# joshspeagle/brutus

Hardware: AMD Instinct MI355X
Metric: stars/sec at 750k-model x 12-band grid; achieved HBM GB/s vs peak (higher is better)
Workload: dtype f64; 1 GPU; configs[1]: 750k-model x 12-band grid, Av-only solve (rvlim=(3.32,3.32)), no parallax; grid = synth.make_mist_like_grid (lattice-ordered like the MIST grid files); grid_generator=mist_like, nmodel=750000, nfilt=12, sub_batch=128, selected_models_last_sub_batch=44670752, streams_per_gpu=3, parallelism=stars sharded, 1 rank(s), no data-path collective

## Files before the change

### brutus_amd/csrc/fastmath.hpp

```cpp
#pragma once

namespace {

__constant__ double kExp2Tbl[64] = {
    1, 1.0108892860517005, 1.0218971486541166, 1.0330248790212284,
    1.0442737824274138, 1.0556451783605572, 1.0671404006768237, 1.0787607977571199,
    1.0905077326652577, 1.1023825833078409, 1.1143867425958924, 1.1265216186082418,
    1.1387886347566916, 1.1511892299529827, 1.1637248587775775, 1.1763969916502812,
    1.189207115002721, 1.2021567314527031, 1.215247359980469, 1.22848053610687,
    1.241857812073484, 1.2553807570246911, 1.2690509571917332, 1.2828700160787783,
    1.2968395546510096, 1.3109612115247644, 1.3252366431597413, 1.3396675240533029,
    1.3542555469368927, 1.3690024229745905, 1.383909881963832, 1.3989796725383112,
    1.4142135623730951, 1.42961333839197, 1.4451808069770467, 1.460917794180647,
    1.4768261459394993, 1.4929077282912648, 1.5091644275934228, 1.5255981507445384,
    1.5422108254079407, 1.5590044002378369, 1.5759808451078865, 1.593142151342267,
    1.6104903319492543, 1.6280274218573478, 1.6457554781539649, 1.6636765803267364,
    1.681792830507429, 1.7001063537185235, 1.7186192981224779, 1.7373338352737062,
    1.7562521603732995, 1.7753764925265212, 1.7947090750031072, 1.8142521755003989,
    1.8340080864093424, 1.8539791250833855, 1.8741676341103, 1.8945759815869656,
    1.9152065613971474, 1.9360617934922943, 1.9571441241754002, 1.9784560263879509};

__device__ __forceinline__ double fast_exp10(double x, const double *__restrict__ tbl = kExp2Tbl) {
    const double ns = fma(x, 212.60339807279118, 6755399441055744.0);
    const double n = ns - 6755399441055744.0;
    double r = fma(-n, 0.0047035936804604717, x);
    r = fma(-n, 1.7892345153159123e-12, r);
    double pl = 0.5393829291955817;
    pl = fma(pl, r, 1.1712551489122673);
    pl = fma(pl, r, 2.034678592293477);
    pl = fma(pl, r, 2.6509490552391997);
    pl = fma(pl, r, 2.302585092994046);
    pl = fma(pl, r, 1.0);
    const int ni = __double2loint(ns);
    return ldexp(tbl[ni & 63] * pl, ni >> 6);
}

__device__ __forceinline__ double poly_exp10(double x) {
    const double n = rint(x * 3.3219280948873623);
    double r = fma(-n, 3.01029995663839276e-01, x);
    r = fma(-n, 1.42502325707809354e-17, r);
    const double t = r * 2.3025850929940457;
    double pl = 1.6059043836821613e-10;
    pl = fma(pl, t, 2.08767569878681e-09);
    pl = fma(pl, t, 2.505210838544172e-08);
    pl = fma(pl, t, 2.755731922398589e-07);
    pl = fma(pl, t, 2.7557319223985893e-06);
    pl = fma(pl, t, 2.48015873015873e-05);
    pl = fma(pl, t, 1.984126984126984e-04);
    pl = fma(pl, t, 1.3888888888888889e-03);
    pl = fma(pl, t, 8.333333333333333e-03);
    pl = fma(pl, t, 4.1666666666666664e-02);
    pl = fma(pl, t, 1.6666666666666666e-01);
    pl = fma(pl, t, 0.5);
    pl = fma(pl, t, 1.0);
    pl = fma(pl, t, 1.0);
    return ldexp(pl, (int)n);
}

__device__ __forceinline__ void stage_exp_table(double *lds_tbl) {
    if (threadIdx.x < 64) lds_tbl[threadIdx.x] = kExp2Tbl[threadIdx.x];
}

__device__ __forceinline__ double fast_exp(double x, const double *__restrict__ tbl = kExp2Tbl) {
    if (!(x > -745.)) return x == x ? 0. : x;
    const double n = rint(x * 92.332482616893657);
    double r = fma(-n, 0.01083042469326756, x);
    r = fma(-n, 2.9815858269852933e-12, r);
    double pl = 8.3333333333333332e-03;
    pl = fma(pl, r, 4.1666666666666664e-02);
    pl = fma(pl, r, 1.6666666666666666e-01);
    pl = fma(pl, r, 0.5);
    pl = fma(pl, r, 1.0);
    pl = fma(pl, r, 1.0);
    const int ni = (int)n;
    return ldexp(tbl[ni & 63] * pl, ni >> 6);
}

__device__ __forceinline__ double fast_log(double x) {
    if (!(x > 0.) || !(x < INFINITY)) return log(x);
    int e;
    double m = frexp(x, &e);
    if (m < 0.70710678118654752440) {
        m *= 2.;
        --e;
    }
    const double s = (m - 1.) / (m + 1.);
    const double z = s * s;
    double pl = 1. / 21.;
    pl = fma(pl, z, 1. / 19.);
    pl = fma(pl, z, 1. / 17.);
    pl = fma(pl, z, 1. / 15.);
    pl = fma(pl, z, 1. / 13.);
    pl = fma(pl, z, 1. / 11.);
    pl = fma(pl, z, 1. / 9.);
    pl = fma(pl, z, 1. / 7.);
    pl = fma(pl, z, 1. / 5.);
    pl = fma(pl, z, 1. / 3.);
    const double lm = fma(2. * s * z, pl, 2. * s);
    const double ed = (double)e;
    return fma(ed, 6.93147180369123816490e-01, fma(ed, 1.90821492927058770002e-10, lm));
}

__device__ __forceinline__ double fast_rcp(double x) {
    double r = __builtin_amdgcn_rcp(x);
    r = fma(fma(-x, r, 1.), r, r);
    r = fma(fma(-x, r, 1.), r, r);
    return r;
}
__device__ __forceinline__ void fast_sqrt_rsqrt(double x, double &sq, double &rsq) {
    const double y = __builtin_amdgcn_rsq(x);
    double g = x * y, h = 0.5 * y;
    const double r = fma(-h, g, 0.5);
    g = fma(g, r, g);
    h = fma(h, r, h);
    g = fma(fma(-g, g, x), h, g);
    g = fma(fma(-g, g, x), h, g);
    double y2 = h + h;
    y2 = fma(y2, fma(-y2, g, 1.), y2);
    y2 = fma(y2, fma(-y2, g, 1.), y2);
    sq = x == 0. ? 0. : g;
    rsq = y2;
}
__device__ __forceinline__ void fast_sqrt_rsqrt_pos(double x, double &sq, double &rsq) {
    const double y = __builtin_amdgcn_rsq(x);
    double g = x * y, h = 0.5 * y;
    const double r = fma(-h, g, 0.5);
    g = fma(g, r, g);
    h = fma(h, r, h);
    g = fma(fma(-g, g, x), h, g);
    g = fma(fma(-g, g, x), h, g);
    double y2 = h + h;
    y2 = fma(y2, fma(-y2, g, 1.), y2);
    y2 = fma(y2, fma(-y2, g, 1.), y2);
    sq = g;
    rsq = y2;
}
__device__ __forceinline__ double fast_sqrt_pos(double x) {
    double g, h;
    fast_sqrt_rsqrt_pos(x, g, h);
    return g;
}
__device__ __forceinline__ double fast_sqrt(double x) {
    double g, h;
    fast_sqrt_rsqrt(x, g, h);
    return g;
}
__device__ __forceinline__ double fast_exp_bf(double x, const double *__restrict__ tbl) {
    const double xc = fmax(x, -745.);
    const double ns = fma(xc, 92.332482616893657, 6755399441055744.0);
    const double n = ns - 6755399441055744.0;
    double r = fma(-n, 0.01083042469326756, xc);
    r = fma(-n, 2.9815858269852933e-12, r);
    double pl = 8.3333333333333332e-03;
    pl = fma(pl, r, 4.1666666666666664e-02);
    pl = fma(pl, r, 1.6666666666666666e-01);
    pl = fma(pl, r, 0.5);
    pl = fma(pl, r, 1.0);
    pl = fma(pl, r, 1.0);
    const int ni = __double2loint(ns);
    const double v = ldexp(tbl[ni & 63] * pl, ni >> 6);
    return x > -745. ? v : (x == x ? 0. : x);
}
__device__ __forceinline__ double fast_exp_fin(double x, const double *__restrict__ tbl) {
    const double xc = fmax(x, -745.);
    const double ns = fma(xc, 92.332482616893657, 6755399441055744.0);
    const double n = ns - 6755399441055744.0;
    double r = fma(-n, 0.01083042469326756, xc);
    r = fma(-n, 2.9815858269852933e-12, r);
    double pl = 8.3333333333333332e-03;
    pl = fma(pl, r, 4.1666666666666664e-02);
    pl = fma(pl, r, 1.6666666666666666e-01);
    pl = fma(pl, r, 0.5);
    pl = fma(pl, r, 1.0);
    pl = fma(pl, r, 1.0);
    const int ni = __double2loint(ns);
    return ldexp(tbl[ni & 63] * pl, ni >> 6);
}
__device__ __forceinline__ double fast_log_r(double x) {
    int e;
    double m = frexp(x, &e);
    const bool lo = m < 0.70710678118654752440;
    m = lo ? 2. * m : m;
    e = lo ? e - 1 : e;
    const double s = (m - 1.) * fast_rcp(m + 1.);
    const double z = s * s;
    double pl = 1. / 21.;
    pl = fma(pl, z, 1. / 19.);
    pl = fma(pl, z, 1. / 17.);
    pl = fma(pl, z, 1. / 15.);
    pl = fma(pl, z, 1. / 13.);
    pl = fma(pl, z, 1. / 11.);
    pl = fma(pl, z, 1. / 9.);
    pl = fma(pl, z, 1. / 7.);
    pl = fma(pl, z, 1. / 5.);
    pl = fma(pl, z, 1. / 3.);
    const double lm = fma(2. * s * z, pl, 2. * s);
    const double ed = (double)e;
    const double v = fma(ed, 6.93147180369123816490e-01, fma(ed, 1.90821492927058770002e-10, lm));
    return x > 0. ? (x < INFINITY ? v : x) : (x == 0. ? -INFINITY : nan(""));
}
__device__ __forceinline__ double fast_log_pos(double x) {
    int e;
    double m = frexp(x, &e);
    const bool lo = m < 0.70710678118654752440;
    m = lo ? 2. * m : m;
    e = lo ? e - 1 : e;
    const double s = (m - 1.) * fast_rcp(m + 1.);
    const double z = s * s;
    double pl = 1. / 21.;
    pl = fma(pl, z, 1. / 19.);
    pl = fma(pl, z, 1. / 17.);
    pl = fma(pl, z, 1. / 15.);
    pl = fma(pl, z, 1. / 13.);
    pl = fma(pl, z, 1. / 11.);
    pl = fma(pl, z, 1. / 9.);
    pl = fma(pl, z, 1. / 7.);
    pl = fma(pl, z, 1. / 5.);
    pl = fma(pl, z, 1. / 3.);
    const double lm = fma(2. * s * z, pl, 2. * s);
    const double ed = (double)e;
    return fma(ed, 6.93147180369123816490e-01, fma(ed, 1.90821492927058770002e-10, lm));
}

}
```

### brutus_amd/csrc/fit2_kernels.hpp

```cpp
#pragma once

#include "fit_kernels.hpp"
#include "pre32_types.hpp"

namespace {

static_assert(PS_TILE == TILE && PS_NBMAX == NBMAX, "pre32_types.hpp and common.hpp disagree");

struct CallInit {
    int32_t *ids_all, *kfix, *k2, *counters;
    int ncounters;
};
__global__ void __launch_bounds__(64)
k_prep32(int nstar, const StarPrep *__restrict__ stars, float eps_scale, int dim_prior,
         Star32 *__restrict__ out, CallInit init) {
    static_assert(NBMAX <= 64, "one lane per band");
    __shared__ double s_a[NBMAX], s_b[NBMAX], s_c[NBMAX];
    __shared__ double s_gbar, s_D;
    __shared__ int s_bad;
    const int s = blockIdx.x, j = threadIdx.x;
    if (s >= nstar) return;
    if (init.ids_all && j == 0) {
        init.ids_all[s] = s;
        init.kfix[s] = 2;
// ... 171 lines not shown
                    ub2 += bw;
                    uy2 += yw;
                    aa2 = pk_fma(a, aw, aa2);
                    ab2 = pk_fma(a, bw, ab2);
                    bb2 = pk_fma(b, bw, bb2);
                    ay2 = pk_fma(a, yw, ay2);
                    by2 = pk_fma(b, yw, by2);
                    yy2 = pk_fma(y, yw, yy2);
                }
                const float ua = hsum(ua2), ub = hsum(ub2), uy = hsum(uy2), aa = hsum(aa2),
                            ab = hsum(ab2), bb = hsum(bb2), ay = hsum(ay2), by = hsum(by2),
                            yy = hsum(yy2);
                auto sweep = [&](float &dav_o, float &drv_o) -> float {
                    const float uR = ua + rv * ub;
                    const float RR = aa + rv * (2.f * ab + rv * bb);
                    const float yR = ay + rv * by;
                    float rs = uy - av * uR;
                    const float ra = (yR - av * RR) + (p.av_mean - av) * p.av_ivar;
                    const float a_den = RR + p.av_ivar;
                    float dav = (sp.S * ra - uR * rs) * __builtin_amdgcn_rcpf(sp.S * a_den - uR * uR);
                    dav = fmaxf(dav, p.avmin - av);
                    dav = fminf(dav, p.avmax - av);
                    av += dav;
                    const float r_den = bb * av * av + p.rv_ivar;
                    const float sr = ub * av;
                    rs = uy - av * uR;
                    const float bres = by - av * (ab + rv * bb);
                    const float rr = av * bres + (p.rv_mean - rv) * p.rv_ivar;
                    float drv = (sp.S * rr - sr * rs) * __builtin_amdgcn_rcpf(sp.S * r_den - sr * sr);
                    drv = fmaxf(drv, p.rvmin - rv);
                    drv = fminf(drv, p.rvmax - rv);
                    rv += drv;
                    const float RR2 = aa + rv * (2.f * ab + rv * bb);
                    const float yR2 = ay + rv * by;
                    dav_o = dav;
                    drv_o = drv;
                    const float uR2 = ua + rv * ub;
                    const float oc = (uy - av * uR2) * __builtin_amdgcn_rcpf(sp.S);
                    const float tt0 = (sp.gbar - mbar) + oc;
                    return -0.5f * ((yy - av * (2.f * yR2 - av * RR2)) + sp.S * (tt0 * tt0 - oc * oc));
                };
                float d1, d2;
                if (K >= 1) {
                    const float lw = sweep(d1, d2);
                    if (live) {
                        if (lw == lw) {
                            const float st = fmaxf(fabsf(d1), fabsf(d2));
                            mx[g][0] = fmaxf(mx[g][0], lw);
                            if (st >= p.mtol_hi) mx[g][1] = fmaxf(mx[g][1], lw);
                            if (st >= p.mtol_lo) mx[g][2] = fmaxf(mx[g][2], lw);
                        } else {
                            mx[g][8] = 1.f;
                        }
                    }
                }
                if (K >= 2) {
                    const float lw = sweep(d1, d2);
                    if (live) {
                        if (lw == lw) {
                            const float st = fmaxf(fabsf(d1), fabsf(d2));
                            mx[g][3] = fmaxf(mx[g][3], lw);
                            if (st >= p.mtol_hi) mx[g][4] = fmaxf(mx[g][4], lw);
                            if (st >= p.mtol_lo) mx[g][5] = fmaxf(mx[g][5], lw);
                        } else {
                            mx[g][8] = 1.f;
                        }
                    }
                }
                for (int k = 2; k < K; ++k) sweep(d1, d2);
            }
            float num, den;
            if constexpr (RVF) {
                num = 0.f;
                den = 0.f;
#pragma unroll
                for (int j = 0; j < NB; ++j) {
                    const float e = __builtin_amdgcn_exp2f(fmaf(C10 * av, R[j], mcC[j]));
                    const float fw = e * sp.iv[j];
                    num = fmaf(sp.dd[j], fw, num);
                    den = fmaf(e, fw, den);
                }
            } else {
                f32x2 num2 = 0.f, den2 = 0.f;
#pragma unroll
                for (int j = 0; j < NB; j += 2) {
                    const f32x2 Rj = pk_fma((f32x2)rv, ld2(dr + j), ld2(R + j));
                    const f32x2 arg = C10 * pk_fma((f32x2)av, Rj, ld2(mc + j));
                    const f32x2 e = {__builtin_amdgcn_exp2f(arg.x), __builtin_amdgcn_exp2f(arg.y)};
                    const f32x2 fw = e * ld2(sp.iv + j);
                    num2 = pk_fma(ld2(sp.dd + j), fw, num2);
                    den2 = pk_fma(e, fw, den2);
                }
                num = hsum(num2);
                den = hsum(den2);
            }
            const float q = __builtin_amdgcn_exp2f(C10 * (sp.gbar - mbar));
            float tt = num * __builtin_amdgcn_rcpf(den);
            float sc = tt * q;
            if (sc <= 1e-20f) {
                sc = 1e-20f;
                tt = sc * __builtin_amdgcn_rcpf(q);
            }
            const float chi2 = fmaf(tt, fmaf(tt, den, -2.f * num), sp.DD2);
            const float lnl = -0.5f * chi2;
            float lnlp = lnl;
            if (sp.has_par) {
                const float dp = __builtin_amdgcn_sqrtf(sc) - sp.par;
                lnlp = lnl - 0.5f * (dp * dp * sp.par_ivar);
            }
            float lnpr = lnl;
            if (p.dim_prior) lnpr = sp.c0 + sp.c1 * __logf(chi2) - 0.5f * chi2;
            if (sp.sp_on) {
                const float vt = sp.sp_var + q * q * __builtin_amdgcn_rcpf(den);
                const float ds = sc - sp.sp_mean;
                lnpr += -0.5f * (ds * ds * __builtin_amdgcn_rcpf(vt) + __logf(6.2831853071795865f * vt));
            }
            if (!(chi2 > 4.f * sp.eps) || !sp.ok) lnlp = NAN;
            lnpr = surv_clean(lnpr);
            if (!(chi2 > sp.chi2_lo) || !sp.ok) lnpr = NAN;
            if (live) {
                const int64_t o = (int64_t)s * nmodel + i;
                lnlp32[o] = lnlp;
                lnpr32[o] = lnpr;
                if (lnlp != lnlp || lnpr != lnpr) mx[g][9] = 1.f;
                if (lnlp > mx[g][6]) mx[g][6] = lnlp;
                if (lnpr > mx[g][7]) mx[g][7] = lnpr;
            }
        }
    }
    const int lane = threadIdx.x & 63;
    const int wv = __builtin_amdgcn_readfirstlane(threadIdx.x >> 6);
#pragma unroll
    for (int g = 0; g < G; ++g)
#pragma unroll
        for (int v = 0; v < NV32; ++v) {
            float x = mx[g][v];
#pragma unroll
            for (int off = 32; off > 0; off >>= 1) x = fmaxf(x, __shfl_xor(x, off, 64));
            if (lane == 0) slot[wv][g * NV32 + v] = x;
        }
    __syncthreads();
    if (threadIdx.x < G * NV32) {
        const int g = threadIdx.x / NV32, v = threadIdx.x % NV32;
        if (g < ng) {
            const int s = star_ids[g0 + g];
            const float x = fmaxf(fmaxf(slot[0][threadIdx.x], slot[1][threadIdx.x]),
                                  fmaxf(slot[2][threadIdx.x], slot[3][threadIdx.x]));
            part[((int64_t)bx * nstar + s) * NV32 + v] = x;
        }
    }
}

__global__ void k_pre_decide(int nblkx, int nstar, const int32_t *__restrict__ star_ids,
                             const float *__restrict__ part, const Star32 *__restrict__ stars,
                             float ln_init, int rvf, int32_t *kfix,
                             int accept, float *__restrict__ st32, int32_t *__restrict__ k1,
                             int32_t *__restrict__ status, double *__restrict__ nomA,
                             int32_t *ctr, int32_t *__restrict__ probe_ids,
                             int32_t *__restrict__ redo_ids, const int32_t *nrun_dev) {
    __shared__ float sm[NV32][4];
    if (nrun_dev && (int)blockIdx.x >= *nrun_dev) return;
    const int s = star_ids[blockIdx.x];
    float v[NV32];
    for (int q = 0; q < NV32; ++q) v[q] = -INFINITY;
    for (int b = threadIdx.x; b < nblkx; b += blockDim.x) {
        const float *pp = part + ((int64_t)b * nstar + s) * NV32;
        for (int q = 0; q < NV32; ++q) v[q] = fmaxf(v[q], pp[q]);
    }
    for (int q = 0; q < NV32; ++q) {
        float x = v[q];
        for (int off = 32; off > 0; off >>= 1) x = fmaxf(x, __shfl_xor(x, off, 64));
        if ((threadIdx.x & 63) == 0) sm[q][threadIdx.x >> 6] = x;
    }
    __syncthreads();
    if (threadIdx.x != 0) return;
    for (int q = 0; q < NV32; ++q)
        v[q] = fmaxf(fmaxf(sm[q][0], sm[q][1]), fmaxf(sm[q][2], sm[q][3]));
    for (int q = 0; q < NV32; ++q) st32[(int64_t)s * NV32 + q] = v[q];
    const Star32 &sp = stars[s];
    const float ew = 2.f * sp.epsw;
    int st = 2, K1 = 0;
    const int K = kfix[s];
    if (sp.ok && !(v[8] > 0.f) && v[0] > -INFINITY) {
        const bool cont1 = v[1] > v[0] + ln_init + ew;
        const bool may1 = v[2] > v[0] + ln_init - ew;
        if (!may1) {
            K1 = 1;
            st = (rvf || K == 1) ? 0 : 1;
        } else if (cont1) {
            if (rvf) {
                K1 = 2;
                st = 0;
            } else if (K >= 2) {
                const bool cont2 = v[4] > v[3] + ln_init + ew;
                const bool may2 = v[5] > v[3] + ln_init - ew;
                if (!may2) {
                    K1 = 2;
                    st = (K == 2) ? 0 : 2;
                } else if (cont2) {
                    st = 2;
                }
            }
        }
    }
    if (!accept) {
        k1[s] = K1;
        status[s] = st;
        if (ctr) {
            if (st == 1) {
                kfix[s] = K1;
                redo_ids[atomicAdd(ctr + 1, 1)] = s;
            } else if (st == 2) {
                probe_ids[atomicAdd(ctr + 0, 1)] = s;
            }
        }
    }
    nomA[s] = (double)v[6] - 2. * (double)sp.eps;
}

template <int NB, bool RVF>
struct Tile64 {
    Coef<NB> c;
    double F0[NB];
    double R[RVF ? NB : 1];
};

template <int NB, bool RVF>
__device__ __forceinline__ void tile_load(const float *__restrict__ grid, int64_t nmodel_pad,
                                          int64_t i, double rv_mean, Tile64<NB, RVF> &t) {
    load_coef<NB>(grid, nmodel_pad, i, t.c);
    load_F0<NB>(grid, nmodel_pad, i, t.F0);
    if constexpr (RVF) coef_R<NB>(t.c, rv_mean, t.R);
}

template <int NB, bool RVF>
__device__ __forceinline__ void mag_phase(const Tile64<NB, RVF> &t, const StarPrep &sp,
                                          const DevParams &p, int K, double &av, double &rv) {
    av = p.av_mean;
    rv = p.rv_mean;
    if constexpr (RVF) {
        GramR Gm;
        gram_init_rf<NB>(t.c, t.R, sp, Gm);
        double a_, c_;
        if (K > 0) gram_sweep_rf(Gm, sp.S, p, av, a_, c_);
    } else {
        Gram Gm;
        gram_init<NB>(t.c, sp, Gm);
        for (int k = 0; k < K; ++k) {
            double a_, b_, c_;
            gram_sweep(Gm, sp.S, p, av, rv, a_, b_, c_);
        }
    }
}

template <int NB, bool RVF, bool FULL>
__device__ __forceinline__ void mle_at(const Tile64<NB, RVF> &t, const StarPrep &sp,
                                       const DevParams &p, double av, double rv,
                                       const double *__restrict__ tbl, Mle &m) {
    if constexpr (RVF) mle_fast_rf<NB, true, FULL ? 2 : 0>(t.c, t.R, t.F0, sp, p, av, tbl, m);
    else mle_fast<NB, true, FULL ? 2 : 0>(t.c, t.F0, sp, p, av, rv, tbl, m);
}

__device__ __forceinline__ void audit(float *__restrict__ aud, int s, float f32v, double f64v,
                                      double thr) {
    if (aud && f64v > thr - 12. && f32v == f32v) {
        const float d = fabsf((float)(f64v - (double)f32v));
        atomicMax(reinterpret_cast<int *>(aud + s), __float_as_int(d));
    }
}

__device__ __forceinline__ int64_t mword(int s, int ntile, int t, int w) {
    return (int64_t)s * (4 * ntile) + (int64_t)t * 4 + w;
}

__global__ void __launch_bounds__(256)
k_hot_list(int nblkx, int nstar, int mode, const float *__restrict__ part32,
           const double *__restrict__ nomA, const double *__restrict__ maxsurv,
           const Star32 *__restrict__ s32, double *__restrict__ nomB, double *__restrict__ part,
           int32_t *__restrict__ hot, int32_t *__restrict__ nhot) {
    const int s = blockIdx.x;
    double nm;
    if (mode == 0) {
        nm = nomA[s];
    } else {
        nm = maxsurv[s] - (double)s32[s].eps;
        if (threadIdx.x == 0) nomB[s] = nm;
    }
    for (int b = threadIdx.x; b < nblkx; b += blockDim.x) {
        const float *pp = part32 + ((int64_t)b * nstar + s) * NV32;
        const bool is_hot = !((double)pp[6 + mode] < nm) || pp[9] > 0.f;
        if (is_hot) hot[atomicAdd(nhot, 1)] = b * BRUTUS_MAX_BATCH + s;
        else part[(int64_t)b * nstar + s] = -INFINITY;
    }
}

template <int NB, bool RVF>
__global__ void __launch_bounds__(TILE, top_waves(NB))
k_top1(const float *__restrict__ grid, int64_t nmodel, int64_t nmodel_pad, int nstar,
       const StarPrep *__restrict__ stars, DevParams p, const int32_t *__restrict__ k1, int ntile,
       int mode, const float *__restrict__ plane32, const double *__restrict__ nom,
       const int32_t *__restrict__ hot, const int32_t *__restrict__ nhot,
       double *__restrict__ part, float *__restrict__ aud) {
    __shared__ double slot[4];
    __shared__ double s_tbl[64];
    const int n = *nhot;
    if ((int)blockIdx.x >= n) return;
    stage_exp_table(s_tbl);
    __syncthreads();
    const int lane = threadIdx.x & 63;
    for (int e = blockIdx.x; e < n; e += gridDim.x) {
        const int entry = hot[e];
        const int b = entry / BRUTUS_MAX_BATCH, s = entry - b * BRUTUS_MAX_BATCH;
        const int t0 = b * F2_T, t1 = min(ntile, t0 + F2_T);
        const StarPrep &sp = stars[s];
        const double nm_s = nom[s];
        const int K = k1[s];
        float v[F2_T];
#pragma unroll
        for (int u = 0; u < F2_T; ++u) {
            const int64_t i = (int64_t)(t0 + u) * TILE + threadIdx.x;
            v[u] = plane32[(int64_t)s * nmodel + (i < nmodel ? i : nmodel - 1)];
        }
        double mx = -INFINITY;
#pragma unroll
        for (int u = 0; u < F2_T; ++u) {
            const int64_t i = (int64_t)(t0 + u) * TILE + threadIdx.x;
            bool mine = t0 + u < t1 && i < nmodel && !((double)v[u] < nm_s);
            if (mode == 1 && mine) mine = !surv_is(v[u]);
            if (__ballot(mine) == 0ull) continue;
            Tile64<NB, RVF> tl;
            tile_load<NB, RVF>(grid, nmodel_pad, i, p.rv_mean, tl);
            double av, rv;
            mag_phase<NB, RVF>(tl, sp, p, K, av, rv);
            Mle m;
            mle_at<NB, RVF, false>(tl, sp, p, av, rv, s_tbl, m);
            double val;
            if (mode == 0) val = cull_stat(sp, m);
            else val = first_cut_lnprob(sp, final_lnl<false>(sp, p, m.chi2, false), m.scale, m.i00);
            if (mine) audit(aud, s, v[u], val, nm_s);
            if (mine && val == val) mx = val > mx ? val : mx;
        }
        block_max_store(mx, slot, part + (int64_t)b * nstar + s);
    }
}

__global__ void k_top_decide(int nblkx, int nstar, const int32_t *__restrict__ star_ids, int mode,
                             const double *__restrict__ part, const Star32 *__restrict__ s32,
                             double ln_thr, const double *__restrict__ maxsurv,
                             double *__restrict__ thr, double *__restrict__ cand) {
    __shared__ double sm[4];
    const int s = star_ids[blockIdx.x];
    double v = -INFINITY;
    for (int b = threadIdx.x; b < nblkx; b += blockDim.x) {
        const double x = part[(int64_t)b * nstar + s];
        v = x > v ? x : v;
    }
    v = wave_max(v);
    if ((threadIdx.x & 63) == 0) sm[threadIdx.x >> 6] = v;
    __syncthreads();
    if (threadIdx.x != 0) return;
    v = sm[0];
    for (int w = 1; w < 4; ++w) v = sm[w] > v ? sm[w] : v;
    if (mode == 0) {
        thr[s] = v + ln_thr;
        cand[s] = v + ln_thr - (double)s32[s].eps;
    } else {
        const double m = maxsurv[s] > v ? maxsurv[s] : v;
        thr[s] = m + ln_thr;
    }
}

__global__ void __launch_bounds__(TILE)
k_cmp_count32(int64_t nmodel, int ntile, const float *__restrict__ plane,
              const double *__restrict__ thr, int64_t *__restrict__ counts,
              unsigned long long *__restrict__ mask) {
    __shared__ int wsum[4];
    const int s = blockIdx.y, c = blockIdx.x;
    const int t0 = (int)((int64_t)ntile * c / NCHUNK), t1 = (int)((int64_t)ntile * (c + 1) / NCHUNK);
    const double th = thr[s];
    int n = 0;
#ifndef CNT_U
#define CNT_U 16
#endif
    constexpr int U = CNT_U;
    for (int tb = t0; tb < t1; tb += U) {
        float v[U];
#pragma unroll
        for (int u = 0; u < U; ++u) {
            const int64_t i = (int64_t)(tb + u) * TILE + threadIdx.x;
            const bool in = tb + u < t1 && i < nmodel;
            const float x = plane[(int64_t)s * nmodel + (in ? i : nmodel - 1)];
            v[u] = in ? x : -INFINITY;
        }
#pragma unroll
        for (int u = 0; u < U; ++u) {
            if (tb + u >= t1) break;
            const bool hit = !((double)v[u] < th);
            n += hit ? 1 : 0;
            const unsigned long long b = __ballot(hit);
            if ((threadIdx.x & 63) == 0)
                mask[(int64_t)s * (4 * ntile) + (int64_t)(tb + u) * 4 + (threadIdx.x >> 6)] = b;
        }
    }
#pragma unroll
    for (int off = 32; off > 0; off >>= 1) n += __shfl_xor(n, off, 64);
    if ((threadIdx.x & 63) == 0) wsum[threadIdx.x >> 6] = n;
    __syncthreads();
    if (threadIdx.x == 0) counts[(int64_t)s * NCHUNK + c] = wsum[0] + wsum[1] + wsum[2] + wsum[3];
}

__global__ void __launch_bounds__(TILE)
k_sel_classify(int64_t nmodel, int ntile, const Star32 *__restrict__ s32,
               const float *__restrict__ lnpr32,
               const double *__restrict__ lnprob_st, const int64_t *__restrict__ cand_off,
               const double *__restrict__ thr_sel,
               int64_t *__restrict__ counts, unsigned long long *__restrict__ mask,
               int64_t *__restrict__ dcounts, unsigned long long *__restrict__ dmask,
               int32_t *__restrict__ bandq, int32_t *__restrict__ bandn) {
    __shared__ int qn;
    __shared__ int wsum[4], dsum[4];
    if (threadIdx.x == 0) qn = 0;
    __syncthreads();
    const int s = blockIdx.y, c = blockIdx.x;
    const int t0 = (int)((int64_t)ntile * c / NCHUNK), t1 = (int)((int64_t)ntile * (c + 1) / NCHUNK);
    const double th = thr_sel[s];
    const double e = (double)s32[s].eps;
    const int64_t cbase = cand_off[s];
    int32_t *queue = bandq + (int64_t)s * nmodel + (int64_t)t0 * TILE;
    int n = 0, nd = 0;
#ifndef CLS_U
#define CLS_U 12
#endif
    constexpr int U = CLS_U;
    for (int tb = t0; tb < t1; tb += U) {
        float v32[U];
#pragma unroll
        for (int u = 0; u < U; ++u) {
            const int64_t i = (int64_t)(tb + u) * TILE + threadIdx.x;
            const bool in = tb + u < t1 && i < nmodel;
            const float x = lnpr32[(int64_t)s * nmodel + (in ? i : nmodel - 1)];
            v32[u] = in ? x : -INFINITY;
        }
        double vst[U];
#pragma unroll
        for (int u = 0; u < U; ++u)
            vst[u] = surv_is(v32[u]) ? lnprob_st[cbase + surv_slot(v32[u])] : 0.;
#pragma unroll
        for (int u = 0; u < U; ++u) {
            const int t = tb + u;
            if (t >= t1) break;
            const int64_t i = (int64_t)t * TILE + threadIdx.x;
            bool yes = false, der = false, bd = false;
            if (i < nmodel) {
                if (surv_is(v32[u])) {
                    yes = vst[u] > th;
                } else {
                    const double v = (double)v32[u];
                    yes = der = v >= th + e;
                    bd = !yes && !(v < th - e);
                }
            }
            n += yes ? 1 : 0;
            nd += der ? 1 : 0;
            const unsigned long long b = __ballot(yes), bdr = __ballot(der);
            if ((threadIdx.x & 63) == 0) {
                const int64_t a = (int64_t)s * (4 * ntile) + (int64_t)t * 4 + (threadIdx.x >> 6);
                mask[a] = b;
                dmask[a] = bdr;
            }
            if (bd) queue[atomicAdd(&qn, 1)] = (int32_t)i;
        }
    }
#pragma unroll
    for (int off = 32; off > 0; off >>= 1) {
        n += __shfl_xor(n, off, 64);
        nd += __shfl_xor(nd, off, 64);
    }
    if ((threadIdx.x & 63) == 0) {
        wsum[threadIdx.x >> 6] = n;
        dsum[threadIdx.x >> 6] = nd;
    }
    __syncthreads();
    if (threadIdx.x == 0) {
        counts[(int64_t)s * NCHUNK + c] = wsum[0] + wsum[1] + wsum[2] + wsum[3];
        dcounts[(int64_t)s * NCHUNK + c] = dsum[0] + dsum[1] + dsum[2] + dsum[3];
        bandn[s * NCHUNK + c] = qn;
    }
}

constexpr int LIST_U = 4;
static_assert(F2_T % LIST_U == 0, "a unit of the list passes must not straddle two blocks");

__device__ __forceinline__ unsigned long long
live_blocks(const float *__restrict__ part32, int nstar, int s, int b0, int blast, double cand,
            bool first_cut, double thr_lo) {
    const int b = b0 + (int)(threadIdx.x & 63);
    bool live = true;
    if (b <= blast) {
        const float *pp = part32 + ((int64_t)b * nstar + s) * NV32;
        const float m6 = pp[6], m7 = pp[7], f9 = pp[9];
        const bool dead = ((double)m6 < cand) & (f9 <= 0.f) & (!first_cut | ((double)m7 < thr_lo));
        live = !dead;
    }
    return __ballot(live);
}

template <bool V4>
__device__ __forceinline__ int64_t unit_model(int t, int k, int lane) {
    return (int64_t)t * TILE + (V4 ? 4 * lane + k : 64 * k + lane);
}
template <bool V4>
__device__ __forceinline__ void unit_load(const float *__restrict__ row, int64_t nmodel, int q,
                                          int ta, int tz, int lane, float (&v)[LIST_U][4]) {
#pragma unroll
    for (int u = 0; u < LIST_U; ++u) {
        const int t = q * LIST_U + u;
        const bool tin = t >= ta && t < tz;
        if constexpr (V4) {
            const int64_t i = unit_model<true>(t, 0, lane);
            const bool in = tin && i < nmodel;
            const float4 x = *reinterpret_cast<const float4 *>(row + (in ? i : nmodel - 4));
            v[u][0] = in ? x.x : -INFINITY;
            v[u][1] = in ? x.y : -INFINITY;
            v[u][2] = in ? x.z : -INFINITY;
            v[u][3] = in ? x.w : -INFINITY;
        } else {
#pragma unroll
            for (int k = 0; k < 4; ++k) {
                const int64_t i = unit_model<false>(t, k, lane);
                const bool in = tin && i < nmodel;
                const float x = row[in ? i : nmodel - 1];
                v[u][k] = in ? x : -INFINITY;
            }
        }
    }
}

template <bool V4>
__device__ __forceinline__ void tile_words(unsigned long long *__restrict__ mrow, int t, bool tin, int lane,
                                           const bool (&hit)[4]) {
    if constexpr (V4) {
        int y = ((hit[0] ? 1 : 0) | (hit[1] ? 2 : 0) | (hit[2] ? 4 : 0) | (hit[3] ? 8 : 0)) << (4 * (lane & 7));
        y |= dpp_i32<0xB1, 0xf>(y);
        y |= dpp_i32<0x4E, 0xf>(y);
        y |= dpp_i32<0x141, 0xf>(y);
        if (tin && (lane & 7) == 0) reinterpret_cast<int *>(mrow)[(int64_t)t * 8 + (lane >> 3)] = y;
    } else {
#pragma unroll
        for (int k = 0; k < 4; ++k) {
            const unsigned long long b = __ballot(hit[k]);
            if (tin && lane == 0) mrow[(int64_t)t * 4 + k] = b;
        }
    }
}
__device__ __forceinline__ void zero_words(unsigned long long *__restrict__ mrow, int ta, int tz, int lane) {
    if (lane < (tz - ta) * 8) reinterpret_cast<int *>(mrow)[(int64_t)ta * 8 + lane] = 0;
}

template <class F>
__device__ __forceinline__ void walk_units(int t0, int t1, const float *__restrict__ part32, int nstar,
                                           int s, double cand, bool first_cut, double thr_lo, F f) {
    if (t0 >= t1) return;
    constexpr int QB = F2_T / LIST_U;
    const int w = __builtin_amdgcn_readfirstlane((int)(threadIdx.x >> 6));
    const int blast = (t1 - 1) / F2_T;
    for (int bs = t0 / F2_T; bs <= blast; bs += 64) {
        const unsigned long long live = live_blocks(part32, nstar, s, bs, blast, cand, first_cut, thr_lo);
        const int qa = max(t0 / LIST_U, bs * QB);
        const int qz = min((t1 + LIST_U - 1) / LIST_U, (bs + 64) * QB);
        for (int q = qa + w; q < qz; q += TILE / 64)
            f(q, max(q * LIST_U, t0), min(q * LIST_U + LIST_U, t1), ((live >> (q / QB - bs)) & 1ull) != 0ull);
    }
}

template <bool V4>
__global__ void __launch_bounds__(TILE)
k_cmp_count32_live(int64_t nmodel, int ntile, int nstar, const float *__restrict__ plane,
                   const float *__restrict__ part32, const double *__restrict__ thr,
                   int64_t *__restrict__ counts, unsigned long long *__restrict__ mask) {
    __shared__ int wsum[4];
    const int s = blockIdx.y, c = blockIdx.x;
    const int t0 = (int)((int64_t)ntile * c / NCHUNK), t1 = (int)((int64_t)ntile * (c + 1) / NCHUNK);
    const double th = thr[s];
    const int lane = threadIdx.x & 63;
    const float *row = plane + (int64_t)s * nmodel;
    unsigned long long *mrow = mask + (int64_t)s * (4 * ntile);
    int n = 0;
    walk_units(t0, t1, part32, nstar, s, th, false, 0., [&](int q, int ta, int tz, bool live) {
        if (!live) {
            zero_words(mrow, ta, tz, lane);
            return;
        }
        float v[LIST_U][4];
        unit_load<V4>(row, nmodel, q, ta, tz, lane, v);
#pragma unroll
        for (int u = 0; u < LIST_U; ++u) {
            const int t = q * LIST_U + u;
            const bool tin = t >= ta && t < tz;
            bool hit[4];
#pragma unroll
            for (int k = 0; k < 4; ++k) {
                hit[k] = tin & (unit_model<V4>(t, k, lane) < nmodel) & !((double)v[u][k] < th);
                n += hit[k] ? 1 : 0;
            }
            tile_words<V4>(mrow, t, tin, lane, hit);
        }
    });
#pragma unroll
    for (int off = 32; off > 0; off >>= 1) n += __shfl_xor(n, off, 64);
    if (lane == 0) wsum[threadIdx.x >> 6] = n;
    __syncthreads();
    if (threadIdx.x == 0) counts[(int64_t)s * NCHUNK + c] = wsum[0] + wsum[1] + wsum[2] + wsum[3];
}

__global__ void __launch_bounds__(TILE)
k_sel_classify_live(int64_t nmodel, int ntile, int nstar, const Star32 *__restrict__ s32,
                    const float *__restrict__ lnpr32, const float *__restrict__ part32,
                    const double *__restrict__ candS,
                    const double *__restrict__ lnprob_st, const int64_t *__restrict__ cand_off,
                    const double *__restrict__ thr_sel,
                    int64_t *__restrict__ counts, unsigned long long *__restrict__ mask,
                    int64_t *__restrict__ dcounts, unsigned long long *__restrict__ dmask,
                    int32_t *__restrict__ bandq, int32_t *__restrict__ bandn) {
    __shared__ int qn;
    __shared__ int wsum[4], dsum[4];
    if (threadIdx.x == 0) qn = 0;
    __syncthreads();
    const int s = blockIdx.y, c = blockIdx.x;
    const int t0 = (int)((int64_t)ntile * c / NCHUNK), t1 = (int)((int64_t)ntile * (c + 1) / NCHUNK);
    const double th = thr_sel[s];
    const double e = (double)s32[s].eps;
    const int64_t cbase = cand_off[s];
    const int lane = threadIdx.x & 63;
    const float *row = lnpr32 + (int64_t)s * nmodel;
    unsigned long long *mrow = mask + (int64_t)s * (4 * ntile), *drow = dmask + (int64_t)s * (4 * ntile);
    int32_t *queue = bandq + (int64_t)s * nmodel + (int64_t)t0 * TILE;
    int n = 0, nd = 0;
    walk_units(t0, t1, part32, nstar, s, candS[s], true, th - e, [&](int q, int ta, int tz, bool live) {
        if (!live) {
            zero_words(mrow, ta, tz, lane);
            zero_words(drow, ta, tz, lane);
            return;
        }
        float v32[LIST_U][4];
        unit_load<true>(row, nmodel, q, ta, tz, lane, v32);
        double vst[LIST_U][4];
#pragma unroll
        for (int u = 0; u < LIST_U; ++u)
#pragma unroll
            for (int k = 0; k < 4; ++k)
                vst[u][k] = surv_is(v32[u][k]) ? lnprob_st[cbase + surv_slot(v32[u][k])] : 0.;
#pragma unroll
        for (int u = 0; u < LIST_U; ++u) {
            const int t = q * LIST_U + u;
            const bool tin = t >= ta && t < tz;
            bool yes[4], der[4];
#pragma unroll
            for (int k = 0; k < 4; ++k) {
                const int64_t i = unit_model<true>(t, k, lane);
                bool bd = false;
                yes[k] = der[k] = false;
                if (tin && i < nmodel) {
                    if (surv_is(v32[u][k])) {
                        yes[k] = vst[u][k] > th;
                    } else {
                        const double v = (double)v32[u][k];
                        yes[k] = der[k] = v >= th + e;
                        bd = !yes[k] && !(v < th - e);
                    }
                }
                n += yes[k] ? 1 : 0;
                nd += der[k] ? 1 : 0;
                if (bd) queue[atomicAdd(&qn, 1)] = (int32_t)i;
            }
            tile_words<true>(mrow, t, tin, lane, yes);
            tile_words<true>(drow, t, tin, lane, der);
        }
    });
#pragma unroll
    for (int off = 32; off > 0; off >>= 1) {
        n += __shfl_xor(n, off, 64);
        nd += __shfl_xor(nd, off, 64);
    }
    if (lane == 0) {
        wsum[threadIdx.x >> 6] = n;
        dsum[threadIdx.x >> 6] = nd;
    }
    __syncthreads();
    if (threadIdx.x == 0) {
        counts[(int64_t)s * NCHUNK + c] = wsum[0] + wsum[1] + wsum[2] + wsum[3];
        dcounts[(int64_t)s * NCHUNK + c] = dsum[0] + dsum[1] + dsum[2] + dsum[3];
        bandn[s * NCHUNK + c] = qn;
    }
}

constexpr int SB_C = 8, SB_Z = 8;
template <int NB, bool RVF>
__global__ void __launch_bounds__(TILE, band_waves(NB))
k_sel_band(const float *__restrict__ grid, int64_t nmodel, int64_t nmodel_pad, int ntile,
           const StarPrep *__restrict__ stars, DevParams p, const int32_t *__restrict__ k1,
           const float *__restrict__ lnpr32, const double *__restrict__ thr_sel,
           const int32_t *__restrict__ bandq, const int32_t *__restrict__ bandn,
           int64_t *__restrict__ counts, unsigned long long *__restrict__ mask,
           int64_t *__restrict__ dcounts, unsigned long long *__restrict__ dmask,
           float *__restrict__ aud) {
    const int s = blockIdx.y, c0 = blockIdx.x * SB_C;
    int pre[SB_C + 1];
    pre[0] = 0;
#pragma unroll
    for (int k = 0; k < SB_C; ++k) pre[k + 1] = pre[k] + bandn[s * NCHUNK + c0 + k];
    const int n = pre[SB_C];
    if ((int)(blockIdx.z * TILE) >= n) return;
    __shared__ double s_tbl[64];
    stage_exp_table(s_tbl);
    __syncthreads();
    const StarPrep &sp = stars[s];
    const double th = thr_sel[s];
    const int K = k1[s];
    for (int q = blockIdx.z * TILE + threadIdx.x; q < n; q += TILE * gridDim.z) {
        int k = 0;
#pragma unroll
        for (int j = 1; j < SB_C; ++j) k += q >= pre[j] ? 1 : 0;
        int qk = q;
#pragma unroll
        for (int j = 1; j < SB_C; ++j) qk = k == j ? q - pre[j] : qk;
        const int c = c0 + k;
        const int t0 = (int)((int64_t)ntile * c / NCHUNK);
        const int64_t i = bandq[(int64_t)s * nmodel + (int64_t)t0 * TILE + qk];
        Tile64<NB, RVF> tl;
        gather_coef<NB>(grid, nmodel_pad, i, tl.c);
        compute_F0_tbl<NB>(tl.c, s_tbl, tl.F0);
        if constexpr (RVF) coef_R<NB>(tl.c, p.rv_mean, tl.R);
        double av, rv;
        mag_phase<NB, RVF>(tl, sp, p, K, av, rv);
        Mle m;
        mle_at<NB, RVF, false>(tl, sp, p, av, rv, s_tbl, m);
        const double lnprob =
            first_cut_lnprob(sp, final_lnl<false>(sp, p, m.chi2, false), m.scale, m.i00);
        audit(aud, s, lnpr32[(int64_t)s * nmodel + i], lnprob, th);
        if (lnprob > th) {
            atomicOr(mask + (int64_t)s * (4 * ntile) + (i >> 6), 1ull << (i & 63));
            atomicOr(dmask + (int64_t)s * (4 * ntile) + (i >> 6), 1ull << (i & 63));
            atomicAdd(reinterpret_cast<unsigned long long *>(counts + (int64_t)s * NCHUNK + c), 1ull);
            atomicAdd(reinterpret_cast<unsigned long long *>(dcounts + (int64_t)s * NCHUNK + c), 1ull);
        }
    }
}


__global__ void k_k1_deep_decide(int ntile, int kmax, const double *__restrict__ part,
                                 double ln_init, int32_t *__restrict__ out_k1) {
    __shared__ double sm[2][4];
    __shared__ int done;
    if (threadIdx.x == 0) done = 0;
    __syncthreads();
    for (int k = 0; k < kmax; ++k) {
        double L = -INFINITY, T = -INFINITY;
        for (int t = threadIdx.x; t < ntile; t += blockDim.x) {
            const double *pp = part + (int64_t)t * (2 * kmax) + 2 * k;
            L = pp[0] > L ? pp[0] : L;
            T = pp[1] > T ? pp[1] : T;
        }
        L = wave_max(L);
        T = wave_max(T);
        if ((threadIdx.x & 63) == 0) {
            sm[0][threadIdx.x >> 6] = L;
            sm[1][threadIdx.x >> 6] = T;
        }
        __syncthreads();
        if (threadIdx.x == 0) {
            for (int w = 1; w < 4; ++w) {
                L = sm[0][w] > L ? sm[0][w] : L;
                T = sm[1][w] > T ? sm[1][w] : T;
            }
            L = L > -BIG ? L : -BIG;
            if (!(T > L + ln_init)) {
                *out_k1 = k + 1;
                done = 1;
            }
        }
        __syncthreads();
        if (done) return;
    }
    if (threadIdx.x == 0) *out_k1 = 0;
}

}
```

### brutus_amd/csrc/fit_kernels.hpp

```cpp
#pragma once

#include "common.hpp"
#include "fastmath.hpp"
#include "grid_kernels.hpp"

namespace {


struct Gram {
    double ua, ub, uy, aa, ab, bb, ay, by, yy;
};

template <int NB>
__device__ __forceinline__ void gram_init(const Coef<NB> &c, const StarPrep &sp, Gram &G) {
    double ua = 0., ub = 0., uy = 0., aa = 0., ab = 0., bb = 0., ay = 0., by = 0., yy = 0.;
#pragma unroll
    for (int j = 0; j < NB; ++j) {
        const double w = sp.iW[j];
        const double a = (double)c.r0[j], b = (double)c.dr[j];
        const double y = sp.g[j] - (double)c.m[j];
        const double aw = a * w, bw = b * w, yw = y * w;
        ua += aw;
        ub += bw;
        uy += yw;
        aa += a * aw;
        ab += a * bw;
        bb += b * bw;
        ay += a * yw;
        by += b * yw;
        yy += y * yw;
    }
    G.ua = ua; G.ub = ub; G.uy = uy; G.aa = aa; G.ab = ab; G.bb = bb;
    G.ay = ay; G.by = by; G.yy = yy;
}

__device__ __forceinline__ void gram_sweep(const Gram &G, double S, const DevParams &p, double &av,
                                           double &rv, double &dav_o, double &drv_o,
                                           double &logwt) {
    const double uR = G.ua + rv * G.ub;
    const double RR = G.aa + rv * (2. * G.ab + rv * G.bb);
    const double yR = G.ay + rv * G.by;
    double rs = G.uy - av * uR;
    const double ra = (yR - av * RR) + (p.av_mean - av) * p.av_ivar;
    const double a_den = RR + p.av_ivar;
    double dav = (S * ra - uR * rs) / (S * a_den - uR * uR);
    if (dav < p.avmin - av) dav = p.avmin - av;
    if (dav > p.avmax - av) dav = p.avmax - av;
    av = av + dav;
    const double r_den = G.bb * av * av + p.rv_ivar;
    const double sr = G.ub * av;
    rs = G.uy - av * uR;
    const double bres = G.by - av * (G.ab + rv * G.bb);
    const double rr = av * bres + (p.rv_mean - rv) * p.rv_ivar;
    double drv = (S * rr - sr * rs) / (S * r_den - sr * sr);
    if (drv < p.rvmin - rv) drv = p.rvmin - rv;
    if (drv > p.rvmax - rv) drv = p.rvmax - rv;
    rv = rv + drv;
    const double RR2 = G.aa + rv * (2. * G.ab + rv * G.bb);
    const double yR2 = G.ay + rv * G.by;
    const double chi2 = G.yy - av * (2. * yR2 - av * RR2);
    dav_o = dav;
    drv_o = drv;
    logwt = -0.5 * chi2;
}

template <int NB, bool TBL, int LV = 2>
__device__ __forceinline__ void mle_fast(const Coef<NB> &c, const double (&F0)[NB],
                                         const StarPrep &sp, const DevParams &p, double av,
                                         double rv, const double *__restrict__ tbl, Mle &o) {
    const double fac = -0.92103403719761827361;
    const double mav = -0.4 * av;
    double F[NB];
    double s_num = 0., s_den = 0.;
#pragma unroll
    for (int j = 0; j < NB; ++j) {
        const double R = (double)c.r0[j] + rv * (double)c.dr[j];
        const double f = F0[j] * (TBL ? fast_exp10(mav * R, tbl) : poly_exp10(mav * R));
        F[j] = f;
        const double fw = f * sp.iV[j];
        s_num += sp.d[j] * fw;
        s_den += f * fw;
    }
    double s = s_num / s_den;
    if (s <= 1e-20) s = 1e-20;
    double SA = 0., SR = 0., AR = 0., AA = 0., RR = 0., AN = 0., RN = 0., chi2 = 0.;
    const double s2 = s + s;
#pragma unroll
    for (int j = 0; j < NB; ++j) {
        const double iv = sp.iV[j];
        const double D0 = (double)c.dr[j];
        const double R0 = (double)c.r0[j] + rv * D0;
        const double u = R0 * F[j], v = D0 * F[j];
        const double res = fma(-s, F[j], sp.d[j]);
        const double rw = res * iv, uw = u * iv, vw = v * iv;
        chi2 = fma(res, rw, chi2);
        AN = fma(u, rw, AN);
        AA = fma(u, uw, AA);
        if (LV >= 1) {
            RN = fma(v, rw, RN);
            RR = fma(v, vw, RR);
        }
        if (LV >= 2) {
            const double t = fma(s2, F[j], -sp.d[j]);
            const double q = fma(-s, F0[j], t);
            SA = fma(uw, t, SA);
            SR = fma(vw, t, SR);
            AR = fma(vw, q, AR);
        }
    }
    const double cs = fac * s, cs2 = cs * cs;
    double a_den = cs2 * AA, r_den = cs2 * RR;
    const double a_num = cs * AN, r_num = cs * RN;
    const double sa_mix = fac * SA, sr_mix = fac * SR, ar_mix = cs * AR;
    o.a_ss = a_den;
    o.r_ss = r_den;
    o.a_num = a_num;
    o.r_num = r_num;
    a_den += p.av_ivar;
    r_den += p.rv_ivar;
    a_den += p.a_reg;
    r_den += p.r_reg;
    o.scale = s;
    o.chi2 = chi2;
    o.i00 = s_den;
    o.i01 = sa_mix;
    o.i02 = sr_mix;
    o.i11 = a_den;
    o.i12 = ar_mix;
    o.i22 = r_den;
}


struct GramR {
    double uR, RR, yR, uy, yy;
};

template <int NB>
__device__ __forceinline__ void coef_R(const Coef<NB> &c, double rv, double (&R)[NB]) {
#pragma unroll
    for (int j = 0; j < NB; ++j) R[j] = (double)c.r0[j] + rv * (double)c.dr[j];
}

template <int NB>
__device__ __forceinline__ void gram_init_rf(const Coef<NB> &c, const double (&R)[NB],
                                             const StarPrep &sp, GramR &G) {
    double uR = 0., RR = 0., yR = 0., uy = 0., yy = 0.;
#pragma unroll
    for (int j = 0; j < NB; ++j) {
        const double w = sp.iW[j];
        const double y = sp.g[j] - (double)c.m[j];
        const double Rw = R[j] * w, yw = y * w;
        uR += Rw;
        RR += R[j] * Rw;
        yR += R[j] * yw;
        uy += yw;
        yy += y * yw;
    }
    G.uR = uR; G.RR = RR; G.yR = yR; G.uy = uy; G.yy = yy;
}

__device__ __forceinline__ void gram_sweep_rf(const GramR &G, double S, const DevParams &p,
                                              double &av, double &dav_o, double &logwt) {
    const double rs = G.uy - av * G.uR;
    const double ra = (G.yR - av * G.RR) + (p.av_mean - av) * p.av_ivar;
    const double a_den = G.RR + p.av_ivar;
    double dav = (S * ra - G.uR * rs) / (S * a_den - G.uR * G.uR);
    if (dav < p.avmin - av) dav = p.avmin - av;
    if (dav > p.avmax - av) dav = p.avmax - av;
    av = av + dav;
    const double chi2 = G.yy - av * (2. * G.yR - av * G.RR);
    dav_o = dav;
    logwt = -0.5 * chi2;
}

template <int NB, bool TBL, int LV>
__device__ __forceinline__ void mle_fast_rf(const Coef<NB> &c, const double (&R)[NB],
                                            const double (&F0)[NB], const StarPrep &sp,
                                            const DevParams &p, double av,
                                            const double *__restrict__ tbl, Mle &o) {
    const double fac = -0.92103403719761827361;
    const double mav = -0.4 * av;
    double F[NB];
    double s_num = 0., s_den = 0.;
#pragma unroll
    for (int j = 0; j < NB; ++j) {
        const double f = F0[j] * (TBL ? fast_exp10(mav * R[j], tbl) : poly_exp10(mav * R[j]));
        F[j] = f;
        const double fw = f * sp.iV[j];
        s_num += sp.d[j] * fw;
        s_den += f * fw;
    }
    double s = s_num / s_den;
    if (s <= 1e-20) s = 1e-20;
    double SA = 0., SR = 0., AR = 0., AA = 0., RR = 0., AN = 0., RN = 0., chi2 = 0.;
    const double s2 = s + s;
#pragma unroll
    for (int j = 0; j < NB; ++j) {
        const double iv = sp.iV[j];
        const double u = R[j] * F[j];
        const double res = fma(-s, F[j], sp.d[j]);
        const double rw = res * iv, uw = u * iv;
        chi2 = fma(res, rw, chi2);
        AN = fma(u, rw, AN);
        AA = fma(u, uw, AA);
        if (LV >= 2) {
            const double t = fma(s2, F[j], -sp.d[j]);
            const double v = (double)c.dr[j] * F[j];
            const double q = fma(-s, F0[j], t);
            const double vw = v * iv;
            SA = fma(uw, t, SA);
            RN = fma(v, rw, RN);
            RR = fma(v, vw, RR);
            SR = fma(vw, t, SR);
            AR = fma(vw, q, AR);
        }
    }
    const double cs = fac * s, cs2 = cs * cs;
    double a_den = cs2 * AA, r_den = cs2 * RR;
    const double a_num = cs * AN, r_num = cs * RN;
    const double sa_mix = fac * SA, sr_mix = fac * SR, ar_mix = cs * AR;
    o.a_ss = a_den;
    o.r_ss = r_den;
    o.a_num = a_num;
    o.r_num = r_num;
    a_den += p.av_ivar;
    r_den += p.rv_ivar;
    a_den += p.a_reg;
    r_den += p.r_reg;
    o.scale = s;
    o.chi2 = chi2;
    o.i00 = s_den;
    o.i01 = sa_mix;
    o.i02 = sr_mix;
    o.i11 = a_den;
    o.i12 = ar_mix;
    o.i22 = r_den;
}

#ifndef BRUTUS_WIDE_FROM
#define BRUTUS_WIDE_FROM 25
#endif
constexpr bool wide_bands(int nb) { return nb >= BRUTUS_WIDE_FROM; }
#ifndef BRUTUS_LIST_OCC1_FROM
#define BRUTUS_LIST_OCC1_FROM 17
#endif
constexpr int list_waves(int nb) { return nb >= BRUTUS_LIST_OCC1_FROM ? 1 : 2; }
#ifndef BRUTUS_FFLUX_OCC1_FROM
#define BRUTUS_FFLUX_OCC1_FROM BRUTUS_LIST_OCC1_FROM
#endif
constexpr int fflux_waves(int nb, bool first) {
    return nb >= (first ? BRUTUS_FFLUX_OCC1_FROM : BRUTUS_LIST_OCC1_FROM) ? 1 : 2;
}
constexpr int top_waves(int nb) { return nb > 24 ? 1 : 2; }
constexpr int band_waves(int nb) { return nb > 16 ? 1 : 2; }
typedef __attribute__((address_space(3))) volatile double *LdsColumn;
#ifndef BRUTUS_WIDE_GROUP
#define BRUTUS_WIDE_GROUP 32
#endif
__device__ __forceinline__ double wide_f64(float x, double after) {
    double r;
    asm("v_cvt_f64_f32_e32 %0, %1" : "=v"(r) : "v"(x), "v"(after));
    return r;
}
#define WIDE_ANCHOR(var, sum) if (j % BRUTUS_WIDE_GROUP == 0 && j) var = (sum)

template <int NB, int LV>
__device__ __forceinline__ void mle_wide(const Coef<NB> &c, const StarPrep &sp,
                                         const DevParams &p, double av, double rv,
                                         const double *__restrict__ tbl, LdsColumn Fc,
                                         Mle &o) {
    const double fac = -0.92103403719761827361;
    const double mav = -0.4 * av;
    double s_num = 0., s_den = 0.;
    double after = mav;
#pragma unroll
    for (int j = 0; j < NB; ++j) {
        WIDE_ANCHOR(after, s_den);
        const double R = fma(rv, wide_f64(c.dr[j], after), wide_f64(c.r0[j], after));
        const double f = fast_exp10(fma(mav, R, -0.4 * wide_f64(c.m[j], after)), tbl);
        Fc[j * TILE] = f;
        const double fw = f * sp.iV[j];
        s_num += sp.d[j] * fw;
        s_den += f * fw;
    }
    double s = s_num / s_den;
    if (s <= 1e-20) s = 1e-20;
    double SA = 0., SR = 0., AR = 0., AA = 0., RR = 0., AN = 0., RN = 0., chi2 = 0.;
    const double s2 = s + s;
    after = s;
#pragma unroll
    for (int j = 0; j < NB; ++j) {
        WIDE_ANCHOR(after, chi2);
        const double iv = sp.iV[j];
        const double f = Fc[j * TILE];
        const double D0 = wide_f64(c.dr[j], after);
        const double u = fma(rv, D0, wide_f64(c.r0[j], after)) * f;
        const double res = fma(-s, f, sp.d[j]);
        const double rw = res * iv, uw = u * iv;
        chi2 = fma(res, rw, chi2);
        AN = fma(u, rw, AN);
        AA = fma(u, uw, AA);
        if (LV >= 1) {
            const double v = D0 * f;
            const double vw = v * iv;
            RN = fma(v, rw, RN);
            RR = fma(v, vw, RR);
            if (LV >= 2) {
                const double t = fma(s2, f, -sp.d[j]);
                const double q = fma(-s, fast_exp10(-0.4 * wide_f64(c.m[j], after), tbl), t);
                SA = fma(uw, t, SA);
                SR = fma(vw, t, SR);
                AR = fma(vw, q, AR);
            }
        }
    }
    const double cs = fac * s, cs2 = cs * cs;
    double a_den = cs2 * AA, r_den = cs2 * RR;
    o.a_ss = a_den;
    o.r_ss = r_den;
    o.a_num = cs * AN;
    o.r_num = cs * RN;
    a_den += p.av_ivar;
    r_den += p.rv_ivar;
    a_den += p.a_reg;
    r_den += p.r_reg;
    o.scale = s;
    o.chi2 = chi2;
    o.i00 = s_den;
    o.i01 = fac * SA;
    o.i02 = fac * SR;
    o.i11 = a_den;
    o.i12 = cs * AR;
    o.i22 = r_den;
}

template <int NB>
__device__ __forceinline__ void gram_init_rf_wide(const Coef<NB> &c, double rv,
                                                  const StarPrep &sp, GramR &G) {
    double uR = 0., RR = 0., yR = 0., uy = 0., yy = 0.;
    double after = rv;
#pragma unroll
    for (int j = 0; j < NB; ++j) {
        WIDE_ANCHOR(after, yy);
        const double w = sp.iW[j];
        const double R = fma(rv, wide_f64(c.dr[j], after), wide_f64(c.r0[j], after));
        const double y = sp.g[j] - wide_f64(c.m[j], after);
        const double Rw = R * w, yw = y * w;
        uR += Rw;
        RR += R * Rw;
        yR += R * yw;
        uy += yw;
        yy += y * yw;
    }
    G.uR = uR; G.RR = RR; G.yR = yR; G.uy = uy; G.yy = yy;
}

template <int NB, bool RVF, bool FULL, int NR, int NF>
__device__ __forceinline__ void mle_list(const Coef<NB> &c, const double (&R)[NR],
                                         const double (&F0)[NF], LdsColumn Fc,
                                         const StarPrep &sp, const DevParams &p, double av,
                                         double rv, const double *__restrict__ tbl, Mle &o) {
    constexpr int LV = FULL ? 2 : RVF ? 0 : 1;
    if constexpr (wide_bands(NB)) mle_wide<NB, LV>(c, sp, p, av, rv, tbl, Fc, o);
    else if constexpr (RVF) mle_fast_rf<NB, true, LV>(c, R, F0, sp, p, av, tbl, o);
    else mle_fast<NB, true, LV>(c, F0, sp, p, av, rv, tbl, o);
}

template <int NB>
__device__ __forceinline__ void load_F0(const float *__restrict__ grid, int64_t nmodel_pad,
                                        int64_t i, double (&F0)[NB]) {
    const double *t = reinterpret_cast<const double *>(grid + (int64_t)6 * NB * nmodel_pad);
#pragma unroll
    for (int j = 0; j < NB; ++j) F0[j] = t[(int64_t)j * nmodel_pad + i];
}
template <int NB>
__device__ __forceinline__ void compute_F0_fast(const Coef<NB> &c, double (&F0)[NB]) {
#pragma unroll
    for (int j = 0; j < NB; ++j) F0[j] = poly_exp10(-0.4 * (double)c.m[j]);
}
template <int NB>
__device__ __forceinline__ void compute_F0_tbl(const Coef<NB> &c, const double *__restrict__ tbl,
                                               double (&F0)[NB]) {
#pragma unroll
    for (int j = 0; j < NB; ++j) F0[j] = fast_exp10(-0.4 * (double)c.m[j], tbl);
}

template <bool FASTLOG = false>
__device__ __forceinline__ double final_lnl(const StarPrep &sp, const DevParams &p, double chi2,
                                            bool survivor) {
    if (p.dim_prior)
        return chi2 > 0. ? sp.c0 + sp.c1 * (FASTLOG ? fast_log_r(chi2) : log(chi2)) - chi2 / 2.
                         : -INFINITY;
    return survivor ? -0.5 * chi2 + sp.lnl_const : -0.5 * chi2;
}
__device__ __forceinline__ double first_cut_lnprob(const StarPrep &sp, double lnl, double scale,
                                                   double i00) {
    double lnprob = lnl;
    if (sp.sp_on) {
        const double serr2 = 1. / fabs(i00);
        const double vt = sp.sp_var + serr2;
        const double ds = scale - sp.sp_mean;
        lnprob = lnl + -0.5 * (ds * ds / vt + log(2. * M_PI * vt));
    }
    if (!isfinite(lnprob)) lnprob = -BIG;
    return lnprob;
}

__device__ __forceinline__ double cull_stat(const StarPrep &sp, const Mle &m) {
    double lnlp = -0.5 * m.chi2;
    if (sp.has_par) {
        const double dp = sqrt(m.scale) - sp.par;
        lnlp -= 0.5 * (dp * dp * sp.par_ivar);
    }
    return lnlp;
}

template <int NB, int KS, bool RVF>
__global__ void __launch_bounds__(TILE)
k_k1probe(const float *__restrict__ grid, int64_t nmodel, int64_t nmodel_pad, int nstar, int nrun,
          const int32_t *__restrict__ star_ids, const StarPrep *__restrict__ stars, DevParams p,
          int tiles_per_block, int ntile, double *__restrict__ part,
          const int32_t *__restrict__ nrun_dev) {
    constexpr int NV = 2 * KS;
    __shared__ double slot[4];
    if (nrun_dev) nrun = *nrun_dev;
    for (int y = blockIdx.y; y < nrun; y += gridDim.y) {
    const int s = star_ids[y];
    const StarPrep &sp = stars[s];
    double mx[NV];
#pragma unroll
    for (int v = 0; v < NV; ++v) mx[v] = -INFINITY;
    const int t0 = blockIdx.x * tiles_per_block;
    const int t1 = min(ntile, t0 + tiles_per_block);
    for (int t = t0; t < t1; ++t) {
        const int64_t i = (int64_t)t * TILE + threadIdx.x;
        const bool live = i < nmodel;
        Coef<NB> c;
        load_coef<NB>(grid, nmodel_pad, i, c);
        double av = p.av_mean, rv = p.rv_mean;
        if constexpr (RVF) {
            double R[NB];
            coef_R<NB>(c, p.rv_mean, R);
            GramR G;
            gram_init_rf<NB>(c, R, sp, G);
            double dav, lw;
            gram_sweep_rf(G, sp.S, p, av, dav, lw);
            if (live && lw == lw) {
                mx[0] = lw > mx[0] ? lw : mx[0];
                if (fabs(dav) >= p.mtol) mx[1] = lw > mx[1] ? lw : mx[1];
#pragma unroll
                for (int k = 1; k < KS; ++k) mx[2 * k] = lw > mx[2 * k] ? lw : mx[2 * k];
            }
        } else {
            Gram G;
            gram_init<NB>(c, sp, G);
#pragma unroll
            for (int k = 0; k < KS; ++k) {
                double dav, drv, lw;
                gram_sweep(G, sp.S, p, av, rv, dav, drv, lw);
                if (live && lw == lw) {
                    const bool big = (fabs(dav) >= p.mtol) || (fabs(drv) >= p.mtol);
                    mx[2 * k] = lw > mx[2 * k] ? lw : mx[2 * k];
                    if (big) mx[2 * k + 1] = lw > mx[2 * k + 1] ? lw : mx[2 * k + 1];
                }
            }
        }
    }
#pragma unroll
    for (int v = 0; v < NV; ++v)
        block_max_store(mx[v], slot, part + ((int64_t)blockIdx.x * nstar + s) * NV + v);
    }
}

__global__ void k_k1_decide(int nblkx, int nstar, const int32_t *__restrict__ star_ids, int KS,
                            const double *__restrict__ part, double ln_init,
                            int32_t *__restrict__ k1, const int32_t *nrun_dev, int32_t *kfix,
                            int32_t *ctr, int32_t *__restrict__ redo_ids, int rvf, int max_iter) {
    __shared__ double sm[KCAP * 2][4];
    if (nrun_dev && (int)blockIdx.x >= *nrun_dev) return;
    const int s = star_ids[blockIdx.x];
    const int NV = 2 * KS;
    double v[KCAP * 2];
    for (int q = 0; q < NV; ++q) v[q] = -INFINITY;
    for (int b = threadIdx.x; b < nblkx; b += blockDim.x) {
        const double *pp = part + ((int64_t)b * nstar + s) * NV;
        for (int q = 0; q < NV; ++q) v[q] = pp[q] > v[q] ? pp[q] : v[q];
    }
    for (int q = 0; q < NV; ++q) {
        const double m = wave_max(v[q]);
        if ((threadIdx.x & 63) == 0) sm[q][threadIdx.x >> 6] = m;
    }
    __syncthreads();
    if (threadIdx.x != 0) return;
    int K1 = 0;
    for (int k = 0; k < KS; ++k) {
        double L = sm[2 * k][0], T = sm[2 * k + 1][0];
        for (int w = 1; w < 4; ++w) {
            L = sm[2 * k][w] > L ? sm[2 * k][w] : L;
            T = sm[2 * k + 1][w] > T ? sm[2 * k + 1][w] : T;
        }
        L = L > -BIG ? L : -BIG;
        if (!(T > L + ln_init)) {
            K1 = k + 1;
            break;
        }
    }
    k1[s] = K1;
    if (ctr) {
        if (K1 == 0 || K1 > max_iter) {
            atomicOr(ctr + 3, 1);
        } else {
            kfix[s] = K1;
            if (!rvf && K1 != 2) redo_ids[atomicAdd(ctr + 1, 1)] = s;
        }
    }
}

struct OffsetsJob {
    const int64_t *counts;
    int64_t *offsets, *star_off;
    int32_t *wbase;
    int64_t *total_out;
};
constexpr int OFF_T = 1024;
__global__ void __launch_bounds__(OFF_T)
k_offsets(int nstar, OffsetsJob job0, OffsetsJob job1) {
    constexpr int NT = OFF_T;
    constexpr int EPT = (BRUTUS_MAX_BATCH * NCHUNK + NT - 1) / NT;
    __shared__ int64_t s_slot64[NT / 64 + 1];
    __shared__ int32_t s_slot32[NT / 64 + 1];
    const OffsetsJob job = (blockIdx.x >> 1) == 0 ? job0 : job1;
    const bool items = (blockIdx.x & 1) != 0;
    const int64_t *__restrict__ counts = job.counts;
    const int total = nstar * NCHUNK;
    const int ept = (total + NT - 1) / NT;
    const int e0 = threadIdx.x * ept;
    if (!items) {
        int64_t r[EPT];
        int64_t sum = 0;
#pragma unroll
        for (int k = 0; k < EPT; ++k) {
            const int e = e0 + k;
            const int64_t v = counts[e < total ? e : total - 1];
            r[k] = k < ept && e < total ? v : 0;
            sum += r[k];
        }
        int64_t all;
        int64_t pre = block_exclusive_sum<int64_t, NT>(sum, s_slot64, all);
#pragma unroll
        for (int k = 0; k < EPT; ++k) {
            if (k < ept && e0 + k < total) {
                job.offsets[e0 + k] = pre;
                if ((e0 + k) % NCHUNK == 0) job.star_off[(e0 + k) / NCHUNK] = pre;
            }
            pre += r[k];
        }
        if (threadIdx.x == 0) {
            job.star_off[nstar] = all;
            if (job.total_out) *job.total_out = all;
        }
        return;
    }
    if (!job.wbase) return;
    {
        int32_t r[EPT];
        int32_t sum = 0;
        int c = e0 / nstar, q = e0 - c * nstar;
#pragma unroll
        for (int k = 0; k < EPT; ++k) {
            const int e = e0 + k;
            const bool in = k < ept && e < total;
            const int64_t v = counts[in ? (int64_t)q * NCHUNK + c : 0];
            r[k] = in ? (int32_t)((v + TILE - 1) / TILE) : 0;
            sum += r[k];
            if (++q == nstar) {
                q = 0;
                ++c;
            }
        }
        int32_t all;
        int32_t pre = block_exclusive_sum<int32_t, NT>(sum, s_slot32, all);
#pragma unroll
        for (int k = 0; k < EPT; ++k) {
            if (k < ept && e0 + k < total) job.wbase[e0 + k] = pre;
            pre += r[k];
        }
        if (threadIdx.x == 0) job.wbase[total] = all;
    }
}

__global__ void __launch_bounds__(TILE)
k_cmp_scatter(int64_t nmodel, int ntile, const unsigned long long *__restrict__ mask,
              const int64_t *__restrict__ offsets, int64_t capacity,
              int32_t *__restrict__ out_idx) {
    __shared__ int s_slot[TILE / 64 + 1];
    __shared__ unsigned long long s_word[TILE];
    __shared__ int s_pre[TILE];
    const int s = blockIdx.y, c = blockIdx.x;
    const int t0 = (int)((int64_t)ntile * c / NCHUNK), t1 = (int)((int64_t)ntile * (c + 1) / NCHUNK);
    int64_t base = offsets[(int64_t)s * NCHUNK + c];
    const int lane = threadIdx.x & 63, w = threadIdx.x >> 6;
    const unsigned long long below = (1ull << lane) - 1ull;
    const unsigned long long *__restrict__ row = mask + (int64_t)s * (4 * ntile);
    for (int tb = t0; tb < t1; tb += TILE / 4) {
        const int nt = min(TILE / 4, t1 - tb);
        const unsigned long long word =
            (int)threadIdx.x < 4 * nt ? row[(int64_t)tb * 4 + threadIdx.x] : 0ull;
        int tot;
        const int pre = block_exclusive_sum<int, TILE>(__popcll(word), s_slot, tot);
        s_word[threadIdx.x] = word;
        s_pre[threadIdx.x] = pre;
        __syncthreads();
#pragma unroll 4
        for (int k = 0; k < nt; ++k) {
            const unsigned long long b = s_word[4 * k + w];
            if ((b >> lane) & 1ull) {
                const int64_t r = base + s_pre[4 * k + w] + __popcll(b & below);
                if (r < capacity) out_idx[r] = (int32_t)((int64_t)(tb + k) * TILE + threadIdx.x);
            }
        }
        base += tot;
        __syncthreads();
    }
}

constexpr int SURV_TAG_END = 27 << 23;
__device__ __forceinline__ float surv_tag(int64_t slot) { return __int_as_float((int)slot + 1); }
__device__ __forceinline__ bool surv_is(float x) {
    const int b = __float_as_int(x);
    return b > 0 && b < SURV_TAG_END;
}
__device__ __forceinline__ float surv_clean(float x) { return fabsf(x) < 0x1p-100f ? 0.f : x; }
__device__ __forceinline__ int surv_slot(float x) { return __float_as_int(x) - 1; }

struct ItemGeom {
    int64_t q0;
    int32_t s, n;
};
__global__ void k_items(int nstar, const int32_t *__restrict__ wbase,
                        const int64_t *__restrict__ offsets, const int64_t *__restrict__ star_off,
                        ItemGeom *__restrict__ items) {
    const int e = blockIdx.x * blockDim.x + threadIdx.x;
    if (e >= NCHUNK * nstar) return;
    const int c = e / nstar, s = e - c * nstar;
    const int64_t start = offsets[(int64_t)s * NCHUNK + c];
    const int64_t end = c + 1 < NCHUNK ? offsets[(int64_t)s * NCHUNK + c + 1] : star_off[s + 1];
    const int first = wbase[e], np = wbase[e + 1] - first;
    for (int k = 0; k < np; ++k) {
        ItemGeom g;
        g.q0 = start + (int64_t)k * TILE;
        g.s = s;
        g.n = (int)(end - g.q0 < TILE ? end - g.q0 : TILE);
        items[first + k] = g;
    }
}

constexpr int LIST_RUN = 16;
struct ItemWalk {
    const int32_t *wbase;
    int nstar, c, item, me, nw, run, left, end, rot;
    __device__ __forceinline__ void seek() {
        for (; c < NCHUNK; c += 8) {
            const int base = wbase[c * nstar];
            end = wbase[(c + 1) * nstar];
            int r = me - rot;
            if (r < 0) r += nw;
            if (run > 1) rot = (rot + (end - base + run - 1) / run) % nw;
            item = base + r * run;
            left = run;
            if (item < end) return;
        }
        item = -1;
    }
    __device__ __forceinline__ void init(const int32_t *wb, int ns, int xcd, int me_, int nw_, int run_) {
        wbase = wb;
        nstar = ns;
        me = me_;
        nw = nw_;
        run = run_;
        if (run_ < 0) {
            const int even = wb[NCHUNK * ns] / (8 * nw_);
            run = -run_ < even ? -run_ : even > 1 ? even : 1;
        }
        rot = 0;
        c = xcd;
        seek();
    }
    __device__ __forceinline__ bool done() const { return item < 0; }
    __device__ __forceinline__ void next() {
        ++item;
        if (--left == 0) {
            item += (nw - 1) * run;
            left = run;
        }
        if (item >= end) {
            c += 8;
            seek();
        }
    }
};

constexpr int CONT_P = 16;
struct SegWalk {
    int item, end;
    __device__ __forceinline__ void init(const int32_t *wbase, int nstar, const int32_t *act, int nact,
                                         int unit) {
        const int c = unit % NCHUNK, a = (unit / NCHUNK) % nact;
        const int piece = unit / (NCHUNK * nact);
        const int e = c * nstar + act[a];
        end = wbase[e + 1];
        item = wbase[e] + piece;
        if (item >= end) item = -1;
    }
    __device__ __forceinline__ bool done() const { return item < 0; }
    __device__ __forceinline__ void next() {
        item += CONT_P;
        if (item >= end) item = -1;
    }
};

template <int NB>
__device__ __forceinline__ void gather_coef(const float *__restrict__ grid, int64_t nmodel_pad,
                                            int64_t i, Coef<NB> &c) {
    const float4 *row =
        reinterpret_cast<const float4 *>(grid + (int64_t)3 * NB * nmodel_pad + i * (3 * NB));
    float t[3 * NB];
#pragma unroll
    for (int q = 0; q < 3 * NB / 4; ++q) {
        const float4 v = row[q];
        t[4 * q] = v.x;
        t[4 * q + 1] = v.y;
        t[4 * q + 2] = v.z;
        t[4 * q + 3] = v.w;
    }
#pragma unroll
    for (int j = 0; j < NB; ++j) {
        c.m[j] = t[3 * j];
        c.r0[j] = t[3 * j + 1];
        c.dr[j] = t[3 * j + 2];
    }
}

typedef float f32x4 __attribute__((ext_vector_type(4)));
template <int NB>
struct RowRegs {
    f32x4 q[3 * NB / 4];
};
template <int NB>
__device__ __forceinline__ void gather_row(const float *__restrict__ grid, int64_t nmodel_pad,
                                           int64_t i, RowRegs<NB> &r) {
    const f32x4 *row =
        reinterpret_cast<const f32x4 *>(grid + (int64_t)3 * NB * nmodel_pad + i * (3 * NB));
#pragma unroll
    for (int q = 0; q < 3 * NB / 4; ++q) r.q[q] = row[q];
}
template <int NB>
__device__ __forceinline__ void row_to_coef(const RowRegs<NB> &r, Coef<NB> &c) {
    float t[3 * NB];
#pragma unroll
    for (int q = 0; q < 3 * NB / 4; ++q) {
        t[4 * q] = r.q[q].x;
        t[4 * q + 1] = r.q[q].y;
        t[4 * q + 2] = r.q[q].z;
        t[4 * q + 3] = r.q[q].w;
    }
#pragma unroll
    for (int j = 0; j < NB; ++j) {
        c.m[j] = t[3 * j];
        c.r0[j] = t[3 * j + 1];
        c.dr[j] = t[3 * j + 2];
    }
}
template <int NB>
__device__ __forceinline__ void landed(RowRegs<NB> &r) {
#pragma unroll
    for (int q = 0; q < 3 * NB / 4; ++q) {
        f32x4 t = r.q[q];
        asm volatile("" : "+v"(t) : : "memory");
        r.q[q] = t;
    }
}
__device__ __forceinline__ void landed(int32_t &x) {
    int32_t t = x;
    asm volatile("" : "+v"(t) : : "memory");
    x = t;
}

struct RecPlanes {
    double *vals;
    int64_t cap;
    __device__ __forceinline__ double *plane(int v) const { return vals + (int64_t)v * cap; }
};

template <int NB, bool RVF, bool FIRST>
__global__ void __launch_bounds__(TILE, fflux_waves(NB, FIRST))
k_fflux(const float *__restrict__ grid, int64_t nmodel, int64_t nmodel_pad, int nstar,
        const StarPrep *__restrict__ stars, DevParams p, const int32_t *__restrict__ k1,
        const int32_t *__restrict__ k2state, const int32_t *__restrict__ cand_idx,
        const int64_t *__restrict__ cand_off, const int32_t *__restrict__ wbase,
        const ItemGeom *__restrict__ items, RecPlanes rec, double *__restrict__ step_st,
        double *__restrict__ lnprob_st, double *__restrict__ part, float *__restrict__ surv32,
        const double *__restrict__ thr_cull, const int32_t *__restrict__ act, int nact,
        const int32_t *__restrict__ nact_dev, int run) {
    if (!FIRST && nact_dev) nact = *nact_dev;
    if (!FIRST && nact <= 0) return;
    __shared__ double s_tbl[64];
    stage_exp_table(s_tbl);
    __syncthreads();
    constexpr bool WIDE = wide_bands(NB);
    __shared__ double s_F[WIDE ? NB * TILE : 1];
    const LdsColumn Fc = (LdsColumn)s_F + (WIDE ? threadIdx.x : 0);
    constexpr int niter = FIRST ? 2 : 1;
    int s_nxt = 0;
    auto lane_model = [&](int item) -> int32_t {
        const ItemGeom ig = items[item < 0 ? 0 : item];
        s_nxt = ig.s;
        const int64_t q = ig.q0 + threadIdx.x;
        const int64_t last = ig.q0 + ig.n - 1;
        return cand_idx[q < last ? q : last];
    };
    double *__restrict__ r_lnl = rec.plane(0), *__restrict__ r_chi2 = rec.plane(1),
                        *__restrict__ r_scale = rec.plane(2), *__restrict__ r_av = rec.plane(3),
                        *__restrict__ r_rv = rec.plane(4);
    auto walk = [&](auto &wk) {
    int32_t i_nxt = lane_model(wk.item);
    constexpr bool PER_STAR = FIRST && NB <= 12;
    double aL = -INFINITY, aT = -INFINITY, aM = -INFINITY;
    while (!wk.done()) {
        const int item = wk.item;
        wk.next();
        const ItemGeom ig = items[item];
        const int s = ig.s;
        const int32_t i_me = i_nxt;
        i_nxt = lane_model(wk.item);
        if (k2state[s] < 0) {
            landed(i_nxt);
            continue;
        }
        const StarPrep &sp = stars[s];
        const int64_t q = ig.q0 + threadIdx.x;
        const bool live = (int)threadIdx.x < ig.n && q < rec.cap;
        double L = -INFINITY, T = -INFINITY, M = -INFINITY;
        bool go = live;
        const int64_t i = i_me;
        const int64_t o = (int64_t)s * nmodel + i;
        if (!FIRST && live) go = surv_is(surv32[o]);
        Mle m;
        double o_lnl = 0., o_lnprob = 0., o_av = 0., o_rv = 0., o_step = 0.;
        bool store = false;
        if (go) {
            Coef<NB> c;
            gather_coef<NB>(grid, nmodel_pad, i, c);
            double F0[WIDE ? 1 : NB];
#ifdef BRUTUS_F0_FROM_TABLE
            if constexpr (!WIDE) load_F0<NB>(grid, nmodel_pad, i, F0);
#else
            if constexpr (!WIDE) compute_F0_tbl<NB>(c, s_tbl, F0);
#endif
            double av, rv, step, lnl_old;
            double R[RVF && !WIDE ? NB : 1];
            if constexpr (RVF && !WIDE) coef_R<NB>(c, p.rv_mean, R);
            if constexpr (FIRST) {
                av = p.av_mean;
                rv = p.rv_mean;
                const int K = k1[s];
                if constexpr (RVF) {
                    GramR G;
                    if constexpr (WIDE) gram_init_rf_wide<NB>(c, p.rv_mean, sp, G);
                    else gram_init_rf<NB>(c, R, sp, G);
                    for (int k = 0; k < K; ++k) {
                        double a_, c_;
                        gram_sweep_rf(G, sp.S, p, av, a_, c_);
                    }
                } else {
                    Gram G;
                    gram_init<NB>(c, sp, G);
                    for (int k = 0; k < K; ++k) {
                        double a_, b_, c_;
                        gram_sweep(G, sp.S, p, av, rv, a_, b_, c_);
                    }
                }
                step = 1.0;
                lnl_old = -BIG;
            } else {
                av = r_av[q];
                rv = RVF ? p.rv_mean : r_rv[q];
                step = step_st[q];
                lnl_old = -0.5 * r_chi2[q];
            }
            mle_list<NB, RVF, false>(c, R, F0, Fc, sp, p, av, rv, s_tbl, m);
            if constexpr (FIRST) {
                go = cull_stat(sp, m) > thr_cull[s];
                if (go) surv32[o] = surv_tag(q - cand_off[s]);
            }
            double lnl_new = lnl_old, dl = 0.;
            for (int it = 0; go && it < niter; ++it) {
                double dav = (m.a_num + (p.av_mean - av) * p.av_ivar) / (m.a_ss + p.av_ivar) * step;
                if (dav < p.avmin - av) dav = p.avmin - av;
                if (dav > p.avmax - av) dav = p.avmax - av;
                av += dav;
                if constexpr (RVF) {
                    if (it + 1 < niter) mle_list<NB, RVF, false>(c, R, F0, Fc, sp, p, av, rv, s_tbl, m);
                    else mle_list<NB, RVF, true>(c, R, F0, Fc, sp, p, av, rv, s_tbl, m);
                } else {
                    double drv = (m.r_num + (p.rv_mean - rv) * p.rv_ivar) / (m.r_ss + p.rv_ivar) * step;
                    if (drv < p.rvmin - rv) drv = p.rvmin - rv;
                    if (drv > p.rvmax - rv) drv = p.rvmax - rv;
                    rv += drv;
                    constexpr bool SHORT_FIRST = NB != 16;
                    if (SHORT_FIRST && it + 1 < niter) mle_list<NB, RVF, false>(c, R, F0, Fc, sp, p, av, rv, s_tbl, m);
                    else mle_list<NB, RVF, true>(c, R, F0, Fc, sp, p, av, rv, s_tbl, m);
                }
                lnl_new = -0.5 * m.chi2;
                dl = fabs(lnl_new - lnl_old);
                if (lnl_new < lnl_old) step /= 1.2;
                lnl_old = lnl_new;
            }
            if (go) {
                o_lnl = final_lnl<RVF>(sp, p, m.chi2, true);
                o_lnprob = first_cut_lnprob(sp, o_lnl, m.scale, m.i00);
                o_av = av;
                o_rv = rv;
                o_step = step;
                M = o_lnprob;
                if (lnl_new == lnl_new) {
                    L = lnl_new;
                    if (dl > p.ltol) T = lnl_new;
                }
            }
            store = go;
        }
        landed(i_nxt);
        if (store) {
#define FF_ST(p, x) __builtin_nontemporal_store((x), (p) + q)
            FF_ST(r_lnl, o_lnl);
            FF_ST(r_chi2, m.chi2);
            FF_ST(r_scale, m.scale);
            FF_ST(r_av, o_av);
            if constexpr (!RVF) FF_ST(r_rv, o_rv);
            FF_ST(rec.plane(5), m.i00);
            FF_ST(rec.plane(6), m.i01);
            FF_ST(rec.plane(7), m.i02);
            FF_ST(rec.plane(8), m.i11);
            FF_ST(rec.plane(9), m.i12);
            FF_ST(rec.plane(10), m.i22);
            FF_ST(step_st, o_step);
            FF_ST(lnprob_st, o_lnprob);
#undef FF_ST
        }
        if constexpr (PER_STAR) {
            aL = L > aL ? L : aL;
            aT = T > aT ? T : aT;
            aM = M > aM ? M : aM;
            L = T = M = -INFINITY;
            if (wk.done() || s_nxt != s) {
                L = wave_max_dpp(aL);
                T = wave_max_dpp(aT);
                M = wave_max_dpp(aM);
                aL = aT = aM = -INFINITY;
            }
        } else {
            L = wave_max_dpp(L);
            T = wave_max_dpp(T);
            M = wave_max_dpp(M);
        }
        if ((threadIdx.x & 63) == 0) {
            double *out = part + ((int64_t)item * (TILE / 64) + (threadIdx.x >> 6)) * 3;
            out[0] = L;
            out[1] = T;
            out[2] = M;
        }
    }
    };
    if constexpr (FIRST) {
        ItemWalk wk;
        wk.init(wbase, nstar, blockIdx.x & 7, blockIdx.x >> 3, (gridDim.x + 7 - (blockIdx.x & 7)) >> 3, run);
        walk(wk);
    } else {
        const int nunit = NCHUNK * nact * CONT_P;
        for (int unit = blockIdx.x; unit < nunit; unit += gridDim.x) {
            SegWalk wk;
            wk.init(wbase, nstar, act, nact, unit);
            walk(wk);
        }
    }
}

__global__ void k_fflux_decide(int nstar, const int32_t *__restrict__ wbase,
                               const double *__restrict__ part, double ln_sub,
                               int32_t *__restrict__ k2state, double *__restrict__ maxsurv,
                               int32_t *__restrict__ n_unconv, int32_t *__restrict__ act,
                               int32_t *__restrict__ zero_next) {
    __shared__ double sm[3][4];
    const int s = blockIdx.x;
    if (zero_next && s == 0 && threadIdx.x == 0) *zero_next = 0;
    if (k2state[s] < 0) return;
    double v[3] = {-INFINITY, -INFINITY, -INFINITY};
    const int per = TILE / 64;
    {
        const int lpc = blockDim.x / NCHUNK;
        const int c = threadIdx.x / lpc, j = threadIdx.x - c * lpc;
        const int e = c * nstar + s;
        const int lo = wbase[e] * per, hi = wbase[e + 1] * per;
        constexpr int U = 4;
        for (int it = lo + j; it < hi; it += U * lpc) {
            double x[U][3];
#pragma unroll
            for (int u = 0; u < U; ++u) {
                const int a = it + u * lpc < hi ? it + u * lpc : it;
#pragma unroll
                for (int q = 0; q < 3; ++q) x[u][q] = part[(int64_t)a * 3 + q];
            }
#pragma unroll
            for (int u = 0; u < U; ++u)
#pragma unroll
                for (int q = 0; q < 3; ++q) v[q] = x[u][q] > v[q] ? x[u][q] : v[q];
        }
    }
    for (int q = 0; q < 3; ++q) {
        const double m = wave_max(v[q]);
        if ((threadIdx.x & 63) == 0) sm[q][threadIdx.x >> 6] = m;
    }
    __syncthreads();
    if (threadIdx.x != 0) return;
    for (int q = 0; q < 3; ++q) {
        double m = sm[q][0];
        for (int w = 1; w < 4; ++w) m = sm[q][w] > m ? sm[q][w] : m;
        v[q] = m;
    }
    maxsurv[s] = v[2];
    if (v[1] > v[0] + ln_sub) {
        k2state[s] += 1;
        const int q = atomicAdd(n_unconv, 1);
        if (act) act[q] = s;
    } else {
        k2state[s] = -k2state[s] - 1;
    }
}

__global__ void __launch_bounds__(TILE)
k_rec_index(int64_t nmodel, int ntile, int nstar, const unsigned long long *__restrict__ mask,
            const unsigned long long *__restrict__ dmask,
            const unsigned long long *__restrict__ cmask, const int64_t *__restrict__ offsets,
            const int64_t *__restrict__ doffsets, const int64_t *__restrict__ coffsets,
            const int64_t *__restrict__ cand_off, int64_t capacity,
            int32_t *__restrict__ rec_idx, int32_t *__restrict__ rec_slot,
            int32_t *__restrict__ der_idx) {
    __shared__ unsigned long long s_slot[TILE / 64 + 1];
    __shared__ unsigned long long s_word[3][TILE];
    __shared__ unsigned long long s_pre[TILE];
    const int s = blockIdx.y, c = blockIdx.x;
    const int t0 = (int)((int64_t)ntile * c / NCHUNK), t1 = (int)((int64_t)ntile * (c + 1) / NCHUNK);
    int64_t base = offsets[(int64_t)s * NCHUNK + c];
    int64_t dbase = doffsets[(int64_t)s * NCHUNK + c] + cand_off[nstar];
    int64_t cbase = coffsets[(int64_t)s * NCHUNK + c];
    const int lane = threadIdx.x & 63, w = threadIdx.x >> 6;
    const unsigned long long below = (1ull << lane) - 1ull;
    const int64_t row = (int64_t)s * (4 * ntile);
    constexpr unsigned long long F20 = (1ull << 20) - 1ull;
    for (int tb = t0; tb < t1; tb += TILE / 4) {
        const int nt = min(TILE / 4, t1 - tb);
        const bool in = (int)threadIdx.x < 4 * nt;
        const int64_t a = row + (int64_t)tb * 4 + (in ? threadIdx.x : 0);
        unsigned long long wm = mask[a], wd = dmask[a], wc = cmask[a];
        if (!in) wm = wd = wc = 0ull;
        unsigned long long tot;
        const unsigned long long pre = block_exclusive_sum<unsigned long long, TILE>(
            (unsigned long long)__popcll(wm) | ((unsigned long long)__popcll(wd) << 20) |
                ((unsigned long long)__popcll(wc) << 40),
            s_slot, tot);
        s_word[0][threadIdx.x] = wm;
        s_word[1][threadIdx.x] = wd;
        s_word[2][threadIdx.x] = wc;
        s_pre[threadIdx.x] = pre;
        __syncthreads();
#pragma unroll 4
        for (int k = 0; k < nt; ++k) {
            const unsigned long long b = s_word[0][4 * k + w];
            if ((b >> lane) & 1ull) {
                const unsigned long long bd = s_word[1][4 * k + w], bc = s_word[2][4 * k + w];
                const unsigned long long pk = s_pre[4 * k + w];
                const int32_t i = (int32_t)((int64_t)(tb + k) * TILE + threadIdx.x);
                const int64_t r = base + (int64_t)(pk & F20) + __popcll(b & below);
                int64_t slot;
                if ((bd >> lane) & 1ull) {
                    slot = dbase + (int64_t)((pk >> 20) & F20) + __popcll(bd & below);
                    der_idx[slot - cand_off[nstar]] = i;
                } else {
                    slot = cbase + (int64_t)(pk >> 40) + __popcll(bc & below);
                }
                if (r < capacity) {
                    rec_idx[r] = i;
                    rec_slot[r] = (int32_t)slot;
                }
            }
        }
        base += (int64_t)(tot & F20);
        dbase += (int64_t)((tot >> 20) & F20);
        cbase += (int64_t)(tot >> 40);
        __syncthreads();
    }
}

template <int NB, bool RVF>
__global__ void __launch_bounds__(TILE, list_waves(NB))
k_derive(const float *__restrict__ grid, int64_t nmodel_pad, int nstar,
         const StarPrep *__restrict__ stars, DevParams p, const int32_t *__restrict__ k1,
         const int32_t *__restrict__ der_idx, const int32_t *__restrict__ wbase,
         const ItemGeom *__restrict__ items, const int64_t *__restrict__ cand_off,
         RecPlanes rec, int run) {
    __shared__ double s_tbl[64];
    stage_exp_table(s_tbl);
    __syncthreads();
    constexpr bool WIDE = wide_bands(NB);
    __shared__ double s_F[WIDE ? NB * TILE : 1];
    const LdsColumn Fc = (LdsColumn)s_F + (WIDE ? threadIdx.x : 0);
    auto lane_model = [&](int item) -> int32_t {
        if (item < 0) return 0;
        const ItemGeom ig = items[item];
        const int64_t q = ig.q0 + threadIdx.x;
        const int64_t last = ig.q0 + ig.n - 1;
        return der_idx[q < last ? q : last];
    };
    const int64_t slot0 = cand_off[nstar];
    ItemWalk wk;
    wk.init(wbase, nstar, blockIdx.x & 7, blockIdx.x >> 3, (gridDim.x + 7 - (blockIdx.x & 7)) >> 3, run);
    if (wk.done()) return;
    int item = wk.item;
    wk.next();
    int item1 = wk.item;
    constexpr bool PIPE = NB <= 12;
    int32_t i0 = lane_model(item), i1 = lane_model(item1);
    RowRegs<NB> nx;
    if (PIPE) gather_row<NB>(grid, nmodel_pad, i0, nx);
    landed(i1);
    if (PIPE) landed<NB>(nx);
    while (item >= 0) {
        Coef<NB> c;
        if (PIPE) {
            row_to_coef<NB>(nx, c);
            gather_row<NB>(grid, nmodel_pad, i1, nx);
        } else {
            gather_row<NB>(grid, nmodel_pad, i0, nx);
            row_to_coef<NB>(nx, c);
        }
        if (item1 >= 0) wk.next();
        const int item2 = item1 >= 0 ? wk.item : -1;
        int32_t i2 = lane_model(item2);
        const ItemGeom ig = items[item];
        const int s = ig.s;
        const int64_t slot = slot0 + ig.q0 + threadIdx.x;
        const bool live = (int)threadIdx.x < ig.n && slot < rec.cap;
        const bool wave_live = (int)(threadIdx.x & ~63u) < ig.n;
        double o_lnl = 0., o_av = 0., o_rv = 0.;
        Mle m;
        if (wave_live) {
            const StarPrep &sp = stars[s];
            double F0[WIDE ? 1 : NB];
#ifdef BRUTUS_F0_FROM_TABLE
            if constexpr (!WIDE) load_F0<NB>(grid, nmodel_pad, i0, F0);
#else
            if constexpr (!WIDE) compute_F0_tbl<NB>(c, s_tbl, F0);
#endif
            double av = p.av_mean, rv = p.rv_mean;
            const int K = k1[s];
            if constexpr (RVF) {
                double R[WIDE ? 1 : NB];
                GramR G;
                if constexpr (WIDE) {
                    gram_init_rf_wide<NB>(c, rv, sp, G);
                } else {
                    coef_R<NB>(c, rv, R);
                    gram_init_rf<NB>(c, R, sp, G);
                }
                double a_, c_;
                if (K > 0) gram_sweep_rf(G, sp.S, p, av, a_, c_);
                mle_list<NB, true, true>(c, R, F0, Fc, sp, p, av, rv, s_tbl, m);
            } else {
                Gram G;
                gram_init<NB>(c, sp, G);
                for (int kk = 0; kk < K; ++kk) {
                    double a_, b_, c_;
                    gram_sweep(G, sp.S, p, av, rv, a_, b_, c_);
                }
                const double R1[1] = {0.};
                mle_list<NB, false, true>(c, R1, F0, Fc, sp, p, av, rv, s_tbl, m);
            }
            o_lnl = final_lnl<RVF>(sp, p, m.chi2, false);
            o_av = av;
            o_rv = rv;
        }
        if (PIPE) landed<NB>(nx);
        landed(i2);
        if (wave_live && live) {
            double *out = rec.vals + slot;
#define REC_ST(k, x) __builtin_nontemporal_store((x), out + (int64_t)(k) * rec.cap)
            REC_ST(0, o_lnl);
            REC_ST(1, m.chi2);
            REC_ST(2, m.scale);
            REC_ST(3, o_av);
            if constexpr (!RVF) REC_ST(4, o_rv);
            REC_ST(5, m.i00);
            REC_ST(6, m.i01);
            REC_ST(7, m.i02);
            REC_ST(8, m.i11);
            REC_ST(9, m.i12);
            REC_ST(10, m.i22);
#undef REC_ST
        }
        item = item1;
        item1 = item2;
        i0 = i1;
        i1 = i2;
    }
}

}
```

### brutus_amd/csrc/post_kernels.hpp

```cpp
#pragma once

#include "common.hpp"
#include "fastmath.hpp"
#include "mt_kernels.hpp"

namespace {

struct Philox4 {
    uint32_t w[4];
};

#define ZIG_TABLE_QUAL __device__ const
#include "zig_table.inc"
#undef ZIG_TABLE_QUAL

__device__ __forceinline__ Philox4 philox4x32_7(uint32_t c0, uint32_t c1, uint32_t c2, uint32_t c3,
                                                uint32_t k0, uint32_t k1) {
#pragma unroll
    for (int r = 0; r < 7; ++r) {
        if (r > 0) {
            k0 += 0x9E3779B9u;
            k1 += 0xBB67AE85u;
        }
        const uint64_t p0 = (uint64_t)0xD2511F53u * c0, p1 = (uint64_t)0xCD9E8D57u * c2;
        const uint32_t hi0 = (uint32_t)(p0 >> 32), lo0 = (uint32_t)p0;
        const uint32_t hi1 = (uint32_t)(p1 >> 32), lo1 = (uint32_t)p1;
        const uint32_t n0 = hi1 ^ c1 ^ k0, n2 = hi0 ^ c3 ^ k1;
        c0 = n0;
        c1 = lo1;
        c2 = n2;
        c3 = lo0;
    }
    Philox4 o;
    o.w[0] = c0; o.w[1] = c1; o.w[2] = c2; o.w[3] = c3;
    return o;
}

__device__ __forceinline__ double u53(uint32_t a, uint32_t b) {
    return ((double)(a >> 5) * 67108864.0 + (double)(b >> 6)) / 9007199254740992.0;
}

__device__ __forceinline__ double rng_uniform(uint64_t seed, uint64_t q) {
    const Philox4 o = philox4x32_7((uint32_t)q, (uint32_t)(q >> 32), 0u, 1u ,
                                   (uint32_t)seed, (uint32_t)(seed >> 32));
    return u53(o.w[0], o.w[1]);
}

constexpr uint32_t STREAM_NORMAL = 0u, STREAM_UNIFORM = 1u, STREAM_RETRY = 2u, STREAM_TAIL = 3u;

__device__ __forceinline__ bool zig_try(uint32_t a, uint32_t b, const double *__restrict__ X,
                                        double &x, int &i, bool &neg) {
    i = (int)(b & (uint32_t)(ZIG_N - 1));
    neg = (b >> 10) & 1u;
    const double u = ldexp((double)a * 2097152.0 + (double)(b >> 11), -53);
    x = u * X[i];
    return x < X[i + 1];
}
__device__ __forceinline__ double zig_signed(double x, uint32_t b) {
    return __hiloint2double(__double2hiint(x) | (int)((b << 21) & 0x80000000u), __double2loint(x));
}
__device__ __forceinline__ Philox4 philox_at(uint64_t seed, uint64_t idx, uint32_t c2, uint32_t stream) {
    return philox4x32_7((uint32_t)idx, (uint32_t)(idx >> 32), c2, stream, (uint32_t)seed,
                        (uint32_t)(seed >> 32));
}
__device__ __forceinline__ double zig_slow(uint64_t seed, uint64_t j, double x, int i, bool neg) {
#pragma clang fp contract(off)
    for (uint32_t r = 0;; ++r) {
        const Philox4 v = philox_at(seed, j, r, STREAM_RETRY);
        if (r > 0 && zig_try(v.w[0], v.w[1], kZigX, x, i, neg)) break;
        if (i == 0) {
            const double R = kZigX[1];
            for (uint32_t k = 0;; ++k) {
                const Philox4 t = philox_at(seed, j, (r << 16) | k, STREAM_TAIL);
                const double xt = -log(1.0 - u53(t.w[0], t.w[1])) / R;
                const double yt = -log(1.0 - u53(t.w[2], t.w[3]));
                if (yt + yt > xt * xt) {
                    x = R + xt;
                    break;
                }
            }
            break;
        }
        const double u2 = u53(v.w[2], v.w[3]);
        const double yl = kZigY[i] + u2 * (kZigY[i + 1] - kZigY[i]);
        if (yl < exp(-0.5 * x * x)) break;
    }
    return neg ? -x : x;
}
__device__ __forceinline__ void rng_normal_call(uint64_t seed, uint64_t q, const double *__restrict__ X,
                                                double &z0, double &z1) {
    const Philox4 o = philox_at(seed, q, 0u, STREAM_NORMAL);
    double x0, x1;
    int i0, i1;
    bool n0, n1;
    const bool f0 = zig_try(o.w[0], o.w[1], X, x0, i0, n0), f1 = zig_try(o.w[2], o.w[3], X, x1, i1, n1);
    z0 = n0 ? -x0 : x0;
    z1 = n1 ? -x1 : x1;
    if (!f0) z0 = zig_slow(seed, 2 * q, x0, i0, n0);
    if (!f1) z1 = zig_slow(seed, 2 * q + 1, x1, i1, n1);
}
__device__ __forceinline__ double rng_normal(uint64_t seed, uint64_t j) {
    double z0, z1;
    rng_normal_call(seed, j >> 1, kZigX, z0, z1);
    return (j & 1) ? z1 : z0;
}
__device__ __forceinline__ void stage_zig_table(double *lds_x) {
    for (int k = threadIdx.x; k <= ZIG_N; k += blockDim.x) lds_x[k] = kZigX[k];
}
__device__ __forceinline__ void stage_zig_pairs(double2 *lds_p) {
    for (int k = threadIdx.x; k < ZIG_N; k += blockDim.x)
        lds_p[k] = make_double2(ldexp(kZigX[k], -53), kZigX[k + 1]);
}
__device__ __forceinline__ bool zig_try_p(uint32_t a, uint32_t b, const double2 *__restrict__ P, double &x) {
    const double2 e = P[b & (uint32_t)(ZIG_N - 1)];
    x = ((double)a * 2097152.0 + (double)(b >> 11)) * e.x;
    return x < e.y;
}

struct PostParams {
    int32_t nmc, ndraws, return_distreds, has_feh, has_loga, per_object;
    double wt_thresh, avlim[2], rvlim[2];
    int64_t nsel_max, object0;
    uint64_t seed, normal_base, uniform_base;
    double R_solar, Z_solar, R_thin, Z_thin, Rs_thin, R_thick, Z_thick, f_thick, Rs_thick;
    double Rs_halo, q_halo_ctr, q_halo_inf, r_q_halo, eta_halo, f_halo;
    double feh_mean[3], feh_sigma[3];
    double age_mean[3], age_sigma[3], age_lnnorm[3], min_age, max_age;
    double frame_mat[9], frame_off[3];
    double ln_f_thick, ln_f_halo, inv_reff_solar2;
    double inv_R_thin, inv_Z_thin, inv_R_thick, inv_Z_thick, inv_r_q;
    double Rs_thin2, Rs_thick2, Rs_halo2, rq2, abs_Z_solar;
    double lnK, c0_thin, c0_thick, c0_halo;
    double feh_nh_isig2[3], feh_c0[3], age_isig[3], age_c0[3];
    double halo_b[7], halo_tbl;
};
constexpr int POST_DERIVED = 37;

__device__ __forceinline__ uint64_t star_seed(const PostParams &pp, int s) {
    return pp.per_object ? pp.seed + (uint64_t)(pp.object0 + s) : pp.seed;
}
__device__ __forceinline__ uint64_t star_ubase(const PostParams &pp, int s) {
    return pp.per_object ? 0ull
                         : pp.uniform_base + (uint64_t)s * (uint64_t)(pp.ndraws * (pp.return_distreds ? 2 : 1));
}

struct StarGeom {
    double ux, uy, uz;
    double par, par_ivar, par_lnorm;
    int has_par;
    int dust_on, nd;
    const double *los;
    double d_off, d_scale, d_smooth, d_scat2;
    int dt_on, dt_nd;
    const double *dtab;
    double mc[32];
};

enum McC {
    MC_A2, MC_A1, MC_A0, MC_UZ, MC_O2, MC_RS_THIN2, MC_RS_THICK2, MC_C0T, MC_IRT, MC_IZT, MC_C0K,
    MC_IRK, MC_IZK, MC_QINF, MC_DQE, MC_RQ2, MC_IRQ, MC_RS_HALO2, MC_B1, MC_B2, MC_B3, MC_B4, MC_B5,
    MC_B6, MC_B7, MC_AV0, MC_AV1, MC_RV0, MC_RV1, MC_PAR, MC_PIVAR, MC_NC
};
static_assert(MC_NC <= 32, "StarGeom::mc");
typedef const double __attribute__((address_space(4))) *CPtr;
__device__ __forceinline__ CPtr mc_refresh(CPtr p) {
    uint64_t a = (uint64_t)p;
    asm volatile("" : "+s"(a));
    return (CPtr)a;
}

struct DustCtx {
    const double *d_los;
    const int32_t *d_ok;
    int nd;
    double offset, scale, smooth, scatter;
};

__device__ __forceinline__ double dust_lnp(const StarGeom &g, double dist, double av) {
    const double *xp = g.los, *fm = g.los + g.nd, *fe = g.los + 2 * g.nd;
    double m, e;
    if (!(dist > xp[0])) {
        m = dist == dist ? fm[0] : dist;
        e = fe[0];
    } else if (dist >= xp[g.nd - 1]) {
        m = fm[g.nd - 1];
        e = fe[g.nd - 1];
    } else {
        int lo = 0, hi = g.nd - 1;
        while (hi - lo > 1) {
            const int mid = (lo + hi) >> 1;
            if (xp[mid] <= dist) lo = mid; else hi = mid;
        }
        const double dx = xp[lo + 1] - xp[lo], t = dist - xp[lo];
        m = (fm[lo + 1] - fm[lo]) / dx * t + fm[lo];
        e = (fe[lo + 1] - fe[lo]) / dx * t + fe[lo];
    }
    const double mean = g.d_scale * m + g.d_off;
    const double er = g.d_smooth * g.d_scale * e;
    const double e2 = er * er + g.d_scat2;
    const double dv = av - mean;
    return -0.5 * (dv * dv / e2 + log(2. * M_PI * e2));
}

struct DistCtx {
    const double *d_tab;
    int nd, replace;
};
constexpr int DT_OFF = 0, DT_MUL = 1, DT_REP = 2, DT_RT = 3;

__device__ __forceinline__ double dtab_lnp(const double *__restrict__ tab, int nd, double dist) {
    const double *xp = tab, *fp = tab + nd;
    if (!(dist > xp[0])) return dist == dist ? fp[0] : dist;
    if (dist >= xp[nd - 1]) return fp[nd - 1];
    int lo = 0, hi = nd - 1;
    while (hi - lo > 1) {
        const int mid = (lo + hi) >> 1;
        if (xp[mid] <= dist) lo = mid; else hi = mid;
    }
    return (fp[lo + 1] - fp[lo]) / (xp[lo + 1] - xp[lo]) * (dist - xp[lo]) + fp[lo];
}

__device__ __forceinline__ double lse3(double a, double b, double c) {
    double m = a > b ? a : b;
    m = c > m ? c : m;
    if (!(m > -INFINITY)) return m;
    return log(exp(a - m) + exp(b - m) + exp(c - m)) + m;
}

__device__ __forceinline__ void label_terms(const PostParams &pp, double feh, double loga,
                                            double (&Fc)[3], double (&Ac)[3],
                                            const double *__restrict__ tbl = kExp2Tbl) {
    const double age = pp.has_loga ? fast_exp10(loga - 9., tbl) : 0.;
    const bool age_out = age < pp.min_age || age > pp.max_age;
#pragma unroll
    for (int c = 0; c < 3; ++c) {
        Fc[c] = 1.;
        Ac[c] = 1.;
        if (pp.has_feh) {
            const double d = pp.feh_mean[c] - feh;
            Fc[c] = fast_exp_fin(fma(d * d, pp.feh_nh_isig2[c], pp.feh_c0[c]), tbl);
        }
        if (pp.has_loga) {
            const double xi = (age - pp.age_mean[c]) * pp.age_isig[c];
            Ac[c] = age_out ? 0. : fast_exp_fin(fma(-0.5 * xi, xi, pp.age_c0[c]), tbl);
        }
    }
}

constexpr int HALO_E0 = 8, HALO_TBL = 384;
__device__ __forceinline__ void stage_halo_table(const PostParams &pp, double *ht) {
    if (pp.halo_tbl == 0.) return;
    const double h = 0.5 * pp.eta_halo;
    for (int k = threadIdx.x; k < 128; k += blockDim.x) {
        const double ic = 1. / (1. + ((double)k + 0.5) * (1. / 128.));
        ht[256 + k] = ic;
        ht[128 + k] = pow(ic, h);
        ht[k] = exp(pp.c0_halo) * pow(pp.inv_reff_solar2, -h) * pow(2., -h * (double)(k - HALO_E0));
    }
}
template <class B>
__device__ __forceinline__ double halo_pow(const B &hb, double Y, const double *__restrict__ ht) {
    const unsigned hi = (unsigned)__double2hiint(Y);
    const unsigned ie = ((hi >> 20) - (unsigned)(1023 - HALO_E0)) & 127u;
    const unsigned k = (hi >> 13) & 127u;
    const double m = __hiloint2double((int)((hi & 0x000fffffu) | 0x3ff00000u), __double2loint(Y));
    const double r = fma(m, ht[256 + k], -1.);
    double pl = hb[6];
    pl = fma(pl, r, hb[5]);
    pl = fma(pl, r, hb[4]);
    pl = fma(pl, r, hb[3]);
    pl = fma(pl, r, hb[2]);
    pl = fma(pl, r, hb[1]);
    pl = fma(pl, r, hb[0]);
    pl = fma(pl, r, 1.);
    return (ht[ie] * ht[128 + k]) * pl;
}

__device__ __forceinline__ double gal_prior_lin(const PostParams &pp, const StarGeom &g, double d,
                                                const double (&EF)[3], const double (&EA)[3],
                                                const double *__restrict__ tbl,
                                                const double *__restrict__ ht = nullptr) {
    const double x = fma(d, g.ux, pp.frame_off[0]), y = fma(d, g.uy, pp.frame_off[1]),
                 Z = fma(d, g.uz, pp.frame_off[2]);
    const double R2 = x * x + y * y;
    const double dZ = fabs(Z) - pp.abs_Z_solar;
    const double Rt = fast_sqrt(R2 + pp.Rs_thin2);
    const double Rk = pp.Rs_thick2 == pp.Rs_thin2 ? Rt : fast_sqrt(R2 + pp.Rs_thick2);
    const double T0 = fast_exp_fin(pp.c0_thin - (Rt * pp.inv_R_thin + dZ * pp.inv_Z_thin), tbl);
    const double T1 = fast_exp_fin(pp.c0_thick - (Rk * pp.inv_R_thick + dZ * pp.inv_Z_thick), tbl);
    const double q = pp.q_halo_inf -
                     (pp.q_halo_inf - pp.q_halo_ctr) *
                         fast_exp_fin(1. - fast_sqrt(R2 + Z * Z + pp.rq2) * pp.inv_r_q, tbl);
    const double zq = Z * fast_rcp(q);
    const double Y = R2 + zq * zq + pp.Rs_halo2;
    const double T2 = ht ? halo_pow(pp.halo_b, Y, ht)
                         : fast_exp_fin(pp.c0_halo - 0.5 * pp.eta_halo * fast_log_pos(Y * pp.inv_reff_solar2), tbl);
    double num = d * d + 1e-300;
    if (pp.has_feh) num *= T0 * EF[0] + T1 * EF[1] + T2 * EF[2];
    if (pp.has_loga) num *= T0 * EA[0] + T1 * EA[1] + T2 * EA[2];
    const double S = T0 + T1 + T2;
    const int npow = (pp.has_feh ? 1 : 0) + (pp.has_loga ? 1 : 0);
    if (npow == 2) num *= fast_rcp(S);
    else if (npow == 0) num *= S;
    return num;
}
__device__ __forceinline__ double gal_lnprior_dev(const PostParams &pp, const StarGeom &g, double d,
                                                  const double (&EF)[3], const double (&EA)[3],
                                                  const double *__restrict__ tbl) {
    return pp.lnK + fast_log_r(gal_prior_lin(pp, g, d, EF, EA, tbl));
}

constexpr int PCH = 64;

__device__ __forceinline__ int64_t mask_base(const int64_t *__restrict__ off, int s) {
    return ((off[s] + 63) >> 6) + 8 * (int64_t)s;
}

__device__ __forceinline__ void rec_range(const int64_t *__restrict__ off, int s, int c, int64_t &a,
                                          int64_t &b) {
    const int64_t lo = off[s], n = off[s + 1] - lo;
    const int64_t ntile = (n + TILE - 1) / TILE;
    a = lo + (ntile * c / PCH) * TILE;
    b = lo + (ntile * (c + 1) / PCH) * TILE;
    if (b > lo + n) b = lo + n;
    if (a > lo + n) a = lo + n;
}

__device__ __forceinline__ void rec_range_n(int64_t lo, int64_t n, int c, int64_t &a, int64_t &b) {
    const int64_t ntile = (n + TILE - 1) / TILE;
    a = lo + (ntile * c / PCH) * TILE;
    b = lo + (ntile * (c + 1) / PCH) * TILE;
    if (b > lo + n) b = lo + n;
    if (a > lo + n) a = lo + n;
}

__global__ void __launch_bounds__(TILE)
k_post_lnp1(PostParams pp, int64_t cap, const int32_t *__restrict__ sel_idx, const int32_t *__restrict__ rec_slot,
            const double *__restrict__ sel_vals, const int64_t *__restrict__ sel_off,
            const StarGeom *__restrict__ geom, const double *__restrict__ lnprior,
            const double *__restrict__ feh, const double *__restrict__ loga,
            double *__restrict__ lnp1, double *__restrict__ part) {
    __shared__ double slot[4];
    __shared__ double s_tbl[64];
    stage_exp_table(s_tbl);
    __syncthreads();
    const int s = blockIdx.y, c = blockIdx.x;
    int64_t a, b;
    rec_range(sel_off, s, c, a, b);
    const StarGeom g = geom[s];
    double m = -INFINITY;
    for (int64_t r0 = a; r0 < b; r0 += TILE) {
        const int64_t r = r0 + threadIdx.x;
        if (r < b) {
            const int64_t i = sel_idx[r], vs = rec_slot[r];
            double Fc[3], Ac[3];
            label_terms(pp, pp.has_feh ? feh[i] : 0., pp.has_loga ? loga[i] : 0., Fc, Ac, s_tbl);
            const double scale = sel_vals[2 * cap + vs];
            const double dist = 1. / sqrt(scale);
            double v = sel_vals[vs] + lnprior[i];
            if (g.dt_on != DT_REP) v += gal_lnprior_dev(pp, g, dist, Fc, Ac, s_tbl);
            if (g.dt_on) v += dtab_lnp(g.dtab, g.dt_nd, dist);
            if (g.dust_on) v += dust_lnp(g, dist, sel_vals[3 * cap + vs]);
            lnp1[r] = v;
            if (v > m) m = v;
        }
    }
    block_max_store(m, slot, part + (int64_t)s * PCH + c);
}

__global__ void __launch_bounds__(TILE)
k_post_count2(double ln_wt, const int64_t *__restrict__ sel_off, const double *__restrict__ lnp1,
              const double *__restrict__ part, int64_t *__restrict__ counts,
              unsigned long long *__restrict__ mask) {
    __shared__ int wsum[4];
    const int s = blockIdx.y, c = blockIdx.x;
    double mx = -INFINITY;
    for (int q = 0; q < PCH; ++q) {
        const double v = part[(int64_t)s * PCH + q];
        mx = v > mx ? v : mx;
    }
    const double thr = mx + ln_wt;
    int64_t a, b;
    rec_range(sel_off, s, c, a, b);
    int n = 0;
    for (int64_t r0 = a; r0 < b; r0 += TILE) {
        const int64_t r = r0 + threadIdx.x;
        const bool hit = r < b && lnp1[r] > thr;
        n += hit ? 1 : 0;
        const unsigned long long bl = __ballot(hit);
        if ((threadIdx.x & 63) == 0)
            mask[mask_base(sel_off, s) + ((r0 - sel_off[s]) >> 6) + (threadIdx.x >> 6)] = bl;
    }
#pragma unroll
    for (int off = 32; off > 0; off >>= 1) n += __shfl_xor(n, off, 64);
    if ((threadIdx.x & 63) == 0) wsum[threadIdx.x >> 6] = n;
    __syncthreads();
    if (threadIdx.x == 0) counts[(int64_t)s * PCH + c] = wsum[0] + wsum[1] + wsum[2] + wsum[3];
}

__global__ void k_post_offsets(PostParams pp, int nstar, const int64_t *__restrict__ counts,
                               int64_t *__restrict__ offsets, int64_t *__restrict__ off2,
                               uint64_t *__restrict__ nbase, int32_t *__restrict__ flags,
                               int64_t *__restrict__ nsel) {
    __shared__ int64_t tot[BRUTUS_MAX_BATCH + 1];
    const int s = threadIdx.x;
    int64_t n = 0;
    if (s < nstar)
        for (int c = 0; c < PCH; ++c) n += counts[(int64_t)s * PCH + c];
    if (s < nstar) tot[s] = n;
    __syncthreads();
    if (s == 0) {
        int64_t run = 0;
        uint64_t nb = pp.normal_base;
        for (int q = 0; q < nstar; ++q) {
            const int64_t m = tot[q];
            tot[q] = run;
            off2[q] = run;
            nbase[q] = pp.per_object ? 0ull : nb;
            const int64_t used = m > pp.nsel_max ? pp.nsel_max : m;
            flags[q] = m > pp.nsel_max ? 1 : 0;
            nsel[q] = used;
            nb += (uint64_t)(3 * (int64_t)pp.nmc * used);
            run += m;
        }
        off2[nstar] = run;
        nbase[nstar] = nb;
    }
    __syncthreads();
    if (s < nstar) {
        int64_t run = tot[s];
        for (int c = 0; c < PCH; ++c) {
            offsets[(int64_t)s * PCH + c] = run;
            run += counts[(int64_t)s * PCH + c];
        }
    }
}

struct RecPost {
    int32_t *src;
    double *lnp;
    double *chol;
};

__device__ __forceinline__ bool inv3_sym(const double (&A)[6], double (&C)[6]) {
    const double a00 = A[0], a01 = A[1], a02 = A[2], a11 = A[3], a12 = A[4], a22 = A[5];
    const double c00 = a11 * a22 - a12 * a12, c01 = a12 * a02 - a01 * a22, c02 = a01 * a12 - a11 * a02;
    const double c11 = a22 * a00 - a02 * a02, c12 = a02 * a01 - a12 * a00;
    const double c22 = a00 * a11 - a01 * a01;
    const double d0 = c00 * a00 + c01 * a01 + c02 * a02;
    const double d1 = c01 * a01 + c11 * a11 + c12 * a12;
    const double d2 = c02 * a02 + c12 * a12 + c22 * a22;
    const double det = (d0 + d1 + d2) / 3.;
    C[0] = c00 / det; C[1] = c01 / det; C[2] = c02 / det;
    C[3] = c11 / det; C[4] = c12 / det; C[5] = c22 / det;
    return true;
}

__device__ __forceinline__ bool is_pd3(const double (&C)[6]) {
    const double m2 = C[0] * C[3] - C[1] * C[1];
    const double m3 = C[0] * (C[3] * C[5] - C[4] * C[4]) - C[1] * (C[1] * C[5] - C[4] * C[2]) +
                      C[2] * (C[1] * C[4] - C[3] * C[2]);
    return C[0] > 0. && m2 > 0. && m3 > 0.;
}

__device__ __forceinline__ void rec_cov(const double *__restrict__ sel_vals, int64_t cap, int64_t vs,
                                        double (&C)[6]) {
    double A[6];
#pragma unroll
    for (int k = 0; k < 6; ++k) A[k] = sel_vals[(int64_t)(5 + k) * cap + vs];
    inv3_sym(A, C);
    const double scale = sel_vals[2 * cap + vs];
    const double width = 0.02;
    double count = 1.;
    for (int it = 0; it < 200 && !is_pd3(C); ++it) {
        const double sf = scale * width;
        const bool i1 = C[0] <= 0., i2 = C[3] <= 0., i3 = C[5] <= 0.;
        if (i1 || (!i2 && !i3)) A[0] += count / (sf * sf);
        if (i2 || (!i1 && !i3)) A[3] += count / (width * width);
        if (i3 || (!i1 && !i2)) A[5] += count / (width * width);
        inv3_sym(A, C);
        count *= 2.;
    }
}

__global__ void __launch_bounds__(TILE)
k_post_scatter2(int64_t cap, const int32_t *__restrict__ sel_idx, const int32_t *__restrict__ rec_slot, const double *__restrict__ sel_vals,
                const int64_t *__restrict__ sel_off, const double *__restrict__ lnprior,
                const unsigned long long *__restrict__ mask, const int64_t *__restrict__ offsets,
                RecPost rp) {
    __shared__ int wsum[4];
    const int s = blockIdx.y, c = blockIdx.x;
    int64_t a, b;
    rec_range(sel_off, s, c, a, b);
    int64_t base = offsets[(int64_t)s * PCH + c];
    const int lane = threadIdx.x & 63, w = threadIdx.x >> 6;
    for (int64_t r0 = a; r0 < b; r0 += TILE) {
        const int64_t r = r0 + threadIdx.x;
        const unsigned long long bl = mask[mask_base(sel_off, s) + ((r0 - sel_off[s]) >> 6) + w];
        const bool sel = (bl >> lane) & 1ull;
        const int rank = __popcll(bl & ((1ull << lane) - 1ull));
        if (lane == 0) wsum[w] = __popcll(bl);
        __syncthreads();
        int woff = 0;
        for (int q = 0; q < w; ++q) woff += wsum[q];
        const int tot = wsum[0] + wsum[1] + wsum[2] + wsum[3];
        if (sel) {
            const int64_t o = base + woff + rank;
            rp.src[o] = (int32_t)(r - sel_off[s]);
            const int64_t vs = rec_slot[r];
            rp.lnp[o] = sel_vals[vs] + lnprior[sel_idx[r]];
            double C[6];
            rec_cov(sel_vals, cap, vs, C);
            const double l00 = sqrt(C[0] + 1e-30);
            const double l10 = C[1] / l00, l20 = C[2] / l00;
            const double l11 = sqrt(C[3] + 1e-30 - l10 * l10);
            const double l21 = (C[4] - l20 * l10) / l11;
            const double l22 = sqrt(C[5] + 1e-30 - l20 * l20 - l21 * l21);
            rp.chol[0 * cap + o] = l00;
            rp.chol[1 * cap + o] = l10;
            rp.chol[2 * cap + o] = l11;
            rp.chol[3 * cap + o] = l20;
            rp.chol[4 * cap + o] = l21;
            rp.chol[5 * cap + o] = l22;
        }
        base += tot;
        __syncthreads();
    }
}

struct NormalReader {
    uint64_t seed, p;
    double z0, z1;
    bool have;
    const double *zs;
    const ZMap *zm;
// ... 1022 lines not shown
```

Before: 39150 stars/s.

## Use 2048-entry exp2 table with cubic polynomial for fast_exp10

Replaces the 64-entry table plus degree-5 polynomial in fast_exp10 with a 2048-entry table and a cubic, cutting FMAs per exp10 in the F0 computation. Kernels now either stage the larger table in LDS (16KB) or read it straight from constant memory, and the F0 computation in the list kernel is moved after the Gram sweep with an asm dependency so it does not raise register pressure. top_waves is raised to 3 for twelve bands or fewer. The larger LDS footprint and scattered constant-memory lookups may cut occupancy or add memory latency, and precision depends on the new table.

Result: no change. 39330 stars/s (median of 6 runs) (+0.5%).

```diff
diff --git a/brutus_amd/csrc/exp2_table.inc b/brutus_amd/csrc/exp2_table.inc
--- /dev/null
+++ b/brutus_amd/csrc/exp2_table.inc
@@ -0,0 +1,515 @@
+constexpr int EXP10_TBL_LOGN = 11;
+__constant__ double kExp2TblFine[2048] = {
+    0x1.0000000000000p+0, 0x1.00162f3904052p+0, 0x1.002c605e2e8cfp+0, 0x1.0042936faa3d8p+0,
+    0x1.0058c86da1c0ap+0, 0x1.006eff583fc3dp+0, 0x1.0085382faef83p+0, 0x1.009b72f41a12bp+0,
+    0x1.00b1afa5abcbfp+0, 0x1.00c7ee448ee02p+0, 0x1.00de2ed0ee0f5p+0, 0x1.00f4714af41d3p+0,
+    0x1.010ab5b2cbd11p+0, 0x1.0120fc089ff63p+0, 0x1.0137444c9b5b5p+0, 0x1.014d8e7ee8d2fp+0,
+    0x1.0163da9fb3335p+0, 0x1.017a28af25567p+0, 0x1.019078ad6a19fp+0, 0x1.01a6ca9aac5f3p+0,
+    0x1.01bd1e77170b4p+0, 0x1.01d37442d5070p+0, 0x1.01e9cbfe113efp+0, 0x1.020025a8f6a35p+0,
+    0x1.02168143b0281p+0, 0x1.022cdece68c4fp+0, 0x1.02433e494b755p+0, 0x1.02599fb483385p+0,
+    0x1.027003103b10ep+0, 0x1.0286685c9e059p+0, 0x1.029ccf99d720ap+0, 0x1.02b338c811703p+0,
+    0x1.02c9a3e778061p+0, 0x1.02e010f835f7bp+0, 0x1.02f67ffa765e6p+0, 0x1.030cf0ee64571p+0,
+    0x1.032363d42b027p+0, 0x1.0339d8abf5851p+0, 0x1.03504f75ef071p+0, 0x1.0366c83242b47p+0,
+    0x1.037d42e11bbccp+0, 0x1.0393bf82a5538p+0, 0x1.03aa3e170aafep+0, 0x1.03c0be9e770cbp+0,
+    0x1.03d7411915a8ap+0, 0x1.03edc58711c63p+0, 0x1.04044be896ab6p+0, 0x1.041ad43dcfa24p+0,
+    0x1.04315e86e7f85p+0, 0x1.0447eac40aff0p+0, 0x1.045e78f5640b9p+0, 0x1.0475091b1e76dp+0,
+    0x1.048b9b35659d8p+0, 0x1.04a22f4464e00p+0, 0x1.04b8c54847a28p+0, 0x1.04cf5d41394cfp+0,
+    0x1.04e5f72f654b1p+0, 0x1.04fc9312f70c5p+0, 0x1.051330ec1a03fp+0, 0x1.0529d0baf9a8fp+0,
+    0x1.0540727fc1762p+0, 0x1.0557163a9ce9fp+0, 0x1.056dbbebb786bp+0, 0x1.058463933cd29p+0,
+    0x1.059b0d3158574p+0, 0x1.05b1b8c635a28p+0, 0x1.05c866520045bp+0, 0x1.05df15d4e3d5ep+0,
+    0x1.05f5c74f0bec2p+0, 0x1.060c7ac0a4252p+0, 0x1.06233029d8216p+0, 0x1.0639e78ad3853p+0,
+    0x1.0650a0e3c1f89p+0, 0x1.06675c34cf276p+0, 0x1.067e197e26c14p+0, 0x1.0694d8bff479ap+0,
+    0x1.06ab99fa6407cp+0, 0x1.06c25d2da1268p+0, 0x1.06d92259d794dp+0, 0x1.06efe97f33152p+0,
+    0x1.0706b29ddf6dep+0, 0x1.071d7db608693p+0, 0x1.07344ac7d9d51p+0, 0x1.074b19d37f833p+0,
+    0x1.0761ead925493p+0, 0x1.0778bdd8f7005p+0, 0x1.078f92d32085dp+0, 0x1.07a669c7cdba9p+0,
+    0x1.07bd42b72a836p+0, 0x1.07d41da162c8cp+0, 0x1.07eafa86a2771p+0, 0x1.0801d967157e8p+0,
+    0x1.0818ba42e7d30p+0, 0x1.082f9d1a456c5p+0, 0x1.084681ed5a462p+0, 0x1.085d68bc525fcp+0,
+    0x1.0874518759bc8p+0, 0x1.088b3c4e9c635p+0, 0x1.08a22912465f2p+0, 0x1.08b917d283be8p+0,
+    0x1.08d0088f8093fp+0, 0x1.08e6fb4968f5dp+0, 0x1.08fdf00068fe2p+0, 0x1.0914e6b4accafp+0,
+    0x1.092bdf66607e0p+0, 0x1.0942da15b03cdp+0, 0x1.0959d6c2c830dp+0, 0x1.0970d56dd4875p+0,
+    0x1.0987d61701716p+0, 0x1.099ed8be7b23dp+0, 0x1.09b5dd646dd77p+0, 0x1.09cce40905c8cp+0,
+    0x1.09e3ecac6f383p+0, 0x1.09faf74ed66a0p+0, 0x1.0a1203f067a63p+0, 0x1.0a2912914f38cp+0,
+    0x1.0a402331b9715p+0, 0x1.0a5735d1d2a39p+0, 0x1.0a6e4a71c726ep+0, 0x1.0a856111c3568p+0,
+    0x1.0a9c79b1f3919p+0, 0x1.0ab39452843b1p+0, 0x1.0acab0f3a1b9cp+0, 0x1.0ae1cf9578784p+0,
+    0x1.0af8f03834e52p+0, 0x1.0b1012dc0372cp+0, 0x1.0b27378110974p+0, 0x1.0b3e5e2788ccbp+0,
+    0x1.0b5586cf9890fp+0, 0x1.0b6cb1796c65ep+0, 0x1.0b83de2530d11p+0, 0x1.0b9b0cd3125bfp+0,
+    0x1.0bb23d833d93fp+0, 0x1.0bc97035df0a2p+0, 0x1.0be0a4eb2353bp+0, 0x1.0bf7dba337098p+0,
+    0x1.0c0f145e46c85p+0, 0x1.0c264f1c7f30ep+0, 0x1.0c3d8bde0ce7ap+0, 0x1.0c54caa31c94fp+0,
+    0x1.0c6c0b6bdae53p+0, 0x1.0c834e3874886p+0, 0x1.0c9a93091632ap+0, 0x1.0cb1d9ddec9bbp+0,
+    0x1.0cc922b7247f7p+0, 0x1.0ce06d94ea9d7p+0, 0x1.0cf7ba776bb94p+0, 0x1.0d0f095ed49a3p+0,
+    0x1.0d265a4b520bap+0, 0x1.0d3dad3d10dc9p+0, 0x1.0d5502343de02p+0, 0x1.0d6c593105ed4p+0,
+    0x1.0d83b23395decp+0, 0x1.0d9b0d3c1a933p+0, 0x1.0db26a4ac0ed5p+0, 0x1.0dc9c95fb5d37p+0,
+    0x1.0de12a7b26300p+0, 0x1.0df88d9d3ef15p+0, 0x1.0e0ff2c62d096p+0, 0x1.0e2759f61d6e6p+0,
+    0x1.0e3ec32d3d1a2p+0, 0x1.0e562e6bb90a8p+0, 0x1.0e6d9bb1be415p+0, 0x1.0e850aff79c41p+0,
+    0x1.0e9c7c55189c6p+0, 0x1.0eb3efb2c7d7bp+0, 0x1.0ecb6518b4874p+0, 0x1.0ee2dc870bc07p+0,
+    0x1.0efa55fdfa9c5p+0, 0x1.0f11d17dae37fp+0, 0x1.0f294f0653b45p+0, 0x1.0f40ce9818366p+0,
+    0x1.0f58503328e6dp+0, 0x1.0f6fd3d7b2f26p+0, 0x1.0f875985e389bp+0, 0x1.0f9ee13de7e15p+0,
+    0x1.0fb66affed31bp+0, 0x1.0fcdf6cc20b73p+0, 0x1.0fe584a2afb21p+0, 0x1.0ffd1483c7669p+0,
+    0x1.1014a66f951cep+0, 0x1.102c3a6646210p+0, 0x1.1043d06807c2fp+0, 0x1.105b68750756ap+0,
+    0x1.1073028d7233ep+0, 0x1.108a9eb175b68p+0, 0x1.10a23ce13f3e2p+0, 0x1.10b9dd1cfc2e8p+0,
+    0x1.10d17f64d9ef1p+0, 0x1.10e923b905eb7p+0, 0x1.1100ca19ad92fp+0, 0x1.11187286fe591p+0,
+    0x1.11301d0125b51p+0, 0x1.1147c98851223p+0, 0x1.115f781cae1fap+0, 0x1.117728be6a309p+0,
+    0x1.118edb6db2dc1p+0, 0x1.11a6902ab5ad2p+0, 0x1.11be46f5a032cp+0, 0x1.11d5ffce9fffep+0,
+    0x1.11edbab5e2ab6p+0, 0x1.120577ab95d00p+0, 0x1.121d36afe70c9p+0, 0x1.1234f7c30403ep+0,
+    0x1.124cbae51a5c8p+0, 0x1.1264801657c12p+0, 0x1.127c4756e9e05p+0, 0x1.129410a6fe6cbp+0,
+    0x1.12abdc06c31ccp+0, 0x1.12c3a97665aafp+0, 0x1.12db78f613d5bp+0, 0x1.12f34a85fb5f7p+0,
+    0x1.130b1e264a0e9p+0, 0x1.1322f3d72dad5p+0, 0x1.133acb98d40a2p+0, 0x1.1352a56b6af72p+0,
+    0x1.136a814f204abp+0, 0x1.13825f4421defp+0, 0x1.139a3f4a9d922p+0, 0x1.13b22162c1466p+0,
+    0x1.13ca058cbae1ep+0, 0x1.13e1ebc8b84ebp+0, 0x1.13f9d416e77afp+0, 0x1.1411be777658bp+0,
+    0x1.1429aaea92de0p+0, 0x1.144199706b04ep+0, 0x1.14598a092ccb7p+0, 0x1.14717cb50633ap+0,
+    0x1.1489717425438p+0, 0x1.14a16846b804fp+0, 0x1.14b9612cec861p+0, 0x1.14d15c26f0d8bp+0,
+    0x1.14e95934f312ep+0, 0x1.15015857214e8p+0, 0x1.1519598da9a9ap+0, 0x1.15315cd8ba461p+0,
+    0x1.154962388149ep+0, 0x1.156169ad2cdefp+0, 0x1.15797336eb333p+0, 0x1.15917ed5ea789p+0,
+    0x1.15a98c8a58e51p+0, 0x1.15c19c5464b2ap+0, 0x1.15d9ae343c1f2p+0, 0x1.15f1c22a0d6cap+0,
+    0x1.1609d83606e12p+0, 0x1.1621f05856c68p+0, 0x1.163a0a912b6acp+0, 0x1.165226e0b3200p+0,
+    0x1.166a45471c3c2p+0, 0x1.168265c495194p+0, 0x1.169a88594c157p+0, 0x1.16b2ad056f92cp+0,
+    0x1.16cad3c92df73p+0, 0x1.16e2fca4b5ad0p+0, 0x1.16fb279835224p+0, 0x1.171354a3dac91p+0,
+    0x1.172b83c7d517bp+0, 0x1.1743b50452885p+0, 0x1.175be85981992p+0, 0x1.17741dc790cc7p+0,
+    0x1.178c554eaea89p+0, 0x1.17a48eef09b7dp+0, 0x1.17bccaa8d0888p+0, 0x1.17d5087c31ad2p+0,
+    0x1.17ed48695bbc0p+0, 0x1.18058a707d4fbp+0, 0x1.181dce91c506ap+0, 0x1.183614cd61836p+0,
+    0x1.184e5d23816c9p+0, 0x1.1866a794536ccp+0, 0x1.187ef4200632bp+0, 0x1.189742c6c8711p+0,
+    0x1.18af9388c8deap+0, 0x1.18c7e66636363p+0, 0x1.18e03b5f3f36bp+0, 0x1.18f8927412a2fp+0,
+    0x1.1910eba4df41fp+0, 0x1.192946f1d3decp+0, 0x1.1941a45b1f487p+0, 0x1.195a03e0f0522p+0,
+    0x1.1972658375d2fp+0, 0x1.198ac942dea64p+0, 0x1.19a32f1f59ab4p+0, 0x1.19bb971915c57p+0,
+    0x1.19d4013041dc2p+0, 0x1.19ec6d650cdadp+0, 0x1.1a04dbb7a5b13p+0, 0x1.1a1d4c283b52dp+0,
+    0x1.1a35beb6fcb75p+0, 0x1.1a4e336418da9p+0, 0x1.1a66aa2fbebc7p+0, 0x1.1a7f231a1d60cp+0,
+    0x1.1a979e2363cf8p+0, 0x1.1ab01b4bc114dp+0, 0x1.1ac89a936440dp+0, 0x1.1ae11bfa7c67bp+0,
+    0x1.1af99f8138a1cp+0, 0x1.1b122527c80b7p+0, 0x1.1b2aacee59c53p+0, 0x1.1b4336d51cf38p+0,
+    0x1.1b5bc2dc40bf0p+0, 0x1.1b745103f4548p+0, 0x1.1b8ce14c66e4cp+0, 0x1.1ba573b5c7a4bp+0,
+    0x1.1bbe084045cd4p+0, 0x1.1bd69eec109b8p+0, 0x1.1bef37b95750bp+0, 0x1.1c07d2a849321p+0,
+    0x1.1c206fb91588fp+0, 0x1.1c390eebeba2ep+0, 0x1.1c51b040fad15p+0, 0x1.1c6a53b8726a0p+0,
+    0x1.1c82f95281c6bp+0, 0x1.1c9ba10f58454p+0, 0x1.1cb44aef2547ap+0, 0x1.1cccf6f21833fp+0,
+    0x1.1ce5a51860746p+0, 0x1.1cfe55622d773p+0, 0x1.1d1707cfaeaedp+0, 0x1.1d2fbc611391cp+0,
+    0x1.1d4873168b9aap+0, 0x1.1d612bf046484p+0, 0x1.1d79e6ee731d7p+0, 0x1.1d92a41141a12p+0,
+    0x1.1dab6358e15e8p+0, 0x1.1dc424c581e4bp+0, 0x1.1ddce85752c71p+0, 0x1.1df5ae0e839d2p+0,
+    0x1.1e0e75eb44027p+0, 0x1.1e273fedc396bp+0, 0x1.1e400c1631fdbp+0, 0x1.1e58da64bedf8p+0,
+    0x1.1e71aad999e82p+0, 0x1.1e8a7d74f2c7ep+0, 0x1.1ea35236f9330p+0, 0x1.1ebc291fdce22p+0,
+    0x1.1ed5022fcd91dp+0, 0x1.1eeddd66fb02dp+0, 0x1.1f06bac594fa0p+0, 0x1.1f1f9a4bcb409p+0,
+    0x1.1f387bf9cda38p+0, 0x1.1f515fcfcbf45p+0, 0x1.1f6a45cdf6085p+0, 0x1.1f832df47bb94p+0,
+    0x1.1f9c18438ce4dp+0, 0x1.1fb504bb596cep+0, 0x1.1fcdf35c1137ap+0, 0x1.1fe6e425e42f3p+0,
+    0x1.1fffd7190241ep+0, 0x1.2018cc359b625p+0, 0x1.2031c37bdf872p+0, 0x1.204abcebfeab3p+0,
+    0x1.2063b88628cd6p+0, 0x1.207cb64a8df0fp+0, 0x1.2095b6395e1d2p+0, 0x1.20aeb852c95d7p+0,
+    0x1.20c7bc96ffc18p+0, 0x1.20e0c306315d1p+0, 0x1.20f9cba08e483p+0, 0x1.2112d666469efp+0,
+    0x1.212be3578a819p+0, 0x1.2144f2748a14ap+0, 0x1.215e03bd7580cp+0, 0x1.217717327cf2cp+0,
+    0x1.21902cd3d09b9p+0, 0x1.21a944a1a0b07p+0, 0x1.21c25e9c1d6aap+0, 0x1.21db7ac37707bp+0,
+    0x1.21f49917ddc96p+0, 0x1.220db99981f59p+0, 0x1.2226dc4893d64p+0, 0x1.2240012543b9cp+0,
+    0x1.2259282fc1f27p+0, 0x1.227251683ed71p+0, 0x1.228b7cceeac25p+0, 0x1.22a4aa63f6134p+0,
+    0x1.22bdda27912d1p+0, 0x1.22d70c19ec773p+0, 0x1.22f0403b385d2p+0, 0x1.2309768ba54ecp+0,
+    0x1.2322af0b63bffp+0, 0x1.233be9baa428fp+0, 0x1.2355269997062p+0, 0x1.236e65a86cd81p+0,
+    0x1.2387a6e756238p+0, 0x1.23a0ea5683718p+0, 0x1.23ba2ff6254f4p+0, 0x1.23d377c66c4e1p+0,
+    0x1.23ecc1c78903ap+0, 0x1.24060df9ac09bp+0, 0x1.241f5c5d05fe6p+0, 0x1.2438acf1c783ep+0,
+    0x1.2451ffb82140ap+0, 0x1.246b54b043df6p+0, 0x1.2484abda600efp+0, 0x1.249e0536a6828p+0,
+    0x1.24b760c547f15p+0, 0x1.24d0be8675170p+0, 0x1.24ea1e7a5eb35p+0, 0x1.250380a1358a3p+0,
+    0x1.251ce4fb2a63fp+0, 0x1.25364b886e0d0p+0, 0x1.254fb44931561p+0, 0x1.25691f3da5140p+0,
+    0x1.25828c65fa1ffp+0, 0x1.259bfbc261576p+0, 0x1.25b56d530b9bcp+0, 0x1.25cee11829d31p+0,
+    0x1.25e85711ece75p+0, 0x1.2601cf4085c6ep+0, 0x1.261b49a425645p+0, 0x1.2634c63cfcb65p+0,
+    0x1.264e450b3cb82p+0, 0x1.2667c60f1668ep+0, 0x1.26814948bacc3p+0, 0x1.269aceb85ae9dp+0,
+    0x1.26b4565e27cddp+0, 0x1.26cde03a52888p+0, 0x1.26e76c4d0c2e5p+0, 0x1.2700fa9685d82p+0,
+    0x1.271a8b16f0a30p+0, 0x1.27341dce7db03p+0, 0x1.274db2bd5e254p+0, 0x1.276749e3c32c0p+0,
+    0x1.2780e341ddf29p+0, 0x1.279a7ed7dfab5p+0, 0x1.27b41ca5f98cbp+0, 0x1.27cdbcac5cd1cp+0,
+    0x1.27e75eeb3ab98p+0, 0x1.28010362c4877p+0, 0x1.281aaa132b832p+0, 0x1.283452fca0f8ap+0,
+    0x1.284dfe1f56381p+0, 0x1.2867ab7b7c95fp+0, 0x1.28815b11456b1p+0, 0x1.289b0ce0e2147p+0,
+    0x1.28b4c0ea83f36p+0, 0x1.28ce772e5c6d7p+0, 0x1.28e82fac9cecap+0, 0x1.2901ea6576df0p+0,
+    0x1.291ba7591bb70p+0, 0x1.29356687bceb6p+0, 0x1.294f27f18bf72p+0, 0x1.2968eb96ba59ap+0,
+    0x1.2982b17779965p+0, 0x1.299c7993fb354p+0, 0x1.29b643ec70c27p+0, 0x1.29d010810bce8p+0,
+    0x1.29e9df51fdee1p+0, 0x1.2a03b05f78ba5p+0, 0x1.2a1d83a9add08p+0, 0x1.2a375930ced25p+0,
+    0x1.2a5130f50d65cp+0, 0x1.2a6b0af69b350p+0, 0x1.2a84e735a9eecp+0, 0x1.2a9ec5b26b45bp+0,
+    0x1.2ab8a66d10f13p+0, 0x1.2ad28965ccac9p+0, 0x1.2aec6e9cd037bp+0, 0x1.2b0656124d56bp+0,
+    0x1.2b203fc675d1fp+0, 0x1.2b3a2bb97b763p+0, 0x1.2b5419eb90148p+0, 0x1.2b6e0a5ce5823p+0,
+    0x1.2b87fd0dad990p+0, 0x1.2ba1f1fe1a36ep+0, 0x1.2bbbe92e5d3e3p+0, 0x1.2bd5e29ea8959p+0,
+    0x1.2befde4f2e280p+0, 0x1.2c09dc401fe4cp+0, 0x1.2c23dc71afbf7p+0, 0x1.2c3ddee40fb02p+0,
+    0x1.2c57e39771b2fp+0, 0x1.2c71ea8c07c89p+0, 0x1.2c8bf3c203f5fp+0, 0x1.2ca5ff3998446p+0,
+    0x1.2cc00cf2f6c18p+0, 0x1.2cda1cee517f3p+0, 0x1.2cf42f2bda93dp+0, 0x1.2d0e43abc41a0p+0,
+    0x1.2d285a6e4030bp+0, 0x1.2d42737380fb4p+0, 0x1.2d5c8ebbb8a15p+0, 0x1.2d76ac47194efp+0,
+    0x1.2d90cc15d5346p+0, 0x1.2daaee281e867p+0, 0x1.2dc5127e277e3p+0, 0x1.2ddf39182258fp+0,
+    0x1.2df961f641589p+0, 0x1.2e138d18b6c33p+0, 0x1.2e2dba7fb4e33p+0, 0x1.2e47ea2b6e077p+0,
+    0x1.2e621c1c14833p+0, 0x1.2e7c5051daadfp+0, 0x1.2e9686ccf2e3bp+0, 0x1.2eb0bf8d8f849p+0,
+    0x1.2ecafa93e2f56p+0, 0x1.2ee537e01f9f1p+0, 0x1.2eff777277ef0p+0, 0x1.2f19b94b1e570p+0,
+    0x1.2f33fd6a454d2p+0, 0x1.2f4e43d01f4bep+0, 0x1.2f688c7cded23p+0, 0x1.2f82d770b6634p+0,
+    0x1.2f9d24abd886bp+0, 0x1.2fb7742e77c89p+0, 0x1.2fd1c5f8c6b93p+0, 0x1.2fec1a0af7ed6p+0,
+    0x1.300670653dfe4p+0, 0x1.3020c907cb896p+0, 0x1.303b23f2d330bp+0, 0x1.30558126879a7p+0,
+    0x1.306fe0a31b715p+0, 0x1.308a4268c1648p+0, 0x1.30a4a677ac276p+0, 0x1.30bf0cd00e71ep+0,
+    0x1.30d975721b004p+0, 0x1.30f3e05e04933p+0, 0x1.310e4d93fdefbp+0, 0x1.3128bd1439df5p+0,
+    0x1.31432edeeb2fdp+0, 0x1.315da2f444b39p+0, 0x1.3178195479413p+0, 0x1.319291ffbbb3cp+0,
+    0x1.31ad0cf63eeacp+0, 0x1.31c78a3835ca1p+0, 0x1.31e209c5d33a0p+0, 0x1.31fc8b9f4a275p+0,
+    0x1.32170fc4cd831p+0, 0x1.323196369042ep+0, 0x1.324c1ef4c560ap+0, 0x1.3266a9ff9fdacp+0,
+    0x1.3281375752b40p+0, 0x1.329bc6fc10f3ap+0, 0x1.32b658ee0da54p+0, 0x1.32d0ed2d7bd8ep+0,
+    0x1.32eb83ba8ea32p+0, 0x1.33061c95791ccp+0, 0x1.3320b7be6e633p+0, 0x1.333b5535a1984p+0,
+    0x1.3355f4fb45e20p+0, 0x1.3370970f8e6b3p+0, 0x1.338b3b72ae62dp+0, 0x1.33a5e224d8fc7p+0,
+    0x1.33c08b26416ffp+0, 0x1.33db36771af9cp+0, 0x1.33f5e41798daap+0, 0x1.34109407ee57fp+0,
+    0x1.342b46484ebb4p+0, 0x1.3445fad8ed52cp+0, 0x1.3460b1b9fd712p+0, 0x1.347b6aebb26d5p+0,
+    0x1.3496266e3fa2dp+0, 0x1.34b0e441d8719p+0, 0x1.34cba466b03e1p+0, 0x1.34e666dcfa710p+0,
+    0x1.35012ba4ea77dp+0, 0x1.351bf2beb3c42p+0, 0x1.3536bc2a89cc4p+0, 0x1.355187e8a00aep+0,
+    0x1.356c55f929ff1p+0, 0x1.3587265c5b2c7p+0, 0x1.35a1f912671b1p+0, 0x1.35bcce1b81578p+0,
+    0x1.35d7a577dd72bp+0, 0x1.35f27f27af022p+0, 0x1.360d5b2b299fcp+0, 0x1.3628398280ea0p+0,
+    0x1.36431a2de883bp+0, 0x1.365dfd2d94143p+0, 0x1.3678e281b7475p+0, 0x1.3693ca2a85cd7p+0,
+    0x1.36aeb428335b4p+0, 0x1.36c9a07af3aa2p+0, 0x1.36e48f22fa77cp+0, 0x1.36ff80207b865p+0,
+    0x1.371a7373aa9cbp+0, 0x1.3735691cbb85fp+0, 0x1.3750611be211cp+0, 0x1.376b5b7152147p+0,
+    0x1.3786581d3f669p+0, 0x1.37a1571fdde55p+0, 0x1.37bc587961726p+0, 0x1.37d75c29fdf3fp+0,
+    0x1.37f26231e754ap+0, 0x1.380d6a9151839p+0, 0x1.3828754870746p+0, 0x1.38438257781f6p+0,
+    0x1.385e91be9c811p+0, 0x1.3879a37e119abp+0, 0x1.3894b7960b71fp+0, 0x1.38afce06be10ep+0,
+    0x1.38cae6d05d866p+0, 0x1.38e601f31de57p+0, 0x1.39011f6f3345fp+0, 0x1.391c3f44d1c41p+0,
+    0x1.393761742d808p+0, 0x1.395285fd7aa09p+0, 0x1.396dace0ed4e1p+0, 0x1.3988d61eb9b74p+0,
+    0x1.39a401b7140efp+0, 0x1.39bf2faa308c8p+0, 0x1.39da5ff8436bcp+0, 0x1.39f592a180ed3p+0,
+    0x1.3a10c7a61d55bp+0, 0x1.3a2bff064ceecp+0, 0x1.3a4738c244064p+0, 0x1.3a6274da36eedp+0,
+    0x1.3a7db34e59ff7p+0, 0x1.3a98f41ee193cp+0, 0x1.3ab4374c020bdp+0, 0x1.3acf7cd5efcc6p+0,
+    0x1.3aeac4bcdf3eap+0, 0x1.3b060f0104d04p+0, 0x1.3b215ba294f39p+0, 0x1.3b3caaa1c41f7p+0,
+    0x1.3b57fbfec6cf4p+0, 0x1.3b734fb9d182fp+0, 0x1.3b8ea5d318befp+0, 0x1.3ba9fe4ad10c4p+0,
+    0x1.3bc559212ef89p+0, 0x1.3be0b6566715fp+0, 0x1.3bfc15eaadfb1p+0, 0x1.3c1777de38434p+0,
+    0x1.3c32dc313a8e5p+0, 0x1.3c4e42e3e9808p+0, 0x1.3c69abf679c2ep+0, 0x1.3c8517692002ep+0,
+    0x1.3ca0853c10f28p+0, 0x1.3cbbf56f81488p+0, 0x1.3cd76803a5c00p+0, 0x1.3cf2dcf8b318dp+0,
+    0x1.3d0e544ede173p+0, 0x1.3d29ce065b842p+0, 0x1.3d454a1f602d0p+0, 0x1.3d60c89a20e40p+0,
+    0x1.3d7c4976d27fap+0, 0x1.3d97ccb5a9db3p+0, 0x1.3db35256dbd67p+0, 0x1.3dceda5a9d55cp+0,
+    0x1.3dea64c123422p+0, 0x1.3e05f18aa2891p+0, 0x1.3e2180b7501ccp+0, 0x1.3e3d124760f3dp+0,
+    0x1.3e58a63b0a09bp+0, 0x1.3e743c92805e2p+0, 0x1.3e8fd54df8f5cp+0, 0x1.3eab706da8d99p+0,
+    0x1.3ec70df1c5175p+0, 0x1.3ee2adda82c14p+0, 0x1.3efe502816ee3p+0, 0x1.3f19f4dab6b9cp+0,
+    0x1.3f359bf29743fp+0, 0x1.3f51456fedb16p+0, 0x1.3f6cf152ef2b8p+0, 0x1.3f889f9bd0e02p+0,
+    0x1.3fa4504ac801cp+0, 0x1.3fc0036009c78p+0, 0x1.3fdbb8dbcb6d2p+0, 0x1.3ff770be4232fp+0,
+    0x1.40132b07a35dfp+0, 0x1.402ee7b82437bp+0, 0x1.404aa6cffa0e5p+0, 0x1.4066684f5a34bp+0,
+    0x1.40822c367a024p+0, 0x1.409df2858ed31p+0, 0x1.40b9bb3cce07cp+0, 0x1.40d5865c6d05ap+0,
+    0x1.40f153e4a136ap+0, 0x1.410d23d5a0095p+0, 0x1.4128f62f9ef0ep+0, 0x1.4144caf2d3653p+0,
+    0x1.4160a21f72e2ap+0, 0x1.417c7bb5b2ea5p+0, 0x1.419857b5c901fp+0, 0x1.41b4361feab3fp+0,
+    0x1.41d016f44d8f5p+0, 0x1.41ebfa332727ap+0, 0x1.4207dfdcad153p+0, 0x1.4223c7f114f50p+0,
+    0x1.423fb2709468ap+0, 0x1.425b9f5b61163p+0, 0x1.42778eb1b0a8bp+0, 0x1.42938073b8cf9p+0,
+    0x1.42af74a1af3f1p+0, 0x1.42cb6b3bc9b00p+0, 0x1.42e764423ddfdp+0, 0x1.43035fb54190bp+0,
+    0x1.431f5d950a897p+0, 0x1.433b5de1ce958p+0, 0x1.4357609bc3850p+0, 0x1.437365c31f2ccp+0,
+    0x1.438f6d5817663p+0, 0x1.43ab775ae20f7p+0, 0x1.43c783cbb50b4p+0, 0x1.43e392aac6413p+0,
+    0x1.43ffa3f84b9d4p+0, 0x1.441bb7b47b105p+0, 0x1.4437cddf8a8fep+0, 0x1.4453e679b0160p+0,
+    0x1.4470018321a1ap+0, 0x1.448c1efc15362p+0, 0x1.44a83ee4c0dbdp+0, 0x1.44c4613d5a9f9p+0,
+    0x1.44e086061892dp+0, 0x1.44fcad3f30cbep+0, 0x1.4518d6e8d965bp+0, 0x1.45350303487fep+0,
+    0x1.4551318eb43ecp+0, 0x1.456d628b52cb4p+0, 0x1.458995f95a532p+0, 0x1.45a5cbd90108bp+0,
+    0x1.45c2042a7d232p+0, 0x1.45de3eee04de2p+0, 0x1.45fa7c23ce7a4p+0, 0x1.4616bbcc103cbp+0,
+    0x1.4632fde7006f4p+0, 0x1.464f4274d5609p+0, 0x1.466b8975c563ep+0, 0x1.4687d2ea06d15p+0,
+    0x1.46a41ed1d0057p+0, 0x1.46c06d2d5761dp+0, 0x1.46dcbdfcd34c8p+0, 0x1.46f911407a306p+0,
+    0x1.471566f8827d0p+0, 0x1.4731bf2522a6ap+0, 0x1.474e19c691265p+0, 0x1.476a76dd0479cp+0,
+    0x1.4786d668b3237p+0, 0x1.47a33869d3aa7p+0, 0x1.47bf9ce09c9abp+0, 0x1.47dc03cd4484ep+0,
+    0x1.47f86d3001fe5p+0, 0x1.4814d9090ba11p+0, 0x1.48314758980bfp+0, 0x1.484db81edde28p+0,
+    0x1.486a2b5c13cd0p+0, 0x1.4886a11070788p+0, 0x1.48a3193c2a96cp+0, 0x1.48bf93df78de3p+0,
+    0x1.48dc10fa920a1p+0, 0x1.48f8908dacda7p+0, 0x1.491512990013fp+0, 0x1.4931971cc2802p+0,
+    0x1.494e1e192aed2p+0, 0x1.496aa78e702dfp+0, 0x1.4987337cc91a5p+0, 0x1.49a3c1e46c8ebp+0,
+    0x1.49c052c5916c4p+0, 0x1.49dce6206e991p+0, 0x1.49f97bf53affdp+0, 0x1.4a1614442d900p+0,
+    0x1.4a32af0d7d3dep+0, 0x1.4a4f4c5161028p+0, 0x1.4a6bec100fdbap+0, 0x1.4a888e49c0cbdp+0,
+    0x1.4aa532feaada6p+0, 0x1.4ac1da2f05135p+0, 0x1.4ade83db0687ap+0, 0x1.4afb3002e64cep+0,
+    0x1.4b17dea6db7d7p+0, 0x1.4b348fc71d388p+0, 0x1.4b514363e2a20p+0, 0x1.4b6df97d62e2cp+0,
+    0x1.4b8ab213d5283p+0, 0x1.4ba76d2770a49p+0, 0x1.4bc42ab86c8f1p+0, 0x1.4be0eac700237p+0,
+    0x1.4bfdad5362a27p+0, 0x1.4c1a725dcb517p+0, 0x1.4c3739e6717aap+0, 0x1.4c5403ed8c6d2p+0,
+    0x1.4c70d073537cap+0, 0x1.4c8d9f77fe01dp+0, 0x1.4caa70fbc35a1p+0, 0x1.4cc744fedae78p+0,
+    0x1.4ce41b817c114p+0, 0x1.4d00f483de431p+0, 0x1.4d1dd00638ed8p+0, 0x1.4d3aae08c3860p+0,
+    0x1.4d578e8bb586bp+0, 0x1.4d74718f466ecp+0, 0x1.4d915713adc1ep+0, 0x1.4dae3f192308cp+0,
+    0x1.4dcb299fddd0dp+0, 0x1.4de816a815ac6p+0, 0x1.4e05063202327p+0, 0x1.4e21f83ddafefp+0,
+    0x1.4e3eeccbd7b2ap+0, 0x1.4e5be3dc2ff30p+0, 0x1.4e78dd6f1b6a6p+0, 0x1.4e95d984d1c81p+0,
+    0x1.4eb2d81d8abffp+0, 0x1.4ecfd9397e0aep+0, 0x1.4eecdcd8e3669p+0, 0x1.4f09e2fbf2958p+0,
+    0x1.4f26eba2e35f0p+0, 0x1.4f43f6cded8f4p+0, 0x1.4f61047d48f73p+0, 0x1.4f7e14b12d6cbp+0,
+    0x1.4f9b2769d2ca7p+0, 0x1.4fb83ca770efep+0, 0x1.4fd5546a3fc17p+0, 0x1.4ff26eb277284p+0,
+    0x1.500f8b804f127p+0, 0x1.502caad3ff72dp+0, 0x1.5049ccadc0412p+0, 0x1.5066f10dc97a0p+0,
+    0x1.508417f4531eep+0, 0x1.50a1416195360p+0, 0x1.50be6d55c7ca9p+0, 0x1.50db9bd122ec9p+0,
+    0x1.50f8ccd3deb0dp+0, 0x1.5116005e33311p+0, 0x1.51333670588bfp+0, 0x1.51506f0a86e4ep+0,
+    0x1.516daa2cf6642p+0, 0x1.518ae7d7df36ep+0, 0x1.51a8280b798f4p+0, 0x1.51c56ac7fda42p+0,
+    0x1.51e2b00da3b14p+0, 0x1.51fff7dca3f75p+0, 0x1.521d423536bbep+0, 0x1.523a8f1794495p+0,
+    0x1.5257de83f4eefp+0, 0x1.5275307a9100ep+0, 0x1.529284fba0d84p+0, 0x1.52afdc075cd2fp+0,
+    0x1.52cd359dfd53dp+0, 0x1.52ea91bfbac28p+0, 0x1.5307f06ccd8bap+0, 0x1.532551a56e20cp+0,
+    0x1.5342b569d4f82p+0, 0x1.53601bba3a8d1p+0, 0x1.537d8496d75fcp+0, 0x1.539aefffe3f54p+0,
+    0x1.53b85df598d78p+0, 0x1.53d5ce782e955p+0, 0x1.53f34187ddc28p+0, 0x1.5410b724def7bp+0,
+    0x1.542e2f4f6ad27p+0, 0x1.544baa07b9f54p+0, 0x1.5469274e05078p+0, 0x1.5486a72284b58p+0,
+    0x1.54a4298571b06p+0, 0x1.54c1ae7704ae4p+0, 0x1.54df35f7766a3p+0, 0x1.54fcc006ffa42p+0,
+    0x1.551a4ca5d920fp+0, 0x1.5537dbd43baa5p+0, 0x1.55556d92600f1p+0, 0x1.557301e07f22cp+0,
+    0x1.559098bed1bdfp+0, 0x1.55ae322d90be2p+0, 0x1.55cbce2cf505bp+0, 0x1.55e96cbd377bep+0,
+    0x1.56070dde910d2p+0, 0x1.5624b1913aaa8p+0, 0x1.564257d56d4a2p+0, 0x1.566000ab61e73p+0,
+    0x1.567dac1351819p+0, 0x1.569b5a0d751e4p+0, 0x1.56b90a9a05c72p+0, 0x1.56d6bdb93c8b0p+0,
+    0x1.56f4736b527dap+0, 0x1.57122bb080b7dp+0, 0x1.572fe68900573p+0, 0x1.574da3f50a7e5p+0,
+    0x1.576b63f4d854cp+0, 0x1.57892688a3072p+0, 0x1.57a6ebb0a3c6dp+0, 0x1.57c4b36d13ca5p+0,
+    0x1.57e27dbe2c4cfp+0, 0x1.58004aa4268f1p+0, 0x1.581e1a1f3bd60p+0, 0x1.583bec2fa56c1p+0,
+    0x1.5859c0d59ca07p+0, 0x1.587798115ac76p+0, 0x1.589571e31939fp+0, 0x1.58b34e4b11567p+0,
+    0x1.58d12d497c7fdp+0, 0x1.58ef0ede941e4p+0, 0x1.590cf30a919edp+0, 0x1.592ad9cdae738p+0,
+    0x1.5948c32824135p+0, 0x1.5966af1a2bfa5p+0, 0x1.59849da3ffa96p+0, 0x1.59a28ec5d8a69p+0,
+    0x1.59c0827ff07ccp+0, 0x1.59de78d280bbep+0, 0x1.59fc71bdc2f8ep+0, 0x1.5a1a6d41f0cdbp+0,
+    0x1.5a386b5f43d92p+0, 0x1.5a566c15f5bf3p+0, 0x1.5a746f664028bp+0, 0x1.5a9275505cc38p+0,
+    0x1.5ab07dd485429p+0, 0x1.5ace88f2f35dcp+0, 0x1.5aec96abe0d1fp+0, 0x1.5b0aa6ff87610p+0,
+    0x1.5b28b9ee20d1ep+0, 0x1.5b46cf77e6f06p+0, 0x1.5b64e79d138d8p+0, 0x1.5b83025de07f2p+0,
+    0x1.5ba11fba87a03p+0, 0x1.5bbf3fb342d0ap+0, 0x1.5bdd62484bf56p+0, 0x1.5bfb8779dcf88p+0,
+    0x1.5c19af482fc8fp+0, 0x1.5c37d9b37e5abp+0, 0x1.5c5606bc02a6dp+0, 0x1.5c743661f6ab6p+0,
+    0x1.5c9268a5946b7p+0, 0x1.5cb09d8715ef3p+0, 0x1.5cced506b543ap+0, 0x1.5ced0f24ac7b2p+0,
+    0x1.5d0b4be135accp+0, 0x1.5d298b3c8af4cp+0, 0x1.5d47cd36e6747p+0, 0x1.5d6611d082522p+0,
+    0x1.5d84590998b93p+0, 0x1.5da2a2e263d9fp+0, 0x1.5dc0ef5b1de9ep+0, 0x1.5ddf3e7401238p+0,
+    0x1.5dfd902d47c65p+0, 0x1.5e1be4872c16dp+0, 0x1.5e3a3b81e85ecp+0, 0x1.5e58951db6eccp+0,
+    0x1.5e76f15ad2148p+0, 0x1.5e955039742eep+0, 0x1.5eb3b1b9d799ap+0, 0x1.5ed215dc36b7bp+0,
+    0x1.5ef07ca0cbf0fp+0, 0x1.5f0ee607d1b29p+0, 0x1.5f2d5211826e8p+0, 0x1.5f4bc0be189bep+0,
+    0x1.5f6a320dceb71p+0, 0x1.5f88a600df413p+0, 0x1.5fa71c9784c0bp+0, 0x1.5fc595d1f9c0fp+0,
+    0x1.5fe411b078d26p+0, 0x1.600290333c8acp+0, 0x1.6021115a7f849p+0, 0x1.603f95267c5f9p+0,
+    0x1.605e1b976dc09p+0, 0x1.607ca4ad8e517p+0, 0x1.609b306918c13p+0, 0x1.60b9beca47c3ep+0,
+    0x1.60d84fd15612ap+0, 0x1.60f6e37e7e6bbp+0, 0x1.611579d1fb925p+0, 0x1.613412cc084f1p+0,
+    0x1.6152ae6cdf6f4p+0, 0x1.61714cb4bbc5bp+0, 0x1.618feda3d829fp+0, 0x1.61ae913a6f78dp+0,
+    0x1.61cd3778bc944p+0, 0x1.61ebe05efa634p+0, 0x1.620a8bed63d1fp+0, 0x1.62293a2433d18p+0,
+    0x1.6247eb03a5585p+0, 0x1.62669e8bf361bp+0, 0x1.628554bd58ee5p+0, 0x1.62a40d981103cp+0,
+    0x1.62c2c91c56acdp+0, 0x1.62e1874a64f97p+0, 0x1.6300482276fe8p+0, 0x1.631f0ba4c7d64p+0,
+    0x1.633dd1d1929fdp+0, 0x1.635c9aa9127fbp+0, 0x1.637b662b829f5p+0, 0x1.639a34591e2d5p+0,
+    0x1.63b90532205d8p+0, 0x1.63d7d8b6c468ap+0, 0x1.63f6aee7458cdp+0, 0x1.641587c3df0d3p+0,
+    0x1.6434634ccc320p+0, 0x1.645341824848bp+0, 0x1.647222648ea3dp+0, 0x1.649105f3da9b2p+0,
+    0x1.64afec30678b7p+0, 0x1.64ced51a70d6bp+0, 0x1.64edc0b231e41p+0, 0x1.650caef7e61fdp+0,
+    0x1.652b9febc8fb7p+0, 0x1.654a938e15ed7p+0, 0x1.656989df08719p+0, 0x1.658882dedc08cp+0,
+    0x1.65a77e8dcc390p+0, 0x1.65c67cec148d8p+0, 0x1.65e57df9f096bp+0, 0x1.660481b79bea1p+0,
+    0x1.6623882552225p+0, 0x1.664291434edf4p+0, 0x1.66619d11cdc5fp+0, 0x1.6680ab910a809p+0,
+    0x1.669fbcc140be7p+0, 0x1.66bed0a2ac343p+0, 0x1.66dde735889b8p+0, 0x1.66fd007a11b33p+0,
+    0x1.671c1c70833f6p+0, 0x1.673b3b1919094p+0, 0x1.675a5c740edf5p+0, 0x1.67798081a0951p+0,
+    0x1.6798a7420a036p+0, 0x1.67b7d0b587083p+0, 0x1.67d6fcdc5386ap+0, 0x1.67f62bb6ab672p+0,
+    0x1.68155d44ca973p+0, 0x1.68349186ed099p+0, 0x1.6853c87d4eb62p+0, 0x1.687302282b9a1p+0,
+    0x1.68923e87bfb7ap+0, 0x1.68b17d9c47168p+0, 0x1.68d0bf65fdc34p+0, 0x1.68f003e51fcfep+0,
+    0x1.690f4b19e9538p+0, 0x1.692e9504966a8p+0, 0x1.694de1a563367p+0, 0x1.696d30fc8bde0p+0,
+    0x1.698c830a4c8d4p+0, 0x1.69abd7cee1755p+0, 0x1.69cb2f4a86ccap+0, 0x1.69ea897d78ceep+0,
+    0x1.6a09e667f3bcdp+0, 0x1.6a29460a33dc8p+0, 0x1.6a48a86475795p+0, 0x1.6a680d76f4e3cp+0,
+    0x1.6a877541ee718p+0, 0x1.6aa6dfc59e7d9p+0, 0x1.6ac64d0241683p+0, 0x1.6ae5bcf81396cp+0,
+    0x1.6b052fa75173ep+0, 0x1.6b24a510376f9p+0, 0x1.6b441d3301feep+0, 0x1.6b63980fed9c4p+0,
+    0x1.6b8315a736c75p+0, 0x1.6ba295f91a04ep+0, 0x1.6bc21905d3df0p+0, 0x1.6be19ecda0e53p+0,
+    0x1.6c012750bdabfp+0, 0x1.6c20b28f66cd2p+0, 0x1.6c404089d8e7dp+0, 0x1.6c5fd14050a07p+0,
+    0x1.6c7f64b30aa09p+0, 0x1.6c9efae243971p+0, 0x1.6cbe93ce38381p+0, 0x1.6cde2f77253cfp+0,
+    0x1.6cfdcddd47645p+0, 0x1.6d1d6f00db723p+0, 0x1.6d3d12e21e2fbp+0, 0x1.6d5cb9814c6b5p+0,
+    0x1.6d7c62dea2f8ap+0, 0x1.6d9c0efa5eb0dp+0, 0x1.6dbbbdd4bc720p+0, 0x1.6ddb6f6df91fcp+0,
+    0x1.6dfb23c651a2fp+0, 0x1.6e1adade02e99p+0, 0x1.6e3a94b549e71p+0, 0x1.6e5a514c63941p+0,
+    0x1.6e7a10a38cee8p+0, 0x1.6e99d2bb02f99p+0, 0x1.6eb9979302bddp+0, 0x1.6ed95f2bc9490p+0,
+    0x1.6ef9298593ae5p+0, 0x1.6f18f6a09f060p+0, 0x1.6f38c67d286ddp+0, 0x1.6f58991b6d08bp+0,
+    0x1.6f786e7ba9fefp+0, 0x1.6f98469e1c7e1p+0, 0x1.6fb8218301b90p+0, 0x1.6fd7ff2a96e7ep+0,
+    0x1.6ff7df9519484p+0, 0x1.7017c2c2c61cdp+0, 0x1.7037a8b3daadbp+0, 0x1.7057916894485p+0,
+    0x1.70777ce1303f6p+0, 0x1.70976b1debeaep+0, 0x1.70b75c1f04a84p+0, 0x1.70d74fe4b7da2p+0,
+    0x1.70f7466f42e87p+0, 0x1.71173fbee3409p+0, 0x1.71373bd3d6551p+0, 0x1.71573aae599dfp+0,
+    0x1.71773c4eaa988p+0, 0x1.719740b506c74p+0, 0x1.71b747e1abb24p+0, 0x1.71d751d4d6e6bp+0,
+    0x1.71f75e8ec5f74p+0, 0x1.72176e0fb67bdp+0, 0x1.72378057e611ap+0, 0x1.72579567925b6p+0,
+    0x1.7277ad3ef9011p+0, 0x1.7297c7de57afep+0, 0x1.72b7e545ec1a8p+0, 0x1.72d80575f3f90p+0,
+    0x1.72f8286ead08ap+0, 0x1.73184e30550c2p+0, 0x1.733876bb29cb8p+0, 0x1.7358a20f69143p+0,
+    0x1.7378d02d50b8fp+0, 0x1.739901151e91ep+0, 0x1.73b934c7107c7p+0, 0x1.73d96b43645b8p+0,
+    0x1.73f9a48a58174p+0, 0x1.7419e09c299d3p+0, 0x1.743a1f7916e05p+0, 0x1.745a61215dd8ep+0,
+    0x1.747aa5953c849p+0, 0x1.749aecd4f0e66p+0, 0x1.74bb36e0b906dp+0, 0x1.74db83b8d2f39p+0,
+    0x1.74fbd35d7cbfdp+0, 0x1.751c25cef4843p+0, 0x1.753c7b0d785e8p+0, 0x1.755cd31946722p+0,
+    0x1.757d2df29ce7cp+0, 0x1.759d8b99b9ed7p+0, 0x1.75bdec0edbb6bp+0, 0x1.75de4f52407c5p+0,
+    0x1.75feb564267c9p+0, 0x1.761f1e44cbfb2p+0, 0x1.763f89f46f40fp+0, 0x1.765ff8734e9cap+0,
+    0x1.768069c1a861dp+0, 0x1.76a0dddfbae9fp+0, 0x1.76c154cdc4937p+0, 0x1.76e1ce8c03c29p+0,
+    0x1.77024b1ab6e09p+0, 0x1.7722ca7a1c5c8p+0, 0x1.77434caa72aa7p+0, 0x1.7763d1abf8444p+0,
+    0x1.7784597eeba8fp+0, 0x1.77a4e4238b5d0p+0, 0x1.77c5719a15ea6p+0, 0x1.77e601e2c9e07p+0,
+    0x1.780694fde5d3fp+0, 0x1.78272aeba85f2p+0, 0x1.7847c3ac50219p+0, 0x1.78685f401bc05p+0,
+    0x1.7888fda749e5dp+0, 0x1.78a99ee219421p+0, 0x1.78ca42f0c88a5p+0, 0x1.78eae9d396795p+0,
+    0x1.790b938ac1cf6p+0, 0x1.792c401689522p+0, 0x1.794cef772bcc9p+0, 0x1.796da1ace80f4p+0,
+    0x1.798e56b7fcf03p+0, 0x1.79af0e98a94adp+0, 0x1.79cfc94f2bfffp+0, 0x1.79f086dbc3f5ep+0,
+    0x1.7a11473eb0187p+0, 0x1.7a320a782f58cp+0, 0x1.7a52d08880ad9p+0, 0x1.7a73996fe3130p+0,
+    0x1.7a94652e958aap+0, 0x1.7ab533c4d71b7p+0, 0x1.7ad60532e6d20p+0, 0x1.7af6d97903c04p+0,
+    0x1.7b17b0976cfdbp+0, 0x1.7b388a8e61a72p+0, 0x1.7b59675e20defp+0, 0x1.7b7a4706e9cd1p+0,
+    0x1.7b9b2988fb9ecp+0, 0x1.7bbc0ee49586dp+0, 0x1.7bdcf719f6bd7p+0, 0x1.7bfde2295e808p+0,
+    0x1.7c1ed0130c132p+0, 0x1.7c3fc0d73ebe2p+0, 0x1.7c60b47635cf9p+0, 0x1.7c81aaf0309b3p+0,
+    0x1.7ca2a4456e7a3p+0, 0x1.7cc3a0762ecb2p+0, 0x1.7ce49f82b0f24p+0, 0x1.7d05a16b34593p+0,
+    0x1.7d26a62ff86f0p+0, 0x1.7d47add13ca87p+0, 0x1.7d68b84f407f8p+0, 0x1.7d89c5aa4373ep+0,
+    0x1.7daad5e2850acp+0, 0x1.7dcbe8f844cebp+0, 0x1.7decfeebc24fep+0, 0x1.7e0e17bd3d240p+0,
+    0x1.7e2f336cf4e62p+0, 0x1.7e5051fb29370p+0, 0x1.7e71736819bcdp+0, 0x1.7e9297b406234p+0,
+    0x1.7eb3bedf2e1b9p+0, 0x1.7ed4e8e9d15c8p+0, 0x1.7ef615d42fa24p+0, 0x1.7f17459e88aebp+0,
+    0x1.7f3878491c491p+0, 0x1.7f59add42a3e4p+0, 0x1.7f7ae63ff260ap+0, 0x1.7f9c218cb4881p+0,
+    0x1.7fbd5fbab091fp+0, 0x1.7fdea0ca26616p+0, 0x1.7fffe4bb55decp+0, 0x1.80212b8e7ef82p+0,
+    0x1.80427543e1a12p+0, 0x1.8063c1dbbdd2dp+0, 0x1.80851156538bep+0, 0x1.80a663b3e2d09p+0,
+    0x1.80c7b8f4abaa9p+0, 0x1.80e91118ee294p+0, 0x1.810a6c20ea617p+0, 0x1.812bca0ce06d9p+0,
+    0x1.814d2add106d9p+0, 0x1.816e8e91ba871p+0, 0x1.818ff52b1ee50p+0, 0x1.81b15ea97db82p+0,
+    0x1.81d2cb0d1736ap+0, 0x1.81f43a562b9c4p+0, 0x1.8215ac84fb2a6p+0, 0x1.82372199c627dp+0,
+    0x1.82589994cce13p+0, 0x1.827a14764fa86p+0, 0x1.829b923e8ed53p+0, 0x1.82bd12edcac4ap+0,
+    0x1.82de968443d9ap+0, 0x1.83001d023a7c8p+0, 0x1.8321a667ef1b2p+0, 0x1.834332b5a2291p+0,
+    0x1.8364c1eb941f7p+0, 0x1.8386540a057cfp+0, 0x1.83a7e91136c5dp+0, 0x1.83c9810168840p+0,
+    0x1.83eb1bdadb46dp+0, 0x1.840cb99dcfa38p+0, 0x1.842e5a4a8634ap+0, 0x1.844ffde13f9a7p+0,
+    0x1.8471a4623c7adp+0, 0x1.84934dcdbd813p+0, 0x1.84b4fa24035eap+0, 0x1.84d6a9654ec9ep+0,
+    0x1.84f85b91e07f1p+0, 0x1.851a10a9f9403p+0, 0x1.853bc8add9d4cp+0, 0x1.855d839dc309cp+0,
+    0x1.857f4179f5b21p+0, 0x1.85a10242b2a5fp+0, 0x1.85c2c5f83ac35p+0, 0x1.85e48c9aceedep+0,
+    0x1.8606562ab00ecp+0, 0x1.862822a81f14dp+0, 0x1.8649f2135cf48p+0, 0x1.866bc46caaa7fp+0,
+    0x1.868d99b4492edp+0, 0x1.86af71ea798e7p+0, 0x1.86d14d0f7cd1dp+0, 0x1.86f32b239409bp+0,
+    0x1.87150c27004c2p+0, 0x1.8736f01a02b53p+0, 0x1.8758d6fcdc666p+0, 0x1.877ac0cfce86dp+0,
+    0x1.879cad931a436p+0, 0x1.87be9d4700ce9p+0, 0x1.87e08febc3608p+0, 0x1.88028581a3370p+0,
+    0x1.88247e08e1957p+0, 0x1.88467981bfc4fp+0, 0x1.886877ec7f144p+0, 0x1.888a794960d7cp+0,
+    0x1.88ac7d98a6699p+0, 0x1.88ce84da91297p+0, 0x1.88f08f0f627cbp+0, 0x1.89129c375bce8p+0,
+    0x1.8934ac52be8f7p+0, 0x1.8956bf61cc361p+0, 0x1.8978d564c63e7p+0, 0x1.899aee5bee2a4p+0,
+    0x1.89bd0a478580fp+0, 0x1.89df2927cdcfbp+0, 0x1.8a014afd08a94p+0, 0x1.8a236fc777a60p+0,
+    0x1.8a4597875c644p+0, 0x1.8a67c23cf887cp+0, 0x1.8a89efe88dba1p+0, 0x1.8aac208a5daa7p+0,
+    0x1.8ace5422aa0dbp+0, 0x1.8af08ab1b49e9p+0, 0x1.8b12c437bf1d4p+0, 0x1.8b3500b50b4fdp+0,
+    0x1.8b574029db01ep+0, 0x1.8b7982967004fp+0, 0x1.8b9bc7fb0c302p+0, 0x1.8bbe1057f1602p+0,
+    0x1.8be05bad61778p+0, 0x1.8c02a9fb9e5e9p+0, 0x1.8c24fb42ea033p+0, 0x1.8c474f8386591p+0,
+    0x1.8c69a6bdb5598p+0, 0x1.8c8c00f1b903ap+0, 0x1.8cae5e1fd35c4p+0, 0x1.8cd0be48466dep+0,
+    0x1.8cf3216b5448cp+0, 0x1.8d1587893f02ep+0, 0x1.8d37f0a248b7fp+0, 0x1.8d5a5cb6b3896p+0,
+    0x1.8d7ccbc6c19e6p+0, 0x1.8d9f3dd2b523dp+0, 0x1.8dc1b2dad04c4p+0, 0x1.8de42adf55502p+0,
+    0x1.8e06a5e0866d9p+0, 0x1.8e2923dea5e85p+0, 0x1.8e4ba4d9f60a1p+0, 0x1.8e6e28d2b9221p+0,
+    0x1.8e90afc931857p+0, 0x1.8eb339bda18f0p+0, 0x1.8ed5c6b04b9f6p+0, 0x1.8ef856a1721cdp+0,
+    0x1.8f1ae99157736p+0, 0x1.8f3d7f803e150p+0, 0x1.8f60186e68793p+0, 0x1.8f82b45c191d6p+0,
+    0x1.8fa553499284bp+0, 0x1.8fc7f5371737ep+0, 0x1.8fea9a24e9c5cp+0, 0x1.900d42134cc29p+0,
+    0x1.902fed0282c8ap+0, 0x1.90529af2ce77ep+0, 0x1.90754be472760p+0, 0x1.9097ffd7b16e8p+0,
+    0x1.90bab6ccce12cp+0, 0x1.90dd70c40b19bp+0, 0x1.91002dbdab403p+0, 0x1.9122edb9f148fp+0,
+    0x1.9145b0b91ffc6p+0, 0x1.916876bb7a289p+0, 0x1.918b3fc142a19p+0, 0x1.91ae0bcabc413p+0,
+    0x1.91d0dad829e70p+0, 0x1.91f3ace9ce785p+0, 0x1.921681ffece05p+0, 0x1.92395a1ac8100p+0,
+    0x1.925c353aa2fe2p+0, 0x1.927f135fc0a74p+0, 0x1.92a1f48a640dcp+0, 0x1.92c4d8bad039cp+0,
+    0x1.92e7bff148396p+0, 0x1.930aaa2e0f204p+0, 0x1.932d977168083p+0, 0x1.935087bb96107p+0,
+    0x1.93737b0cdc5e5p+0, 0x1.939671657e1cep+0, 0x1.93b96ac5be7d1p+0, 0x1.93dc672de0b57p+0,
+    0x1.93ff669e2802bp+0, 0x1.94226916d7a71p+0, 0x1.94456e9832eadp+0, 0x1.946877227d1bfp+0,
+    0x1.948b82b5f98e5p+0, 0x1.94ae9152eb9b9p+0, 0x1.94d1a2f996a33p+0, 0x1.94f4b7aa3e0aap+0,
+    0x1.9517cf65253d1p+0, 0x1.953aea2a8fab7p+0, 0x1.955e07fac0ccdp+0, 0x1.958128d5fc1dcp+0,
+    0x1.95a44cbc8520fp+0, 0x1.95c773ae9f5ecp+0, 0x1.95ea9dac8e658p+0, 0x1.960dcab695c95p+0,
+    0x1.9630faccf9243p+0, 0x1.96542deffc160p+0, 0x1.9677641fe2446p+0, 0x1.969a9d5cef5afp+0,
+    0x1.96bdd9a7670b3p+0, 0x1.96e118ff8d0c6p+0, 0x1.97045b65a51bap+0, 0x1.9727a0d9f2fc0p+0,
+    0x1.974ae95cba768p+0, 0x1.976e34ee3f59dp+0, 0x1.9791838ec57abp+0, 0x1.97b4d53e90b39p+0,
+    0x1.97d829fde4e50p+0, 0x1.97fb81cd05f52p+0, 0x1.981edcac37d05p+0, 0x1.98423a9bbe688p+0,
+    0x1.98659b9bddb5bp+0, 0x1.9888ffacd9b5dp+0, 0x1.98ac66cef66c8p+0, 0x1.98cfd10277e37p+0,
+    0x1.98f33e47a22a2p+0, 0x1.9916ae9eb9561p+0, 0x1.993a220801829p+0, 0x1.995d9883bed0dp+0,
+    0x1.9981121235681p+0, 0x1.99a48eb3a9753p+0, 0x1.99c80e685f2b5p+0, 0x1.99eb91309ac33p+0,
+    0x1.9a0f170ca07bap+0, 0x1.9a329ffcb4995p+0, 0x1.9a562c011b66dp+0, 0x1.9a79bb1a1934cp+0,
+    0x1.9a9d4d47f2598p+0, 0x1.9ac0e28aeb316p+0, 0x1.9ae47ae3481edp+0, 0x1.9b0816514d89ep+0,
+    0x1.9b2bb4d53fe0dp+0, 0x1.9b4f566f6397ap+0, 0x1.9b72fb1ffd285p+0, 0x1.9b96a2e75112ep+0,
+    0x1.9bba4dc5a3dd3p+0, 0x1.9bddfbbb3a131p+0, 0x1.9c01acc858463p+0, 0x1.9c2560ed430e4p+0,
+    0x1.9c49182a3f090p+0, 0x1.9c6cd27f90d9fp+0, 0x1.9c908fed7d2aap+0, 0x1.9cb4507448aa9p+0,
+    0x1.9cd81414380f2p+0, 0x1.9cfbdacd9013dp+0, 0x1.9d1fa4a09579dp+0, 0x1.9d43718d8d089p+0,
+    0x1.9d674194bb8d5p+0, 0x1.9d8b14b665db3p+0, 0x1.9daeeaf2d0cb8p+0, 0x1.9dd2c44a413d6p+0,
+    0x1.9df6a0bcfc15ep+0, 0x1.9e1a804b46403p+0, 0x1.9e3e62f564ad5p+0, 0x1.9e6248bb9c545p+0,
+    0x1.9e86319e32323p+0, 0x1.9eaa1d9d6b4a0p+0, 0x1.9ece0cb98ca4bp+0, 0x1.9ef1fef2db513p+0,
+    0x1.9f15f4499c647p+0, 0x1.9f39ecbe14f97p+0, 0x1.9f5de8508a311p+0, 0x1.9f81e70141324p+0,
+    0x1.9fa5e8d07f29ep+0, 0x1.9fc9edbe894adp+0, 0x1.9fedf5cba4ce0p+0, 0x1.a01200f816f25p+0,
+    0x1.a0360f4424fcbp+0, 0x1.a05a20b01437fp+0, 0x1.a07e353c29f50p+0, 0x1.a0a24ce8ab8adp+0,
+    0x1.a0c667b5de565p+0, 0x1.a0ea85a407ba5p+0, 0x1.a10ea6b36d1fep+0, 0x1.a132cae453f5ep+0,
+    0x1.a156f23701b15p+0, 0x1.a17b1cabbbcd4p+0, 0x1.a19f4a42c7ca9p+0, 0x1.a1c37afc6b306p+0,
+    0x1.a1e7aed8eb8bbp+0, 0x1.a20be5d88e6fbp+0, 0x1.a2301ffb99757p+0, 0x1.a2545d42523c1p+0,
+    0x1.a2789dacfe68cp+0, 0x1.a29ce13be3a6cp+0, 0x1.a2c127ef47a74p+0, 0x1.a2e571c77021ap+0,
+    0x1.a309bec4a2d33p+0, 0x1.a32e0ee7257f5p+0, 0x1.a352622f3def6p+0, 0x1.a376b89d31f2fp+0,
+    0x1.a39b1231475f7p+0, 0x1.a3bf6eebc4108p+0, 0x1.a3e3ceccede7cp+0, 0x1.a40831d50accdp+0,
+    0x1.a42c980460ad8p+0, 0x1.a451015b357d9p+0, 0x1.a4756dd9cf36ep+0, 0x1.a499dd8073d96p+0,
+    0x1.a4be504f696b1p+0, 0x1.a4e2c646f5f7fp+0, 0x1.a5073f675f924p+0, 0x1.a52bbbb0ec521p+0,
+    0x1.a5503b23e255dp+0, 0x1.a574bdc087c1bp+0, 0x1.a599438722c03p+0, 0x1.a5bdcc77f981ep+0,
+    0x1.a5e25893523d4p+0, 0x1.a606e7d9732f1p+0, 0x1.a62b7a4aa29a1p+0, 0x1.a6500fe726c72p+0,
+    0x1.a674a8af46052p+0, 0x1.a69944a346a93p+0, 0x1.a6bde3c36f0e6p+0, 0x1.a6e286100595fp+0,
+    0x1.a7072b8950a73p+0, 0x1.a72bd42f96afap+0, 0x1.a75080031e22bp+0, 0x1.a7752f042d7a1p+0,
+    0x1.a799e1330b358p+0, 0x1.a7be968ffddaep+0, 0x1.a7e34f1b4bf62p+0, 0x1.a8080ad53c195p+0,
+    0x1.a82cc9be14dcap+0, 0x1.a8518bd61cde7p+0, 0x1.a876511d9ac32p+0, 0x1.a89b1994d5354p+0,
+    0x1.a8bfe53c12e59p+0, 0x1.a8e4b4139a8acp+0, 0x1.a909861bb2e1dp+0, 0x1.a92e5b54a2adcp+0,
+    0x1.a95333beb0b7ep+0, 0x1.a9780f5a23cf6p+0, 0x1.a99cee2742c9dp+0, 0x1.a9c1d0265482cp+0,
+    0x1.a9e6b5579fdbfp+0, 0x1.aa0b9dbb6bbd5p+0, 0x1.aa308951ff14dp+0, 0x1.aa55781ba0d6ap+0,
+    0x1.aa7a6a1897fd2p+0, 0x1.aa9f5f492b88cp+0, 0x1.aac457ada2803p+0, 0x1.aae9534643f03p+0,
+    0x1.ab0e521356ebap+0, 0x1.ab335415228bbp+0, 0x1.ab58594bedefap+0, 0x1.ab7d61b8003cdp+0,
+    0x1.aba26d59a09eep+0, 0x1.abc77c311647ap+0, 0x1.abec8e3ea86eep+0, 0x1.ac11a3829e52cp+0,
+    0x1.ac36bbfd3f37ap+0, 0x1.ac5bd7aed267dp+0, 0x1.ac80f6979f340p+0, 0x1.aca618b7ecf31p+0,
+    0x1.accb3e100301ep+0, 0x1.acf066a028c3ap+0, 0x1.ad159268a5a1cp+0, 0x1.ad3ac169c10bbp+0,
+    0x1.ad5ff3a3c2774p+0, 0x1.ad852916f1606p+0, 0x1.adaa61c395493p+0, 0x1.adcf9da9f5b9fp+0,
+    0x1.adf4dcca5a413p+0, 0x1.ae1a1f250a73bp+0, 0x1.ae3f64ba4dec6p+0, 0x1.ae64ad8a6c4c5p+0,
+    0x1.ae89f995ad3adp+0, 0x1.aeaf48dc58659p+0, 0x1.aed49b5eb5803p+0, 0x1.aef9f11d0c44bp+0,
+    0x1.af1f4a17a4735p+0, 0x1.af44a64ec5d26p+0, 0x1.af6a05c2b82e9p+0, 0x1.af8f6873c35acp+0,
+    0x1.afb4ce622f2ffp+0, 0x1.afda378e438d7p+0, 0x1.afffa3f84858cp+0, 0x1.b02513a0857dbp+0,
+    0x1.b04a868742ee4p+0, 0x1.b06ffcacc8a2ap+0, 0x1.b09576115e994p+0, 0x1.b0baf2b54cd6dp+0,
+    0x1.b0e07298db666p+0, 0x1.b105f5bc5258fp+0, 0x1.b12b7c1ff9c61p+0, 0x1.b15105c419cb6p+0,
+    0x1.b17692a8fa8cdp+0, 0x1.b19c22cee4349p+0, 0x1.b1c1b6361ef31p+0, 0x1.b1e74cdef2fefp+0,
+    0x1.b20ce6c9a8952p+0, 0x1.b23283f687f8fp+0, 0x1.b2582465d973cp+0, 0x1.b27dc817e5555p+0,
+    0x1.b2a36f0cf3f3ap+0, 0x1.b2c919454daafp+0, 0x1.b2eec6c13adddp+0, 0x1.b314778103f50p+0,
+    0x1.b33a2b84f15fbp+0, 0x1.b35fe2cd4b932p+0, 0x1.b3859d5a5b0b1p+0, 0x1.b3ab5b2c68495p+0,
+    0x1.b3d11c43bbd62p+0, 0x1.b3f6e0a09e3ffp+0, 0x1.b41ca843581bap+0, 0x1.b442732c32044p+0,
+    0x1.b468415b749b1p+0, 0x1.b48e12d16887dp+0, 0x1.b4b3e78e56786p+0, 0x1.b4d9bf9287210p+0,
+    0x1.b4ff9ade433c6p+0, 0x1.b5257971d38b2p+0, 0x1.b54b5b4d80d4ap+0, 0x1.b571407193e63p+0,
+    0x1.b59728de5593ap+0, 0x1.b5bd14940eb70p+0, 0x1.b5e303930830cp+0, 0x1.b608f5db8ae79p+0,
+    0x1.b62eeb6ddfc87p+0, 0x1.b654e44a4fc6cp+0, 0x1.b67ae07123dc3p+0, 0x1.b6a0dfe2a508bp+0,
+    0x1.b6c6e29f1c52ap+0, 0x1.b6ece8a6d2c6ap+0, 0x1.b712f1fa1177bp+0, 0x1.b738fe99217f1p+0,
+    0x1.b75f0e844bfc6p+0, 0x1.b78521bbda15cp+0, 0x1.b7ab384014f76p+0, 0x1.b7d1521145d3fp+0,
+    0x1.b7f76f2fb5e47p+0, 0x1.b81d8f9bae684p+0, 0x1.b843b35578a51p+0, 0x1.b869da5d5de6fp+0,
+    0x1.b89004b3a7804p+0, 0x1.b8b632589ec9bp+0, 0x1.b8dc634c8d228p+0, 0x1.b902978fbbf01p+0,
+    0x1.b928cf22749e4p+0, 0x1.b94f0a05009f3p+0, 0x1.b9754837a96b7p+0, 0x1.b99b89bab881fp+0,
+    0x1.b9c1ce8e77680p+0, 0x1.b9e816b32fa95p+0, 0x1.ba0e62292ad7dp+0, 0x1.ba34b0f0b28c0p+0,
+    0x1.ba5b030a1064ap+0, 0x1.ba8158758e06dp+0, 0x1.baa7b133751e3p+0, 0x1.bace0d440f5cap+0,
+    0x1.baf46ca7a67a7p+0, 0x1.bb1acf5e84367p+0, 0x1.bb413568f255ap+0, 0x1.bb679ec73aa38p+0,
+    0x1.bb8e0b79a6f1fp+0, 0x1.bbb47b8081194p+0, 0x1.bbdaeedc12f82p+0, 0x1.bc01658ca673bp+0,
+    0x1.bc27df9285775p+0, 0x1.bc4e5cedf9f50p+0, 0x1.bc74dd9f4de4fp+0, 0x1.bc9b61a6cb460p+0,
+    0x1.bcc1e904bc1d2p+0, 0x1.bce873b96a760p+0, 0x1.bd0f01c520628p+0, 0x1.bd35932827fb0p+0,
+    0x1.bd5c27e2cb5e5p+0, 0x1.bd82bff554b1bp+0, 0x1.bda95b600e20bp+0, 0x1.bdcffa2341dd7p+0,
+    0x1.bdf69c3f3a207p+0, 0x1.be1d41b44128ap+0, 0x1.be43ea82a13b5p+0, 0x1.be6a96aaa4a46p+0,
+    0x1.be91462c95b60p+0, 0x1.beb7f908bec8ep+0, 0x1.bedeaf3f6a3c2p+0, 0x1.bf0568d0e2756p+0,
+    0x1.bf2c25bd71e09p+0, 0x1.bf52e60562f02p+0, 0x1.bf79a9a9001d2p+0, 0x1.bfa070a893e6cp+0,
+    0x1.bfc73b0468d30p+0, 0x1.bfee08bcc96e0p+0, 0x1.c014d9d2004aap+0, 0x1.c03bae4458020p+0,
+    0x1.c06286141b33dp+0, 0x1.c089614194863p+0, 0x1.c0b03fcd0ea5cp+0, 0x1.c0d721b6d445ap+0,
+    0x1.c0fe06ff301f4p+0, 0x1.c124efa66cf2cp+0, 0x1.c14bdbacd586ap+0, 0x1.c172cb12b4a7dp+0,
+    0x1.c199bdd85529cp+0, 0x1.c1c0b3fe01e67p+0, 0x1.c1e7ad8405be6p+0, 0x1.c20eaa6aab985p+0,
+    0x1.c235aab23e61ep+0, 0x1.c25cae5b090edp+0, 0x1.c283b56556999p+0, 0x1.c2aabfd172031p+0,
+    0x1.c2d1cd9fa652cp+0, 0x1.c2f8ded03e967p+0, 0x1.c31ff36385e29p+0, 0x1.c3470b59c7521p+0,
+    0x1.c36e26b34e065p+0, 0x1.c395457065275p+0, 0x1.c3bc679157e38p+0, 0x1.c3e38d16716fcp+0,
+    0x1.c40ab5fffd07ap+0, 0x1.c431e24e45ed2p+0, 0x1.c45912019768cp+0, 0x1.c480451a3cc98p+0,
+    0x1.c4a77b9881650p+0, 0x1.c4ceb57cb0975p+0, 0x1.c4f5f2c715c31p+0, 0x1.c51d3377fc517p+0,
+    0x1.c544778fafb22p+0, 0x1.c56bbf0e7b5b6p+0, 0x1.c59309f4aac9fp+0, 0x1.c5ba584289812p+0,
+    0x1.c5e1a9f8630adp+0, 0x1.c608ff1682f76p+0, 0x1.c630579d34dddp+0, 0x1.c657b38cc45b9p+0,
+    0x1.c67f12e57d14bp+0, 0x1.c6a675a7aab3ep+0, 0x1.c6cddbd398ea4p+0, 0x1.c6f54569936f8p+0,
+    0x1.c71cb269e601fp+0, 0x1.c74422d4dc667p+0, 0x1.c76b96aac2686p+0, 0x1.c7930debe3d9cp+0,
+    0x1.c7ba88988c933p+0, 0x1.c7e206b10873bp+0, 0x1.c8098835a3611p+0, 0x1.c8310d26a9479p+0,
+    0x1.c8589584661a1p+0, 0x1.c880214f25d1fp+0, 0x1.c8a7b087346f4p+0, 0x1.c8cf432cddf8bp+0,
+    0x1.c8f6d9406e7b5p+0, 0x1.c91e72c2320b0p+0, 0x1.c9460fb274c22p+0, 0x1.c96db01182c1bp+0,
+    0x1.c99553dfa8313p+0, 0x1.c9bcfb1d313eep+0, 0x1.c9e4a5ca6a1f8p+0, 0x1.ca0c53e79f0e7p+0,
+    0x1.ca3405751c4dbp+0, 0x1.ca5bba732e25dp+0, 0x1.ca8372e220e61p+0, 0x1.caab2ec240e43p+0,
+    0x1.cad2ee13da7cbp+0, 0x1.cafab0d73a12ap+0, 0x1.cb22770cac0f9p+0, 0x1.cb4a40b47ce3fp+0,
+    0x1.cb720dcef9069p+0, 0x1.cb99de5c6cf50p+0, 0x1.cbc1b25d25337p+0, 0x1.cbe989d16e4cbp+0,
+    0x1.cc1164b994d23p+0, 0x1.cc394315e55bfp+0, 0x1.cc6124e6ac88bp+0, 0x1.cc890a2c36fddp+0,
+    0x1.ccb0f2e6d1675p+0, 0x1.ccd8df16c877cp+0, 0x1.cd00cebc68e87p+0, 0x1.cd28c1d7ff795p+0,
+    0x1.cd50b869d8f0fp+0, 0x1.cd78b272421c9p+0, 0x1.cda0aff187d02p+0, 0x1.cdc8b0e7f6e61p+0,
+    0x1.cdf0b555dc3fap+0, 0x1.ce18bd3b84c4bp+0, 0x1.ce40c8993d63dp+0, 0x1.ce68d76f53122p+0,
+    0x1.ce90e9be12cb9p+0, 0x1.ceb8ff85c992ap+0, 0x1.cee118c6c4709p+0, 0x1.cf09358150754p+0,
+    0x1.cf3155b5bab74p+0, 0x1.cf5979645053cp+0, 0x1.cf81a08d5e6ecp+0, 0x1.cfa9cb313232ep+0,
+    0x1.cfd1f95018d17p+0, 0x1.cffa2aea5f825p+0, 0x1.d022600053845p+0, 0x1.d04a9892421ccp+0,
+    0x1.d072d4a07897cp+0, 0x1.d09b142b44480p+0, 0x1.d0c35732f2870p+0, 0x1.d0eb9db7d0b4fp+0,
+    0x1.d113e7ba2c38cp+0, 0x1.d13c353a527ffp+0, 0x1.d164863890feep+0, 0x1.d18cdab535307p+0,
+    0x1.d1b532b08c968p+0, 0x1.d1dd8e2ae4b97p+0, 0x1.d205ed248b287p+0, 0x1.d22e4f9dcd795p+0,
+    0x1.d256b596f948cp+0, 0x1.d27f1f105c3a0p+0, 0x1.d2a78c0a43f72p+0, 0x1.d2cffc84fe310p+0,
+    0x1.d2f87080d89f2p+0, 0x1.d320e7fe20ffap+0, 0x1.d34962fd2517ap+0, 0x1.d371e17e32b2ep+0,
+    0x1.d39a638197a3cp+0, 0x1.d3c2e907a1c38p+0, 0x1.d3eb72109ef21p+0, 0x1.d413fe9cdd164p+0,
+    0x1.d43c8eacaa1d6p+0, 0x1.d465224053fbdp+0, 0x1.d48db95828ac7p+0, 0x1.d4b653f47630fp+0,
+    0x1.d4def2158a91fp+0, 0x1.d50793bbb3de9p+0, 0x1.d53038e7402cep+0, 0x1.d558e1987d99ap+0,
+    0x1.d5818dcfba487p+0, 0x1.d5aa3d8d44639p+0, 0x1.d5d2f0d16a1c3p+0, 0x1.d5fba79c79aa1p+0,
+    0x1.d62461eec14bep+0, 0x1.d64d1fc88f472p+0, 0x1.d675e12a31e7fp+0, 0x1.d69ea613f7816p+0,
+    0x1.d6c76e862e6d3p+0, 0x1.d6f03a81250bfp+0, 0x1.d7190a0529c51p+0, 0x1.d741dd128b06ap+0,
+    0x1.d76ab3a99745bp+0, 0x1.d7938dca9cfdfp+0, 0x1.d7bc6b75eab1fp+0, 0x1.d7e54cabceeb1p+0,
+    0x1.d80e316c98398p+0, 0x1.d83719b895343p+0, 0x1.d86005901478fp+0, 0x1.d888f4f364ac5p+0,
+    0x1.d8b1e7e2d479dp+0, 0x1.d8dade5eb2939p+0, 0x1.d903d8674db2bp+0, 0x1.d92cd5fcf4971p+0,
+    0x1.d955d71ff6075p+0, 0x1.d97edbd0a0d11p+0, 0x1.d9a7e40f43c89p+0, 0x1.d9d0efdc2dc92p+0,
+    0x1.d9f9ff37adb4ap+0, 0x1.da23122212740p+0, 0x1.da4c289baaf6ep+0, 0x1.da7542a4c633ep+0,
+    0x1.da9e603db3285p+0, 0x1.dac78166c0d87p+0, 0x1.daf0a6203e4f5p+0, 0x1.db19ce6a7a9eep+0,
+    0x1.db42fa45c4dfdp+0, 0x1.db6c29b26c31dp+0, 0x1.db955cb0bfbb6p+0, 0x1.dbbe93410ea9dp+0,
+    0x1.dbe7cd63a8315p+0, 0x1.dc110b18db8cfp+0, 0x1.dc3a4c60f7feap+0, 0x1.dc63913c4ccf3p+0,
+    0x1.dc8cd9ab294e4p+0, 0x1.dcb625addcd27p+0, 0x1.dcdf7544b6b92p+0, 0x1.dd08c87006669p+0,
+    0x1.dd321f301b460p+0, 0x1.dd5b798544c98p+0, 0x1.dd84d76fd269ep+0, 0x1.ddae38f013a72p+0,
+    0x1.ddd79e065807dp+0, 0x1.de0106b2ef19bp+0, 0x1.de2a72f628712p+0, 0x1.de53e2d053a9ap+0,
+    0x1.de7d5641c0658p+0, 0x1.dea6cd4abe4ddp+0, 0x1.ded047eb9d12dp+0, 0x1.def9c624ac6b6p+0,
+    0x1.df2347f63c159p+0, 0x1.df4ccd609bd61p+0, 0x1.df7656641b78cp+0, 0x1.df9fe3010ad03p+0,
+    0x1.dfc97337b9b5fp+0, 0x1.dff30708780a8p+0, 0x1.e01c9e7395b56p+0, 0x1.e046397962a4cp+0,
+    0x1.e06fd81a2ece1p+0, 0x1.e0997a564a2d6p+0, 0x1.e0c3202e04c5dp+0, 0x1.e0ecc9a1aea18p+0,
+    0x1.e11676b197d17p+0, 0x1.e140275e106d8p+0, 0x1.e169dba768949p+0, 0x1.e193938df06c8p+0,
+    0x1.e1bd4f11f8220p+0, 0x1.e1e70e33cfe8dp+0, 0x1.e210d0f3c7fbap+0, 0x1.e23a9752309c0p+0,
+    0x1.e264614f5a129p+0, 0x1.e28e2eeb94aecp+0, 0x1.e2b8002730c71p+0, 0x1.e2e1d5027eb91p+0,
+    0x1.e30bad7dcee90p+0, 0x1.e335899971c26p+0, 0x1.e35f6955b7b78p+0, 0x1.e3894cb2f141ap+0,
+    0x1.e3b333b16ee12p+0, 0x1.e3dd1e51811d3p+0, 0x1.e4070c9378842p+0, 0x1.e430fe77a5ab3p+0,
+    0x1.e45af3fe592e8p+0, 0x1.e484ed27e3b15p+0, 0x1.e4aee9f495ddcp+0, 0x1.e4d8ea64c0651p+0,
+    0x1.e502ee78b3ff6p+0, 0x1.e52cf630c16bep+0, 0x1.e557018d3970bp+0, 0x1.e581108e6cdafp+0,
+    0x1.e5ab2334ac7eep+0, 0x1.e5d539804937ap+0, 0x1.e5ff537193e75p+0, 0x1.e6297108dd773p+0,
+    0x1.e653924676d76p+0, 0x1.e67db72ab0ff2p+0, 0x1.e6a7dfb5dcecap+0, 0x1.e6d20be84ba53p+0,
+    0x1.e6fc3bc24e350p+0, 0x1.e7266f4435af7p+0, 0x1.e750a66e532ebp+0, 0x1.e77ae140f7d42p+0,
+    0x1.e7a51fbc74c83p+0, 0x1.e7cf61e11b3a4p+0, 0x1.e7f9a7af3c60bp+0, 0x1.e823f12729791p+0,
+    0x1.e84e3e4933c7ep+0, 0x1.e8788f15ac98ap+0, 0x1.e8a2e38ce53dfp+0, 0x1.e8cd3baf2f118p+0,
+    0x1.e8f7977cdb740p+0, 0x1.e921f6f63bcd2p+0, 0x1.e94c5a1ba18bdp+0, 0x1.e976c0ed5e25dp+0,
+    0x1.e9a12b6bc3181p+0, 0x1.e9cb999721e6ap+0, 0x1.e9f60b6fcc1c7p+0, 0x1.ea2080f6134bcp+0,
+    0x1.ea4afa2a490dap+0, 0x1.ea75770cbf025p+0, 0x1.ea9ff79dc6d14p+0, 0x1.eaca7bddb228cp+0,
+    0x1.eaf503ccd2be5p+0, 0x1.eb1f8f6b7a4e9p+0, 0x1.eb4a1eb9fa9d1p+0, 0x1.eb74b1b8a5749p+0,
+    0x1.eb9f4867cca6ep+0, 0x1.ebc9e2c7c20d0p+0, 0x1.ebf480d8d786dp+0, 0x1.ec1f229b5efb8p+0,
+    0x1.ec49c80faa594p+0, 0x1.ec7471360b955p+0, 0x1.ec9f1e0ed4ac2p+0, 0x1.ecc9ce9a57a12p+0,
+    0x1.ecf482d8e67f1p+0, 0x1.ed1f3acad3578p+0, 0x1.ed49f67070435p+0, 0x1.ed74b5ca0f628p+0,
+    0x1.ed9f78d802dc2p+0, 0x1.edca3f9a9cde5p+0, 0x1.edf50a122f9e6p+0, 0x1.ee1fd83f0d58cp+0,
+    0x1.ee4aaa2188510p+0, 0x1.ee757fb9f2d1dp+0, 0x1.eea059089f2d0p+0, 0x1.eecb360ddfbb8p+0,
+    0x1.eef616ca06dd6p+0, 0x1.ef20fb3d66f9ep+0, 0x1.ef4be368527f6p+0, 0x1.ef76cf4b1be36p+0,
+    0x1.efa1bee615a27p+0, 0x1.efccb23992408p+0, 0x1.eff7a945e4487p+0, 0x1.f022a40b5e4c6p+0,
+    0x1.f04da28a52e59p+0, 0x1.f078a4c314b47p+0, 0x1.f0a3aab5f6609p+0, 0x1.f0ceb4634a98ap+0,
+    0x1.f0f9c1cb6412ap+0, 0x1.f124d2ee958b9p+0, 0x1.f14fe7cd31c7bp+0, 0x1.f17b00678b927p+0,
+    0x1.f1a61cbdf5be7p+0, 0x1.f1d13cd0c3256p+0, 0x1.f1fc60a046a84p+0, 0x1.f227882cd32f3p+0,
+    0x1.f252b376bba97p+0, 0x1.f27de27e530dap+0, 0x1.f2a91543ec595p+0, 0x1.f2d44bc7da917p+0,
+    0x1.f2ff860a70c22p+0, 0x1.f32ac40c01fe8p+0, 0x1.f35605cce1613p+0, 0x1.f3814b4d620bdp+0,
+    0x1.f3ac948dd7274p+0, 0x1.f3d7e18e93e39p+0, 0x1.f403324feb781p+0, 0x1.f42e86d231233p+0,
+    0x1.f459df15b82acp+0, 0x1.f4853b1ad3dbbp+0, 0x1.f4b09ae1d78a1p+0, 0x1.f4dbfe6b16915p+0,
+    0x1.f50765b6e4540p+0, 0x1.f532d0c5943c0p+0, 0x1.f55e3f9779ba5p+0, 0x1.f589b22ce8474p+0,
+    0x1.f5b5288633625p+0, 0x1.f5e0a2a3ae925p+0, 0x1.f60c2085ad652p+0, 0x1.f637a22c83701p+0,
+    0x1.f6632798844f8p+0, 0x1.f68eb0ca03a75p+0, 0x1.f6ba3dc155226p+0, 0x1.f6e5ce7ecc72fp+0,
+    0x1.f7116302bd526p+0, 0x1.f73cfb4d7b819p+0, 0x1.f768975f5ac86p+0, 0x1.f7943738aef61p+0,
+    0x1.f7bfdad9cbe14p+0, 0x1.f7eb824305679p+0, 0x1.f8172d74af6e1p+0, 0x1.f842dc6f1de12p+0,
+    0x1.f86e8f32a4b45p+0, 0x1.f89a45bf97e28p+0, 0x1.f8c600164b6dcp+0, 0x1.f8f1be37135f9p+0,
+    0x1.f91d802243c89p+0, 0x1.f94945d830c0cp+0, 0x1.f9750f592e677p+0, 0x1.f9a0dca590e33p+0,
+    0x1.f9ccadbdac61dp+0, 0x1.f9f882a1d5187p+0, 0x1.fa245b525f439p+0, 0x1.fa5037cf9f26ep+0,
+    0x1.fa7c1819e90d8p+0, 0x1.faa7fc319149cp+0, 0x1.fad3e416ec354p+0, 0x1.faffcfca4e310p+0,
+    0x1.fb2bbf4c0ba54p+0, 0x1.fb57b29c7901ap+0, 0x1.fb83a9bbeabd1p+0, 0x1.fbafa4aab555cp+0,
+    0x1.fbdba3692d514p+0, 0x1.fc07a5f7a73c7p+0, 0x1.fc33ac5677ab8p+0, 0x1.fc5fb685f33a0p+0,
+    0x1.fc8bc4866e8adp+0, 0x1.fcb7d6583e482p+0, 0x1.fce3ebfbb7237p+0, 0x1.fd1005712dd5bp+0,
+    0x1.fd3c22b8f71f1p+0, 0x1.fd6843d367c72p+0, 0x1.fd9468c0d49ccp+0, 0x1.fdc0918192765p+0,
+    0x1.fdecbe15f6314p+0, 0x1.fe18ee7e54b2bp+0, 0x1.fe4522bb02e6ep+0, 0x1.fe715acc55c18p+0,
+    0x1.fe9d96b2a23d9p+0, 0x1.fec9d66e3d5d9p+0, 0x1.fef619ff7c2b3p+0, 0x1.ff226166b3b7ap+0,
+    0x1.ff4eaca4391b6p+0, 0x1.ff7afbb861765p+0, 0x1.ffa74ea381efcp+0, 0x1.ffd3a565efb65p+0,
+};
diff --git a/brutus_amd/csrc/fastmath.hpp b/brutus_amd/csrc/fastmath.hpp
--- a/brutus_amd/csrc/fastmath.hpp
+++ b/brutus_amd/csrc/fastmath.hpp
@@ -20,19 +20,36 @@
     1.8340080864093424, 1.8539791250833855, 1.8741676341103, 1.8945759815869656,
     1.9152065613971474, 1.9360617934922943, 1.9571441241754002, 1.9784560263879509};
 
-__device__ __forceinline__ double fast_exp10(double x, const double *__restrict__ tbl = kExp2Tbl) {
-    const double ns = fma(x, 212.60339807279118, 6755399441055744.0);
+#include "exp2_table.inc"
+
+template <int LOGN, int DEG>
+__device__ __forceinline__ double fast_exp10_form(double x, const double *__restrict__ tbl) {
+    static_assert((LOGN == 6 && DEG == 5) || (LOGN == EXP10_TBL_LOGN && DEG == 3), "no such form");
+    constexpr double up = (double)(1 << (LOGN - 6));
+    const double ns = fma(x, 212.60339807279118 * up, 6755399441055744.0);
     const double n = ns - 6755399441055744.0;
-    double r = fma(-n, 0.0047035936804604717, x);
-    r = fma(-n, 1.7892345153159123e-12, r);
-    double pl = 0.5393829291955817;
-    pl = fma(pl, r, 1.1712551489122673);
-    pl = fma(pl, r, 2.034678592293477);
+    double r = fma(-n, 0.0047035936804604717 / up, x);
+    r = fma(-n, 1.7892345153159123e-12 / up, r);
+    double pl = 2.034678592293477;
+    if constexpr (DEG == 5) {
+        pl = 0.5393829291955817;
+        pl = fma(pl, r, 1.1712551489122673);
+        pl = fma(pl, r, 2.034678592293477);
+    }
     pl = fma(pl, r, 2.6509490552391997);
     pl = fma(pl, r, 2.302585092994046);
-    pl = fma(pl, r, 1.0);
     const int ni = __double2loint(ns);
-    return ldexp(tbl[ni & 63] * pl, ni >> 6);
+    const double t = tbl[ni & ((1 << LOGN) - 1)];
+    if constexpr (LOGN == 6) return ldexp(t * fma(pl, r, 1.0), ni >> LOGN);
+    else return ldexp(fma(t * pl, r, t), ni >> LOGN);
+}
+
+constexpr int EXP10_N = 1 << EXP10_TBL_LOGN;
+__device__ __forceinline__ double fast_exp10(double x, const double *__restrict__ tbl = kExp2TblFine) {
+    return fast_exp10_form<EXP10_TBL_LOGN, 3>(x, tbl);
+}
+__device__ __forceinline__ double fast_exp10_64(double x, const double *__restrict__ tbl = kExp2Tbl) {
+    return fast_exp10_form<6, 5>(x, tbl);
 }
 
 __device__ __forceinline__ double poly_exp10(double x) {
@@ -59,6 +76,9 @@
 
 __device__ __forceinline__ void stage_exp_table(double *lds_tbl) {
     if (threadIdx.x < 64) lds_tbl[threadIdx.x] = kExp2Tbl[threadIdx.x];
+}
+__device__ __forceinline__ void stage_exp10_table(double *lds_tbl) {
+    for (int k = threadIdx.x; k < EXP10_N; k += blockDim.x) lds_tbl[k] = kExp2TblFine[k];
 }
 
 __device__ __forceinline__ double fast_exp(double x, const double *__restrict__ tbl = kExp2Tbl) {
diff --git a/brutus_amd/csrc/fit2_kernels.hpp b/brutus_amd/csrc/fit2_kernels.hpp
--- a/brutus_amd/csrc/fit2_kernels.hpp
+++ b/brutus_amd/csrc/fit2_kernels.hpp
@@ -497,11 +497,9 @@
        const int32_t *__restrict__ hot, const int32_t *__restrict__ nhot,
        double *__restrict__ part, float *__restrict__ aud) {
     __shared__ double slot[4];
-    __shared__ double s_tbl[64];
+    const double *s_tbl = kExp2TblFine;
     const int n = *nhot;
     if ((int)blockIdx.x >= n) return;
-    stage_exp_table(s_tbl);
-    __syncthreads();
     const int lane = threadIdx.x & 63;
     for (int e = blockIdx.x; e < n; e += gridDim.x) {
         const int entry = hot[e];
@@ -906,9 +904,7 @@
     for (int k = 0; k < SB_C; ++k) pre[k + 1] = pre[k] + bandn[s * NCHUNK + c0 + k];
     const int n = pre[SB_C];
     if ((int)(blockIdx.z * TILE) >= n) return;
-    __shared__ double s_tbl[64];
-    stage_exp_table(s_tbl);
-    __syncthreads();
+    const double *s_tbl = kExp2TblFine;
     const StarPrep &sp = stars[s];
     const double th = thr_sel[s];
     const int K = k1[s];
diff --git a/brutus_amd/csrc/fit_kernels.hpp b/brutus_amd/csrc/fit_kernels.hpp
--- a/brutus_amd/csrc/fit_kernels.hpp
+++ b/brutus_amd/csrc/fit_kernels.hpp
@@ -251,7 +251,7 @@
 constexpr int fflux_waves(int nb, bool first) {
     return nb >= (first ? BRUTUS_FFLUX_OCC1_FROM : BRUTUS_LIST_OCC1_FROM) ? 1 : 2;
 }
-constexpr int top_waves(int nb) { return nb > 24 ? 1 : 2; }
+constexpr int top_waves(int nb) { return nb > 24 ? 1 : nb <= 12 ? 3 : 2; }
 constexpr int band_waves(int nb) { return nb > 16 ? 1 : 2; }
 typedef __attribute__((address_space(3))) volatile double *LdsColumn;
 #ifndef BRUTUS_WIDE_GROUP
@@ -383,6 +383,16 @@
                                                double (&F0)[NB]) {
 #pragma unroll
     for (int j = 0; j < NB; ++j) F0[j] = fast_exp10(-0.4 * (double)c.m[j], tbl);
+}
+template <int NB>
+__device__ __forceinline__ void compute_F0_tbl_after(const Coef<NB> &c, const double *__restrict__ tbl,
+                                                     double dep, double (&F0)[NB]) {
+#pragma unroll
+    for (int j = 0; j < NB; ++j) {
+        double x = -0.4 * (double)c.m[j];
+        asm("" : "+v"(x) : "v"(dep));
+        F0[j] = fast_exp10(x, tbl);
+    }
 }
 
 template <bool FASTLOG = false>
@@ -804,9 +814,12 @@
         const int32_t *__restrict__ nact_dev, int run) {
     if (!FIRST && nact_dev) nact = *nact_dev;
     if (!FIRST && nact <= 0) return;
-    __shared__ double s_tbl[64];
-    stage_exp_table(s_tbl);
-    __syncthreads();
+    __shared__ double s_stage[FIRST ? EXP10_N : 1];
+    const double *s_tbl = FIRST ? s_stage : kExp2TblFine;
+    if constexpr (FIRST) {
+        stage_exp10_table(s_stage);
+        __syncthreads();
+    }
     constexpr bool WIDE = wide_bands(NB);
     __shared__ double s_F[WIDE ? NB * TILE : 1];
     const LdsColumn Fc = (LdsColumn)s_F + (WIDE ? threadIdx.x : 0);
@@ -852,11 +865,7 @@
             Coef<NB> c;
             gather_coef<NB>(grid, nmodel_pad, i, c);
             double F0[WIDE ? 1 : NB];
-#ifdef BRUTUS_F0_FROM_TABLE
-            if constexpr (!WIDE) load_F0<NB>(grid, nmodel_pad, i, F0);
-#else
             if constexpr (!WIDE) compute_F0_tbl<NB>(c, s_tbl, F0);
-#endif
             double av, rv, step, lnl_old;
             double R[RVF && !WIDE ? NB : 1];
             if constexpr (RVF && !WIDE) coef_R<NB>(c, p.rv_mean, R);
@@ -1109,8 +1118,8 @@
          const int32_t *__restrict__ der_idx, const int32_t *__restrict__ wbase,
          const ItemGeom *__restrict__ items, const int64_t *__restrict__ cand_off,
          RecPlanes rec, int run) {
-    __shared__ double s_tbl[64];
-    stage_exp_table(s_tbl);
+    __shared__ double s_tbl[EXP10_N];
+    stage_exp10_table(s_tbl);
     __syncthreads();
     constexpr bool WIDE = wide_bands(NB);
     __shared__ double s_F[WIDE ? NB * TILE : 1];
@@ -1157,11 +1166,6 @@
         if (wave_live) {
             const StarPrep &sp = stars[s];
             double F0[WIDE ? 1 : NB];
-#ifdef BRUTUS_F0_FROM_TABLE
-            if constexpr (!WIDE) load_F0<NB>(grid, nmodel_pad, i0, F0);
-#else
-            if constexpr (!WIDE) compute_F0_tbl<NB>(c, s_tbl, F0);
-#endif
             double av = p.av_mean, rv = p.rv_mean;
             const int K = k1[s];
             if constexpr (RVF) {
@@ -1175,6 +1179,7 @@
                 }
                 double a_, c_;
                 if (K > 0) gram_sweep_rf(G, sp.S, p, av, a_, c_);
+                if constexpr (!WIDE) compute_F0_tbl_after<NB>(c, s_tbl, av, F0);
                 mle_list<NB, true, true>(c, R, F0, Fc, sp, p, av, rv, s_tbl, m);
             } else {
                 Gram G;
@@ -1183,6 +1188,7 @@
                     double a_, b_, c_;
                     gram_sweep(G, sp.S, p, av, rv, a_, b_, c_);
                 }
+                if constexpr (!WIDE) compute_F0_tbl_after<NB>(c, s_tbl, av, F0);
                 const double R1[1] = {0.};
                 mle_list<NB, false, true>(c, R1, F0, Fc, sp, p, av, rv, s_tbl, m);
             }
diff --git a/brutus_amd/csrc/post_kernels.hpp b/brutus_amd/csrc/post_kernels.hpp
--- a/brutus_amd/csrc/post_kernels.hpp
+++ b/brutus_amd/csrc/post_kernels.hpp
@@ -230,7 +230,7 @@
 __device__ __forceinline__ void label_terms(const PostParams &pp, double feh, double loga,
                                             double (&Fc)[3], double (&Ac)[3],
                                             const double *__restrict__ tbl = kExp2Tbl) {
-    const double age = pp.has_loga ? fast_exp10(loga - 9., tbl) : 0.;
+    const double age = pp.has_loga ? fast_exp10_64(loga - 9., tbl) : 0.;
     const bool age_out = age < pp.min_age || age > pp.max_age;
 #pragma unroll
     for (int c = 0; c < 3; ++c) {
```
